# zkwebauthn/webauthn-halo2

Hardware: AMD Instinct MI355X
Metric: webauthn_es256_proofs_per_sec_k19 (higher is better)
Workload: dtype u256-montgomery (9x29-bit carry-free limbs in the hot kernels: bucket accumulation, NTT, reduction tails, quotient; 8x32-bit limbs elsewhere and in memory)

## Files before the change

include/zkmi355.h:

```cpp
#ifndef ZKMI355_H
#define ZKMI355_H

#include <stddef.h>
#include <stdint.h>

#ifdef __cplusplus
extern "C" {
#endif

#define ZK_OK 0
#define ZK_EINVAL (-1)
#define ZK_ENOMEM (-2)
#define ZK_EHIP (-3)
#define ZK_ENODEV (-4)
#define ZK_ESTATE (-5)
#define ZK_EWITNESS (-6)
#define ZK_EINTERNAL (-7)
#define ZK_ELAYOUT (-8)

typedef struct zk_ctx zk_ctx;
typedef uint64_t zk_poly;

#define ZK_BASIS_MONOMIAL 0
#define ZK_BASIS_LAGRANGE 1
// ... 106 lines not shown
#define ZK_SCHEME_GWC 1
#define ZK_SCHEME_SHPLONK 2

int zk_keygen(zk_ctx* ctx, const zk_circuit_params* params, const uint64_t* fixed_canonical ,
              size_t n_fixed_columns ,
              const uint32_t* copies, size_t n_copies, zk_pk* out);
int zk_pk_set_transcript_repr(zk_ctx* ctx, zk_pk pk, const uint64_t transcript_repr_mont[4]);
int zk_pk_free(zk_ctx* ctx, zk_pk pk);
int zk_vk_export(zk_ctx* ctx, zk_pk pk, uint64_t* fixed_commitments, uint64_t* perm_commitments,
                 uint64_t transcript_repr[4], uint32_t counts[2]);
int zk_vk_write(zk_ctx* ctx, zk_pk pk, int format, uint8_t* out, size_t cap, size_t* len);
int zk_vk_load(zk_ctx* ctx, zk_pk pk, const uint8_t* vk_bytes, size_t len, int format, const uint64_t transcript_repr_mont[4]);
int zk_pk_write(zk_ctx* ctx, zk_pk pk, int format, uint8_t* out, size_t cap, size_t* len);
int zk_pk_read(zk_ctx* ctx, const zk_circuit_params* params, const uint8_t* bytes, size_t len, int format,
               const uint64_t transcript_repr_mont[4], zk_pk* out);
int zk_pk_shape(zk_ctx* ctx, zk_pk pk, uint32_t out[8]);
int zk_quotient(zk_ctx* ctx, zk_pk pk, const zk_poly* advice_ext, size_t n_advice, const zk_poly* perm_z_ext, size_t n_chunks,
                const zk_poly* lookup_ext, size_t n_lookups, const uint64_t beta[4], const uint64_t gamma[4], const uint64_t y[4],
                int divide, zk_poly out_ext);
int zk_lookup_permute(zk_ctx* ctx, zk_pk pk, const zk_poly* advice, size_t n_advice, zk_poly* permuted_input ,
                      zk_poly* permuted_table , size_t n_lookups);
int zk_lookup_product(zk_ctx* ctx, zk_pk pk, const zk_poly* advice, size_t n_advice, const zk_poly* permuted_input,
                      const zk_poly* permuted_table, size_t n_lookups, const uint64_t beta[4], const uint64_t gamma[4],
                      zk_poly* z_out );
int zk_permutation_product(zk_ctx* ctx, zk_pk pk, const zk_poly* advice, size_t n_advice, const uint64_t beta[4],
                           const uint64_t gamma[4], zk_poly* z_out , size_t n_chunks);
#define ZK_PK_FIXED_POLY 0
#define ZK_PK_SIGMA_POLY 1
int zk_pk_export_poly(zk_ctx* ctx, zk_pk pk, int which, size_t index, zk_poly dst);
int zk_random_poly(zk_ctx* ctx, const uint8_t chacha_key[32], uint64_t first_block, zk_poly out);
int zk_proof_size(zk_ctx* ctx, zk_pk pk, int transcript, int scheme, size_t* out);
int zk_prove(zk_ctx* ctx, zk_pk pk, const zk_poly* advice, size_t n_advice, const uint8_t rng_seed[32],
             int transcript, int scheme, uint8_t* proof_out, size_t proof_cap, size_t* proof_len);
#define ZK_PROVE_BATCH_MAX 64
int zk_prove_batch(zk_ctx* ctx, zk_pk pk, size_t batch, const zk_poly* advice , size_t n_advice,
                   const uint8_t* rng_seeds , int transcript, int scheme, uint8_t* proofs_out, size_t proof_stride,
                   size_t* proof_len);
int zk_poly_upload_canonical(zk_ctx* ctx, zk_poly p, const uint64_t* host_canonical, size_t n);

#define ZK_FAIL_GATE 1
#define ZK_FAIL_GATE_BLINDED 2
#define ZK_FAIL_LOOKUP 3
#define ZK_FAIL_COPY 4
typedef struct { uint32_t kind, index, row, other_index, other_row, reserved; } zk_witness_failure;
int zk_witness_check(zk_ctx* ctx, zk_pk pk, const zk_poly* advice, size_t n_advice, zk_witness_failure* out, size_t cap,
                     uint64_t counts[5]);

#define ZK_PK_PART_FIXED_COMMIT 1
#define ZK_PK_PART_SIGMA_COMMIT 2
#define ZK_PK_PART_FIXED_POLY   3
#define ZK_PK_PART_SIGMA_POLY   4
#define ZK_PK_PART_FIXED_COSET  5
#define ZK_PK_PART_SIGMA_COSET  6
#define ZK_PK_PART_L_COSET      7
#define ZK_PK_PART_SIGMA_LABEL  8
#define ZK_PK_PART_SIGMA_MAP    9
typedef struct { uint32_t part, column, index, reserved; uint64_t count; } zk_pk_finding;

#define ZK_PK_CHECK_COMMITMENTS 1u
#define ZK_PK_CHECK_POLYS       2u
#define ZK_PK_CHECK_COSETS      4u
#define ZK_PK_CHECK_SIGMA       8u
#define ZK_PK_CHECK_ALL        15u
#define ZK_PK_CHECK_REPR       16u
int zk_pk_check(zk_ctx* ctx, zk_pk pk, uint32_t* flags, zk_pk_finding* out, size_t cap, size_t* n_findings);

int zk_vk_read(zk_ctx* ctx, const zk_circuit_params* params, const uint8_t* bytes, size_t len, int format,
               const uint64_t transcript_repr_mont[4], zk_pk* out);
int zk_vk_from_parts(zk_ctx* ctx, const zk_circuit_params* params, const uint64_t* fixed_commitments, const uint64_t* perm_commitments,
                     const uint64_t transcript_repr_mont[4], zk_pk* out);
int zk_verify(zk_ctx* ctx, zk_pk pk, int transcript, int scheme, const uint8_t* proof, size_t len, int* ok);
#define ZK_VERIFY_BATCH_MAX 1024
int zk_verify_batch(zk_ctx* ctx, zk_pk pk, size_t batch, int transcript, int scheme, const uint8_t* const* proofs, const size_t* lens,
                    uint8_t* verdicts);

#define ZK_T_MSM 0
#define ZK_T_NTT 1
#define ZK_T_QUOTIENT 2
#define ZK_T_EVAL 3
#define ZK_T_MSM_ACCUM 4
#define ZK_T_MSM_COLUMNS 5
#define ZK_T_MSM_TAIL_MAIN 6
#define ZK_T_MSM_TAIL 7
#define ZK_T_COUNT 8
int zk_last_kernel_ms(zk_ctx* ctx, int which, float* out_ms);
int zk_audit_report(zk_ctx* ctx, uint64_t counts[2], char* msg, size_t cap);
int zk_timer_reset(zk_ctx* ctx);
int zk_clock_probe(zk_ctx* ctx, uint32_t millis, uint64_t out[4]);
int zk_timer_stats(zk_ctx* ctx, int which, double* total_ms, uint64_t* count);

typedef struct {
    uint32_t n_queues;
    uint32_t flags;
    uint8_t  main_queue[8];
    uint8_t  role_queue[8][3];
    uint8_t  spare_queue[8];
    uint32_t rounds, streams;
    float    probe_ms;
} zk_placement;
#define ZK_PLACEMENT_MAINS_OK   1u
#define ZK_PLACEMENT_LONE_OK    2u
#define ZK_PLACEMENT_PAIR_OK    4u
#define ZK_PLACEMENT_LAYER1_OK  8u
#define ZK_PLACEMENT_OK        15u
#define ZK_PLACEMENT_CALIBRATED 16u
#define ZK_PLACEMENT_UNRESOLVED 32u
int zk_stream_placement(int device_id, int mode , zk_placement* out);
typedef struct {
    int32_t  slot;
    uint8_t  queue[4];
    uint64_t counts[4];
} zk_ctx_streams;
int zk_ctx_stream_info(zk_ctx* ctx, zk_ctx_streams* out);

#ifdef __cplusplus
}
#endif
#endif
```

webauthn-halo2_amd/csrc/ctx.h:

```cpp
#pragma once
#include <map>
#include <memory>
#include <new>
#include <mutex>
#include <unordered_map>
#include <vector>

#include "../../include/zkmi355.h"
#include "engine.h"
#include "audit.h"
#include "hostutil.h"

using namespace zk;

struct zk_pk_rec;

struct PolyRec {
    Fr* ptr;
    size_t n;
};

struct SrsBlock {
    int device = -1;
    G1Affine *g = nullptr, *g_lagrange = nullptr, *g_table = nullptr, *g_lagrange_table = nullptr;
    ~SrsBlock() {
        if (device >= 0) hipSetDevice(device);
        if (g) hipFree(g);
        if (g_lagrange) hipFree(g_lagrange);
        if (g_table) hipFree(g_table);
        if (g_lagrange_table) hipFree(g_lagrange_table);
    }
};

struct zk_ctx {
    int device = -1;
    hipStream_t stream = nullptr;
    int stream_slot = -1;
    bool stream_own_priority = false;
    int last_hip = 0;
    StreamAudit audit;
    bool audit_fault = false;
    std::mutex mu;
    std::map<uint32_t, Fr*> twiddles;
    std::map<uint32_t, Fr*> coset_points;
    std::map<uint32_t, Fr*> twiddles_ntt;
    std::map<uint32_t, Fr> ninv;
    std::map<uint32_t, Fr*> twiddles_ninv;
    std::map<uint32_t, Fr*> coset3_pre;
    std::map<uint32_t, Coset3Consts> coset3_consts;
    uint32_t opt_quotient_domain = 0;
    std::shared_ptr<SrsBlock> srs;
    int srs_k = -1;
    G1Affine* g = nullptr;
    G1Affine* g_lagrange = nullptr;
    G1Affine* g_table = nullptr;
    G1Affine* g_lagrange_table = nullptr;
    uint32_t table_c = 0;
    bool g_has_identity = true, g_lagrange_has_identity = true;
    bool g2_valid = false;
    uint8_t g2_raw[128] = {0}, s_g2_raw[128] = {0};
    uint64_t srs_gen = 0;
    uint32_t opt_msm_window = 0, opt_msm_batch = 0, opt_ntt_max_r = 0, opt_gp_batch_invert = 0;
    uint32_t opt_tail_stream = 0;
    uint32_t opt_tail_main_above = 0;
    uint32_t opt_batch_pass_cols = 0;
    uint32_t msm_min_cols = 0;
    uint32_t opt_no_activity_hold = 0;
    bool opt_activity_pinned = false;
    bool act_held = false;
    int act_slot = -1;
    hipStream_t tail_stream = nullptr;
    hipStream_t msm_stream = nullptr;
    hipEvent_t ev_msm_in = nullptr;
    bool msm_side = false;
    uint32_t opt_msm_stream = 0;
    uint32_t opt_msm_t1 = 0;
    hipStream_t xform_stream = nullptr;
    hipEvent_t ev_rows = nullptr, ev_xform = nullptr;
    bool xform_pending = false;
    uint32_t opt_xform_stream = 0;
    uint64_t stream_counts[4] = {0, 0, 0, 0};
    static constexpr int MSM_LANES = 3;
    struct MsmLane {
        MsmWorkspace* ws = nullptr;
        MsmWorkspace* ws_gen = nullptr;
        MsmWorkspace* ws_run = nullptr;
        hipStream_t tail = nullptr;
        hipEvent_t head_done = nullptr, tail_done = nullptr;
        hipEvent_t t_head[2] = {nullptr, nullptr};
        hipEvent_t t_acc[4] = {nullptr, nullptr, nullptr, nullptr};
        size_t n = 0;
        const G1Affine* table = nullptr;
        G1X* host_buf = nullptr;
        bool busy = false;
        uint32_t nwin = 0, cw = 0;
        uint32_t batch = 1;
        bool fixed = false;
    } lanes[MSM_LANES];
    Fr* scratch = nullptr;
    size_t scratch_n = 0;
    void* seam_buf[2] = {nullptr, nullptr};
    size_t seam_bytes[2] = {0, 0};
    Fr* small = nullptr;
    struct VerifyWs* vws = nullptr;
    Fr* host_small = nullptr;
    std::unordered_map<uint64_t, PolyRec> polys;
    static constexpr size_t POLY_SPARE_MAX = 16, POLY_SPARE_BYTES = (size_t)2 << 30;
    std::vector<PolyRec> poly_spare;
    size_t poly_spare_bytes = 0;
    uint64_t next_handle = 1;
    Fr zeta, zeta2;
    std::unordered_map<uint64_t, zk_pk_rec*> pks;
    hipEvent_t ev[ZK_T_COUNT][2] = {};
    bool ev_valid[ZK_T_COUNT] = {false};
    double acc_ms[ZK_T_COUNT] = {0};
    uint64_t acc_n[ZK_T_COUNT] = {0};
    uint64_t msm_launches = 0;
    float last_plain_ms[ZK_T_COUNT] = {0};
};

static inline hipError_t aud_record(zk_ctx* c, hipEvent_t ev, hipStream_t st) {
    const hipError_t e = hipEventRecord(ev, st);
    c->audit.record(ev, st);
    return e;
}
static inline hipError_t aud_wait(zk_ctx* c, hipStream_t st, hipEvent_t ev) {
    const hipError_t e = hipStreamWaitEvent(st, ev, 0);
    c->audit.wait(st, ev);
    return e;
}
static inline hipError_t aud_sync(zk_ctx* c, hipStream_t st) {
    const hipError_t e = hipStreamSynchronize(st);
    if (e == hipSuccess) c->audit.host_stream(st);
    return e;
}
static inline hipError_t aud_esync(zk_ctx* c, hipEvent_t ev) {
    const hipError_t e = hipEventSynchronize(ev);
    if (e == hipSuccess) c->audit.host_event(ev);
    return e;
}
static inline int aud_verdict(zk_ctx* c, uint64_t violations_before, int rc) {
    return (rc == ZK_OK && c->audit.on && c->audit.violations != violations_before) ? ZK_EINTERNAL : rc;
}

#define ZK_API(name, params, args)                          \
    static int name##_impl params;                          \
    extern "C" int name params {                            \
        try {                                               \
            return name##_impl args;                        \
        } catch (const std::bad_alloc&) {                   \
            return ZK_ENOMEM;                               \
        } catch (...) {                                     \
            return ZK_EINTERNAL;                            \
        }                                                   \
    }                                                       \
    static int name##_impl params

#define HIPCHK(ctx, x)                 \
    do {                               \
// ... 42 lines not shown
```

webauthn-halo2_amd/csrc/engine.h:

```cpp
#pragma once
#include <hip/hip_runtime.h>
#include <stddef.h>
#include <stdint.h>

#include "ec.hip.h"
#include "field.hip.h"

namespace zk {

static constexpr uint32_t NTT_MAX_BATCH = 96;
struct NttJob {
    const Fr* src;
    Fr* dst;
    Fr* tmp;
    uint32_t batch;
    const Fr* srcs[NTT_MAX_BATCH];
    Fr* dsts[NTT_MAX_BATCH];
    const Fr* tw;
    const Fr* tw_last;
    uint32_t tw_last_has_post;
    uint32_t log_n;
    uint32_t inverse;
    uint32_t n_in, n_out;
    uint32_t has_pre, has_post;
    Fr pre[3], post[3];
    const Fr* pre_tabs[NTT_MAX_BATCH];
    uint32_t max_log_r;
};
hipError_t ntt_run(const NttJob& job, hipStream_t st);
void launch_twiddles(Fr* tw, const Fr& w, uint32_t n, hipStream_t st);
void launch_twiddles_scaled(Fr* tw, const Fr& w, const Fr& scale, uint32_t n, hipStream_t st);
void launch_twiddles_internal(Fr* tw, const Fr& w, uint32_t n, hipStream_t st);

struct Coset3Consts {
    Fr inv2, inv_2z, zi, inv_2z2;
    Fr zinv[3];
};
void launch_coset3_pre(const Fr* tw_ext, uint32_t n, uint32_t j, const Fr zp1024[3], Fr* tab, hipStream_t st);
void launch_coset3_relayout(const Fr* const* src, Fr* const* dst, uint32_t count, uint32_t n, hipStream_t st);
void launch_coset3_combine(Fr* h, const Fr* tw_ext, uint32_t n, const Coset3Consts& k, hipStream_t st);

struct MsmWorkspace;
static constexpr uint32_t MSM_MAX_BATCH = 256;
MsmWorkspace* msm_workspace_create(size_t max_n, uint32_t c, hipError_t* err, uint32_t max_batch = 1);
void msm_workspace_destroy(MsmWorkspace* ws);
uint32_t msm_auto_window(size_t n, uint32_t override_c = 0);
uint32_t msm_auto_window_generic(size_t n);
uint32_t msm_num_windows(uint32_t c);
size_t msm_ws_max_n(const MsmWorkspace* ws);
uint32_t msm_ws_max_batch(const MsmWorkspace* ws);
uint32_t msm_ws_window(const MsmWorkspace* ws);
void msm_ws_set_t1_mode(MsmWorkspace* ws, uint32_t mode);
bool msm_ws_last_pass_wide(const MsmWorkspace* ws);
hipError_t msm_build_table(const G1Affine* bases, uint32_t n, uint32_t c, G1Affine* table, hipStream_t st);
bool msm_table_is_internal(uint32_t c, size_t n);
hipError_t msm_run(MsmWorkspace* ws, const Fr* const* scalars_list, uint32_t batch, const G1Affine* bases, size_t n,
                   hipStream_t st, G1X* host_window_sums, uint32_t* nwin_out, uint32_t* c_out,
                   hipEvent_t* accum_events = nullptr, const G1Affine* table = nullptr, uint32_t table_stride = 0,
                   hipStream_t tail_st = nullptr, hipEvent_t head_done = nullptr, bool bases_may_be_identity = true);
hipError_t msm_bases_have_identity(const G1Affine* bases, uint32_t n, hipStream_t st, uint32_t* d_word, uint32_t* h_word, bool* out);
uint32_t msm_sums_per_result(uint32_t c);
uint32_t msm_ws_sums_per_result(const MsmWorkspace* ws);
G1Jac msm_ws_finish_fixed(const MsmWorkspace* ws, const G1X* sums);
uint32_t msm_wide_redo_count(const MsmWorkspace* ws, const G1X* host_window_sums, uint32_t batch);
hipError_t msm_wide_redo(MsmWorkspace* ws, uint32_t batch, size_t n, hipStream_t st, G1X* host_window_sums, const G1Affine* table);
G1Jac msm_finish_host(const G1X* window_sums, uint32_t nwin, uint32_t c);

G1Affine g1_jac_to_affine_host(const G1Jac& p);

}
```

webauthn-halo2_amd/csrc/engine.hip:

```cpp
#include <stdlib.h>

#include <algorithm>
#include <atomic>
#include <chrono>
#include <new>

#include "ctx.h"
#include "placement.h"

namespace zk {
placement::Classes placement_probe(const hipStream_t* streams, int n, placement::Stamp* stamps);
uint32_t eval_blocks(uint32_t n);
void launch_eval(const Fr* c, uint32_t n, const Fr& x, Fr* scratch, hipStream_t st);
void launch_srs_lagrange_scalars(const Fr* tw, uint32_t n, const Fr& s, const Fr& c, Fr* out, hipStream_t st);
void launch_srs_fixed_base(const Fr* scalars, uint32_t n, const G1Affine* table, G1Affine* out, hipStream_t st);

G1Affine g1_jac_to_affine_host(const G1Jac& p) {
    G1Affine r;
    if (p.z.is_zero()) {
        r.x = Fq::zero();
        r.y = Fq::zero();
        return r;
    }
    const Fq zi = fe_inv_fast(p.z);
    const Fq zi2 = fe_sqr(zi);
    r.x = fe_mul(p.x, zi2);
    r.y = fe_mul(p.y, fe_mul(zi2, zi));
    return r;
}
}

int ctx_bind(zk_ctx* c) {
    hipError_t e = hipSetDevice(c->device);
    if (e != hipSuccess) {
        c->last_hip = (int)e;
        return ZK_EHIP;
    }
    return ZK_OK;
}

int ctx_ensure_scratch(zk_ctx* c, size_t n) {
    if (c->scratch_n >= n) return ZK_OK;
    if (c->xform_stream) aud_sync(c, c->xform_stream);
    if (c->scratch) hipFree(c->scratch);
    c->scratch = nullptr;
    c->scratch_n = 0;
    hipError_t e = hipMalloc(&c->scratch, n * sizeof(Fr));
    if (e != hipSuccess) {
        c->last_hip = (int)e;
        return ZK_ENOMEM;
    }
    c->scratch_n = n;
    return ZK_OK;
}

int ctx_get_twiddles(zk_ctx* c, uint32_t log_n, const Fr** out) {
    auto it = c->twiddles.find(log_n);
    if (it != c->twiddles.end()) {
        *out = it->second;
        return ZK_OK;
    }
    if (log_n > 28) return ZK_EINVAL;
    Fr* tw = nullptr;
    const size_t n = (size_t)1 << log_n;
    if (hipMalloc(&tw, n * sizeof(Fr)) != hipSuccess) return ZK_ENOMEM;
    launch_twiddles(tw, fr_omega(log_n), (uint32_t)n, c->stream);
    aud_sync(c, c->stream);
    c->twiddles[log_n] = tw;
    *out = tw;
    return ZK_OK;
}

int ctx_get_twiddles_ntt(zk_ctx* c, uint32_t log_n, const Fr** out) {
    auto it = c->twiddles_ntt.find(log_n);
    if (it != c->twiddles_ntt.end()) {
        *out = it->second;
        return ZK_OK;
    }
    if (log_n > 28) return ZK_EINVAL;
    Fr* tw = nullptr;
    const size_t n = (size_t)1 << log_n;
    if (hipMalloc(&tw, n * sizeof(Fr)) != hipSuccess) return ZK_ENOMEM;
    launch_twiddles_internal(tw, fr_omega(log_n), (uint32_t)n, c->stream);
    aud_sync(c, c->stream);
    c->twiddles_ntt[log_n] = tw;
    *out = tw;
    return ZK_OK;
}

int ctx_get_twiddles_ninv(zk_ctx* c, uint32_t log_n, const Fr** out) {
    auto it = c->twiddles_ninv.find(log_n);
    if (it != c->twiddles_ninv.end()) {
        *out = it->second;
        return ZK_OK;
    }
    if (log_n > 28) return ZK_EINVAL;
// ... 180 lines not shown
int64_t act_now() { return std::chrono::duration_cast<std::chrono::nanoseconds>(std::chrono::steady_clock::now().time_since_epoch()).count(); }
}
void ctx_activity_register(zk_ctx* c) {
    c->act_slot = -1;
    if (c->device < 0 || c->device >= ACT_DEVICES) return;
    std::atomic<uint64_t>& used = g_act_used[c->device];
    uint64_t cur = used.load();
    for (;;) {
        if (~cur == 0) return;
        const int slot = __builtin_ctzll(~cur);
        if (used.compare_exchange_weak(cur, cur | (1ull << slot))) {
            g_act_ts[c->device][slot].store(0);
            c->act_slot = slot;
            return;
        }
    }
}
void ctx_activity_unregister(zk_ctx* c) {
    if (c->act_slot < 0 || c->device < 0 || c->device >= ACT_DEVICES) return;
    g_act_ts[c->device][c->act_slot].store(0);
    g_act_used[c->device].fetch_and(~(1ull << c->act_slot));
    c->act_slot = -1;
}
static int activity_count(int device, int64_t now) {
    int active = 0;
    uint64_t used = g_act_used[device].load();
    while (used) {
        const int slot = __builtin_ctzll(used);
        used &= used - 1;
        const int64_t ts = g_act_ts[device][slot].load();
        if (ts && (ts == ACT_HELD || now - ts < ACT_WINDOW_NS)) active++;
    }
    return active;
}
int ctx_activity_touch(zk_ctx* c) {
    if (c->device < 0 || c->device >= ACT_DEVICES) return 1;
    const int64_t now = act_now();
    if (c->act_slot >= 0 && !c->act_held) g_act_ts[c->device][c->act_slot].store(now);
    return (c->act_slot >= 0 ? 0 : 1) + activity_count(c->device, now);
}
void ctx_activity_hold(zk_ctx* c, bool on) {
    if (on && c->opt_no_activity_hold) return;
    if (!on && c->opt_activity_pinned) return;
    c->act_held = on;
    if (c->act_slot < 0 || c->device < 0 || c->device >= ACT_DEVICES) return;
    g_act_ts[c->device][c->act_slot].store(on ? ACT_HELD : act_now());
}

int ctx_msm_begin_batch(zk_ctx* c, int lane, const Fr* const* d_scalars, uint32_t batch, const G1Affine* d_bases, size_t n) {
    if (lane < 0 || lane >= zk_ctx::MSM_LANES || c->lanes[lane].busy || batch == 0) return ZK_EINVAL;
    zk_ctx::MsmLane& L = c->lanes[lane];
    MsmWorkspace* ws;
    const G1Affine* table = nullptr;
    uint32_t stride = 0;
    bool ident = true;
    if (c->srs_k >= 0 && c->table_c) {
        if (d_bases == c->g) {
            table = c->g_table;
            ident = c->g_has_identity;
        } else if (d_bases == c->g_lagrange) {
            table = c->g_lagrange_table;
            ident = c->g_lagrange_has_identity;
        }
        stride = 1u << c->srs_k;
    }
    int rc = get_msm_ws(c, lane, table ? (size_t)stride : n, table ? c->table_c : 0u, &ws);
    if (rc) return rc;
    if (batch > 1 && (!table || batch > msm_ws_max_batch(ws))) return ZK_EINVAL;
    const int active = ctx_activity_touch(c);
    const uint32_t above = c->opt_tail_main_above ? c->opt_tail_main_above : 2u;
    const bool tail_on_main = c->opt_tail_stream == 2 || (c->opt_tail_stream == 0 && (uint32_t)active > above);
    if ((!tail_on_main || c->msm_side) && !c->tail_stream && ctx_side_stream(c, &c->tail_stream, 0)) return ZK_EHIP;
    L.tail = tail_on_main ? c->stream : c->tail_stream;
    if (L.tail == c->stream) c->acc_n[ZK_T_MSM_TAIL_MAIN]++;
    hipStream_t hs = c->stream;
    if (c->msm_side && c->msm_stream) {
        hs = c->msm_stream;
        HIPCHK(c, aud_record(c, c->ev_msm_in, c->stream));
        HIPCHK(c, aud_wait(c, hs, c->ev_msm_in));
        if (L.tail == c->stream) L.tail = c->tail_stream;
    }
    c->stream_counts[L.tail == c->stream ? 0 : 1]++;
    HIPCHK(c, aud_record(c, L.t_head[0], hs));
    msm_ws_set_t1_mode(ws, c->opt_msm_t1);
    HIPCHK(c, msm_run(ws, d_scalars, batch, d_bases, n, hs, L.host_buf, &L.nwin, &L.cw, L.t_acc, table, stride, L.tail,
                      L.head_done, !table || ident));
    if (c->audit.on) {
        const void* rd[MSM_MAX_BATCH];
        for (uint32_t q = 0; q < batch; q++) rd[q] = d_scalars[q];
        const void* wr[1] = {ws};
        c->audit.op_v(hs, rd, batch, wr, 1, "MSM pass: sort head + accumulation");
        if (L.tail != hs) {
            c->audit.record(L.head_done, hs);
            c->audit.wait(L.tail, L.head_done);
        }
        c->audit.op(L.tail, {ws}, {ws, L.host_buf}, "MSM pass: reduction tail");
    }
    HIPCHK(c, aud_record(c, L.tail_done, L.tail));
    HIPCHK(c, aud_record(c, L.t_head[1], hs));
    c->msm_launches++;
    L.n = n;
    L.batch = batch;
    L.table = table;
    L.fixed = table != nullptr;
    L.busy = true;
    return ZK_OK;
}

int ctx_msm_begin(zk_ctx* c, int lane, const Fr* d_scalars, const G1Affine* d_bases, size_t n) {
    return ctx_msm_begin_batch(c, lane, &d_scalars, 1, d_bases, n);
}

int ctx_msm_end_batch(zk_ctx* c, int lane, G1Jac* out) {
    if (lane < 0 || lane >= zk_ctx::MSM_LANES || !c->lanes[lane].busy) return ZK_EINVAL;
    zk_ctx::MsmLane& L = c->lanes[lane];
    L.busy = false;
    HIPCHK(c, aud_esync(c, L.tail_done));
    c->audit.host_read(L.host_buf, "MSM pass: the host collects the sums");
    if (L.fixed && L.n > 0 && msm_wide_redo_count(L.ws_run, L.host_buf, L.batch)) {
        HIPCHK(c, msm_wide_redo(L.ws_run, L.batch, L.n, L.tail, L.host_buf, L.table));
        c->audit.op(L.tail, {L.ws_run}, {L.ws_run, L.host_buf}, "MSM pass: checked redo + tail");
        HIPCHK(c, aud_sync(c, L.tail));
    }
    if (L.fixed) {
        const uint32_t per = msm_ws_sums_per_result(L.ws_run);
        for (uint32_t q = 0; q < L.batch; q++) out[q] = msm_ws_finish_fixed(L.ws_run, L.host_buf + (size_t)q * per);
    } else {
        out[0] = msm_finish_host(L.host_buf, L.nwin, L.cw);
    }
    float ms = 0.f;
    c->acc_n[ZK_T_MSM]++;
    if (L.n > 0 && hipEventElapsedTime(&ms, L.t_head[0], L.t_acc[1]) == hipSuccess) {
        c->acc_ms[ZK_T_MSM] += ms;
        c->last_plain_ms[ZK_T_MSM] = ms;
    }
    if (L.n > 0 && hipEventElapsedTime(&ms, L.t_acc[0], L.t_acc[1]) == hipSuccess) {
        c->acc_ms[ZK_T_MSM_ACCUM] += ms;
        c->acc_n[ZK_T_MSM_ACCUM]++;
        c->acc_n[ZK_T_MSM_COLUMNS] += L.batch;
        c->last_plain_ms[ZK_T_MSM_ACCUM] = ms;
    }
    if (L.n > 0 && L.fixed && msm_ws_last_pass_wide(L.ws_run) && hipEventElapsedTime(&ms, L.t_acc[2], L.t_acc[3]) == hipSuccess) {
        c->acc_ms[ZK_T_MSM_TAIL] += ms;
        c->acc_n[ZK_T_MSM_TAIL]++;
        c->last_plain_ms[ZK_T_MSM_TAIL] = ms;
    }
    return ZK_OK;
}

void ctx_msm_drain(zk_ctx* c) {
    for (int q = 0; q < zk_ctx::MSM_LANES; q++)
        if (c->lanes[q].busy) {
            aud_esync(c, c->lanes[q].tail_done);
            c->lanes[q].busy = false;
        }
}

int ctx_msm_end(zk_ctx* c, int lane, G1Jac* out) {
    if (lane >= 0 && lane < zk_ctx::MSM_LANES && c->lanes[lane].busy && c->lanes[lane].batch != 1) return ZK_EINVAL;
    return ctx_msm_end_batch(c, lane, out);
}

int ctx_msm_device(zk_ctx* c, const Fr* d_scalars, const G1Affine* d_bases, size_t n, G1Jac* out) {
    int rc = ctx_msm_begin(c, 0, d_scalars, d_bases, n);
    if (rc) return rc;
    return ctx_msm_end(c, 0, out);
}


int zk_device_count(void) {
    int n = 0;
    if (hipGetDeviceCount(&n) != hipSuccess) return 0;
    return n;
}

ZK_API(zk_device_pci_bus_id, (int device_id, char* out, size_t cap), (device_id, out, cap)) {
    if (!out || cap < 16) return ZK_EINVAL;
    int ndev = 0;
    if (hipGetDeviceCount(&ndev) != hipSuccess || ndev <= 0) return ZK_ENODEV;
    if (device_id < 0 || device_id >= ndev) return ZK_EINVAL;
    if (hipDeviceGetPCIBusId(out, (int)cap, device_id) != hipSuccess) return ZK_EHIP;
    return ZK_OK;
}
// ... 1147 lines not shown
        const Fr two = fr_from_u64(2);
        Coset3Consts q;
        q.inv2 = fe_inv_fast(two);
        q.inv_2z = fe_inv_fast(fe_mul(two, z));
        q.zi = fe_mul(z, i4);
        q.inv_2z2 = fe_inv_fast(fe_mul(two, fe_sqr(z)));
        q.zinv[0] = Fr::one();
        q.zinv[1] = c->zeta2;
        q.zinv[2] = c->zeta;
        it = c->coset3_consts.emplace(k, q).first;
    }
    if (c->audit.on) c->audit.op(c->stream, {h}, {h}, "three cosets -> h pieces");
    launch_coset3_combine(h, tw_ext, (uint32_t)n, it->second, c->stream);
    return ZK_OK;
}

static int ntt_resident(zk_ctx* c, PolyRec* src, PolyRec* dst, uint32_t log_n, bool inverse, bool coset, size_t n_out) {
    return ctx_ntt(c, src->ptr, src->n, dst->ptr, log_n, inverse, coset, n_out);
}

static uint32_t log2_exact(size_t n) {
    uint32_t l = 0;
    while (((size_t)1 << l) < n) l++;
    return ((size_t)1 << l) == n ? l : 0xffffffffu;
}

ZK_API(zk_lagrange_to_coeff, (zk_ctx* c, zk_poly h), (c, h)) {
    if (!c) return ZK_EINVAL;
    std::lock_guard<std::mutex> lk(c->mu);
    PolyRec* r = find_poly(c, h);
    if (!r) return ZK_EINVAL;
    const uint32_t lg = log2_exact(r->n);
    if (lg > 26) return ZK_EINVAL;
    int rc = ctx_bind(c);
    if (rc) return rc;
    return ntt_resident(c, r, r, lg, true, false, r->n);
}

ZK_API(zk_coeff_to_lagrange, (zk_ctx* c, zk_poly h), (c, h)) {
    if (!c) return ZK_EINVAL;
    std::lock_guard<std::mutex> lk(c->mu);
    PolyRec* r = find_poly(c, h);
    if (!r) return ZK_EINVAL;
    const uint32_t lg = log2_exact(r->n);
    if (lg > 26) return ZK_EINVAL;
    int rc = ctx_bind(c);
    if (rc) return rc;
    return ntt_resident(c, r, r, lg, false, false, r->n);
}

ZK_API(zk_coeff_to_extended, (zk_ctx* c, zk_poly src, zk_poly dst), (c, src, dst)) {
    if (!c) return ZK_EINVAL;
    std::lock_guard<std::mutex> lk(c->mu);
    PolyRec *s = find_poly(c, src), *d = find_poly(c, dst);
    if (!s || !d || s == d) return ZK_EINVAL;
    const uint32_t lg = log2_exact(d->n);
    if (lg > 26 || s->n > d->n) return ZK_EINVAL;
    int rc = ctx_bind(c);
    if (rc) return rc;
    return ntt_resident(c, s, d, lg, false, true, d->n);
}

ZK_API(zk_extended_to_coeff, (zk_ctx* c, zk_poly ext, size_t n_out), (c, ext, n_out)) {
    if (!c) return ZK_EINVAL;
    std::lock_guard<std::mutex> lk(c->mu);
    PolyRec* r = find_poly(c, ext);
    if (!r || n_out > r->n) return ZK_EINVAL;
    const uint32_t lg = log2_exact(r->n);
    if (lg > 26) return ZK_EINVAL;
    int rc = ctx_bind(c);
    if (rc) return rc;
    return ntt_resident(c, r, r, lg, true, true, n_out);
}

ZK_API(zk_eval, (zk_ctx* c, zk_poly h, const uint64_t x[4], uint64_t out[4]), (c, h, x, out)) {
    if (!c || !x || !out) return ZK_EINVAL;
    std::lock_guard<std::mutex> lk(c->mu);
    PolyRec* r = find_poly(c, h);
    if (!r || r->n > 0xffffffffu) return ZK_EINVAL;
    int rc = ctx_bind(c);
    if (rc) return rc;
    Fr xx;
    memcpy(&xx, x, 32);
    const uint32_t blocks = eval_blocks((uint32_t)r->n);
    aud_record(c, c->ev[ZK_T_EVAL][0], c->stream);
    launch_eval(r->ptr, (uint32_t)r->n, xx, c->small, c->stream);
    aud_record(c, c->ev[ZK_T_EVAL][1], c->stream);
    c->ev_valid[ZK_T_EVAL] = true;
    HIPCHK(c, hipMemcpyAsync(c->host_small, c->small + blocks, sizeof(Fr), hipMemcpyDeviceToHost, c->stream));
    HIPCHK(c, aud_sync(c, c->stream));
    memcpy(out, c->host_small, 32);
    return ZK_OK;
}

namespace zk {
uint32_t kate_division_scratch(uint32_t n);
void launch_kate_division(const Fr* p, Fr* q, uint32_t n, const Fr& z, Fr* scratch, hipStream_t st);
}

ZK_API(zk_kate_division, (zk_ctx* c, zk_poly hp, const uint64_t z[4], zk_poly hq), (c, hp, z, hq)) {
    if (!c || !z) return ZK_EINVAL;
    std::lock_guard<std::mutex> lk(c->mu);
    PolyRec* p = find_poly(c, hp);
    PolyRec* q = find_poly(c, hq);
    if (!p || !q || p->n != q->n || p->n == 0 || p->n > ((size_t)1 << 26)) return ZK_EINVAL;
    int rc = ctx_bind(c);
    if (rc) return rc;
    if ((rc = ctx_ensure_scratch(c, kate_division_scratch((uint32_t)p->n)))) return rc;
    Fr zz;
    memcpy(&zz, z, 32);
    launch_kate_division(p->ptr, q->ptr, (uint32_t)p->n, zz, c->scratch, c->stream);
    HIPCHK(c, hipGetLastError());
    HIPCHK(c, aud_sync(c, c->stream));
    return ZK_OK;
}
```

webauthn-halo2_amd/csrc/field29.hip.h:

```cpp
#pragma once
#include "field.hip.h"

namespace zk {

static constexpr uint32_t M29 = (1u << 29) - 1;

template <class PRM>
struct Lim29 {
    static constexpr uint32_t kp_limb(uint32_t K, int i) {
        uint64_t w[9] = {0, 0, 0, 0, 0, 0, 0, 0, 0};
        uint64_t carry = 0;
        for (int j = 0; j < 8; j++) {
            const uint64_t t = (uint64_t)PRM::P[j] * K + carry;
            w[j] = t & 0xffffffffu;
            carry = t >> 32;
        }
        w[8] = carry;
        const int bit = 29 * i, q = bit >> 5, o = bit & 31;
        uint64_t two = w[q];
        if (q + 1 < 9) two |= w[q + 1] << 32;
        return (uint32_t)(two >> o) & M29;
    }
    static constexpr uint32_t INV = PRM::INV & M29;
    static constexpr uint32_t spread(uint32_t K, int E, int i) {
// ... 251 lines not shown
                x[cnt] = a.l[k / 2];
                y[cnt] = a.l[k / 2];
                cnt++;
            }
            if (k == 0) mad_first(acc, a.l[0], a.l[0]);
            else madcol_v(acc, cnt, x, y);
        } else {
#pragma unroll
            for (int i = (k > 8 ? k - 8 : 0); 2 * i < k; i++) mad29<SER>(acc, a2[i], a.l[k - i]);
            if ((k & 1) == 0) mad29<SER>(acc, a.l[k / 2], a.l[k / 2]);
        }
        if (k < 9) {
            if (k) col_mp<PRM, SER>(acc, m, k, 0, k - 1);
            m[k] = ((uint32_t)acc * Lim29<PRM>::INV) & M29;
            mad29c<SER>(acc, m[k], Lim29<PRM>::P[0]);
        } else {
            col_mp<PRM, SER>(acc, m, k, k - 8, 8);
            if (ZK_MUL29_MASKRUN && SER && MUL29_BLOCK) raw[k - 9] = (uint32_t)acc;
            else r.l[k - 9] = (uint32_t)acc & M29;
        }
        acc >>= 29;
    }
    if (ZK_MUL29_MASKRUN && SER && MUL29_BLOCK) mask_run8(r.l, raw);
    r.l[8] = (uint32_t)acc;
    return r;
}

template <int K, class PRM, bool SER = MUL29_SER>
__device__ __forceinline__ Fe29<PRM> mulKadd29(const Fe29<PRM> (&a)[K], const Fe29<PRM> (&b)[K]) {
    static_assert(K >= 1 && K <= 5, "a column of 9 K + 9 products of 58 bits must fit 64 bits");
    uint32_t m[9];
    Fe29<PRM> r;
    uint64_t acc = 0;
#pragma unroll
    for (int k = 0; k < 17; k++) {
#pragma unroll
        for (int j = 0; j < K; j++) {
#pragma unroll
            for (int i = (k > 8 ? k - 8 : 0); i <= (k < 9 ? k : 8); i++) acc += (uint64_t)a[j].l[i] * b[j].l[k - i];
        }
        if (k < 9) {
#pragma unroll
            for (int i = 0; i < k; i++) acc += (uint64_t)m[i] * Lim29<PRM>::P[k - i];
            m[k] = ((uint32_t)acc * Lim29<PRM>::INV) & M29;
            acc += (uint64_t)m[k] * Lim29<PRM>::P[0];
        } else {
#pragma unroll
            for (int i = k - 8; i < 9; i++) acc += (uint64_t)m[i] * Lim29<PRM>::P[k - i];
            r.l[k - 9] = (uint32_t)acc & M29;
        }
        acc >>= 29;
    }
    r.l[8] = (uint32_t)acc;
    return r;
}

template <class PRM>
__device__ __forceinline__ Fe29<PRM> add29(const Fe29<PRM>& a, const Fe29<PRM>& b) {
    Fe29<PRM> r;
#pragma unroll
    for (int i = 0; i < 9; i++) r.l[i] = a.l[i] + b.l[i];
    return r;
}

template <uint32_t K, int E, class PRM>
__device__ __forceinline__ Fe29<PRM> sub29(const Fe29<PRM>& a, const Fe29<PRM>& b) {
    Fe29<PRM> r;
#pragma unroll
    for (int i = 0; i < 9; i++) r.l[i] = a.l[i] + (Spread29<PRM, K, E>::C[i] - b.l[i]);
    return r;
}

template <class PRM>
__device__ __forceinline__ Fe29<PRM> norm29(const Fe29<PRM>& a) {
    Fe29<PRM> r;
    uint32_t c = 0;
#pragma unroll
    for (int i = 0; i < 8; i++) {
        const uint32_t t = a.l[i] + c;
        r.l[i] = t & M29;
        c = t >> 29;
    }
    r.l[8] = a.l[8] + c;
    return r;
}

template <class PRM>
__device__ __forceinline__ bool is_zero29(const Fe29<PRM>& a) {
    uint32_t any = 0, dif = 0;
#pragma unroll
    for (int i = 0; i < 9; i++) {
        any |= a.l[i];
        dif |= a.l[i] ^ Lim29<PRM>::P[i];
    }
    return any == 0 || dif == 0;
}

template <class PRM>
struct Conv29 {
    static constexpr void pow2_words(int e, uint32_t (&out)[8]) {
        uint32_t v[8] = {1, 0, 0, 0, 0, 0, 0, 0};
        for (int s = 0; s < e; s++) {
            uint32_t carry = 0;
            for (int j = 0; j < 8; j++) {
                const uint32_t n = (v[j] << 1) | carry;
                carry = v[j] >> 31;
                v[j] = n;
            }
            bool ge = true;
            for (int j = 7; j >= 0; j--) {
                if (v[j] != PRM::P[j]) {
                    ge = v[j] > PRM::P[j];
                    break;
                }
            }
            if (ge) {
                uint64_t borrow = 0;
                for (int j = 0; j < 8; j++) {
                    const uint64_t t = (uint64_t)v[j] - PRM::P[j] - borrow;
                    v[j] = (uint32_t)t;
                    borrow = (t >> 63) & 1;
                }
            }
        }
        for (int j = 0; j < 8; j++) out[j] = v[j];
    }
    static constexpr uint32_t pow2_limb(int e, int i) {
        uint32_t w[8] = {0, 0, 0, 0, 0, 0, 0, 0};
        pow2_words(e, w);
        const int bit = 29 * i, q = bit >> 5, o = bit & 31;
        uint64_t two = w[q];
        if (q + 1 < 8) two |= (uint64_t)w[q + 1] << 32;
        return (uint32_t)(two >> o) & M29;
    }
};

template <class PRM, int E>
struct Pow2_29 {
    typedef Conv29<PRM> C;
    static constexpr uint32_t L[9] = {C::pow2_limb(E, 0), C::pow2_limb(E, 1), C::pow2_limb(E, 2), C::pow2_limb(E, 3), C::pow2_limb(E, 4),
                                      C::pow2_limb(E, 5), C::pow2_limb(E, 6), C::pow2_limb(E, 7), C::pow2_limb(E, 8)};
};
template <int E, class PRM>
__device__ __forceinline__ Fe29<PRM> const_pow2_29() {
    Fe29<PRM> r;
#pragma unroll
    for (int i = 0; i < 9; i++) r.l[i] = Pow2_29<PRM, E>::L[i];
    return r;
}

template <class PRM>
__device__ __forceinline__ Fe29<PRM> std_to_internal(const Fe<PRM>& a) {
    return mul29(to29(a), const_pow2_29<266, PRM>());
}
template <class PRM>
__device__ __forceinline__ Fe<PRM> internal_to_std(const Fe29<PRM>& a) {
    Fe<PRM> r = from29(mul29(a, const_pow2_29<256, PRM>()));
    reduce_once(r);
    return r;
}

}
```

webauthn-halo2_amd/csrc/msm.hip:

```cpp
#include <stdlib.h>
#include <string.h>
#include <vector>

#ifndef ZK_MUL29_ASM
#define ZK_MUL29_ASM 2
#endif
#ifndef ZK_TAIL_SER
#define ZK_TAIL_SER false
#endif
#ifndef ZK_T1B_SER
#define ZK_T1B_SER true
#endif
#ifndef ZK_T1B_LMAX
#define ZK_T1B_LMAX 24
#endif
#include "ec29.hip.h"
#include "engine.h"

namespace zk {

static constexpr uint32_t SIGN_BIT = 0x80000000u;
static constexpr uint32_t SKIP_ENTRY = 0xffffffffu;
static constexpr uint32_t WIDE_FLAG = 0x40000000u;
static constexpr uint32_t CHUNK = 16384;
static constexpr uint32_t SORT_LDS_BUCKETS = 8192;
#ifndef ZK_SEG0
#define ZK_SEG0 16
#endif
#ifndef ZK_GA
#define ZK_GA 4
#endif
static constexpr uint32_t SEG0 = ZK_SEG0;
static constexpr uint32_t GA = ZK_GA;
#ifndef ZK_GLANES
#define ZK_GLANES 16
#endif
static constexpr uint32_t GLANES_FIXED = ZK_GLANES;
#ifndef ZK_GSHARE
#define ZK_GSHARE 64
#endif
static constexpr uint32_t GSHARE = ZK_GSHARE;
static constexpr uint32_t PAD = SEG0 * GA;

struct MsmBatch {
    const Fr* s[MSM_MAX_BATCH];
};

struct MsmWorkspace {
    size_t max_n;
    uint32_t max_batch;
    uint32_t c, nwin, nb;
    uint32_t parts_fixed, parts_generic;
    size_t slot_elems;
    int16_t* digits;
    uint32_t* totals;
    uint32_t* bucket_start;
    uint32_t* blockbase;
    uint32_t* counts;
    uint32_t* entries;
    uint32_t* inter;
    uint32_t* coarse;
    uint32_t coarse_stride;
    uint32_t* cursor;
    size_t inter_stride;
    uint32_t* redo;
    G1X29S* slot_pt;
    G1X29S* partial;
    G1X29S* part;
    G1X* bit_sum;
    bool wide;
    bool w_redo_valid;
    uint32_t w_t1_mode;
    bool w_last_wide;
    bool w_clean;
    uint32_t* w_tot[2];
    uint32_t* w_cur[2];
    uint32_t w_par;
    uint32_t w_used_cols[2];
    uint32_t w_ib, w_fb;
    size_t w_ent_stride;
    uint32_t w_lane_stride;
    uint32_t w_slot_stride;
    uint32_t w_part_stride;
    uint32_t* w_lane_b;
    uint32_t* w_bstart;
    uint32_t* w_pstart;
    uint32_t* w_pbucket;
    G1X29S* w_part;
    G1X29S* w_rc;
};

static inline uint32_t nwin_for(uint32_t c) { return 254 / c + 1; }
#ifndef ZK_W17_MIN_LG
#define ZK_W17_MIN_LG 99
#endif
static bool msm_wide_shape(uint32_t c, size_t table_stride, uint32_t* ib_out, uint32_t* fb_out) {
    if (c < 15 || c > 17 || table_stride == 0) return false;
    const uint64_t idx = (uint64_t)nwin_for(c) * table_stride;
    uint32_t ib = 24;
    while (((uint64_t)1 << ib) < idx) ib++;
    if (ib > 26) return false;
    const uint32_t fb = 31 - ib > 7 ? 7 : 31 - ib;
    if (((1u << (c - 1)) >> fb) > 512) return false;
    if (ib_out) *ib_out = ib;
    if (fb_out) *fb_out = fb;
    return true;
}
static bool msm_wide_applies(uint32_t c, size_t table_stride) { return msm_wide_shape(c, table_stride, nullptr, nullptr); }
uint32_t msm_auto_window(size_t n, uint32_t override_c) {
    uint32_t lg = 0;
    while (((size_t)1 << (lg + 1)) <= n) lg++;
    int c = lg >= 22 ? 15 : (lg == 21 ? 16 : (lg >= ZK_W17_MIN_LG ? 17 : (lg >= 16 ? 16 : (int)lg - 5)));
    if (override_c) c = (int)override_c;
    if (c < 9) c = 9;
    if (c > 17) c = 17;
    while (c > 15 && !msm_wide_applies(c, n)) c--;
    if (c >= 15 && n < 1024) c = 14;
    return (uint32_t)c;
}

uint32_t msm_auto_window_generic(size_t n) {
    uint32_t lg = 0;
    while (((size_t)1 << (lg + 1)) <= n) lg++;
    int c = lg >= 19 ? (int)lg - 6 : (lg >= 16 ? 12 : (int)lg - 5);
    if (c > 14) c = lg >= 21 ? 15 : 14;
    if (c < 9) c = 9;
    return (uint32_t)c;
}

uint32_t msm_num_windows(uint32_t c) { return nwin_for(c); }
size_t msm_ws_max_n(const MsmWorkspace* ws) { return ws->max_n; }
uint32_t msm_ws_max_batch(const MsmWorkspace* ws) { return ws->max_batch; }
uint32_t msm_ws_window(const MsmWorkspace* ws) { return ws->c; }
void msm_ws_set_t1_mode(MsmWorkspace* ws, uint32_t mode) { ws->w_t1_mode = mode; }
bool msm_ws_last_pass_wide(const MsmWorkspace* ws) { return ws->w_last_wide; }

#include "msm_legacy.hip.h"
#include "msm_wide.hip.h"
#include "msm_tables.hip.h"


#define MSM_TRY(x)                     \
    do {                               \
        hipError_t _e = (x);           \
        if (_e != hipSuccess) {        \
            if (err) *err = _e;        \
            msm_workspace_destroy(ws); \
            return nullptr;            \
        }                              \
    } while (0)

MsmWorkspace* msm_workspace_create(size_t max_n, uint32_t c, hipError_t* err, uint32_t max_batch) {
    if (err) *err = hipSuccess;
    if (c == 0) c = msm_auto_window(max_n);
    if (max_batch == 0) max_batch = 1;
    if (c < 9 || c > 17 || (c >= 16 && !msm_wide_applies(c, max_n)) || max_n == 0 || max_n > ((size_t)1 << 26) || max_batch > MSM_MAX_BATCH) {
        if (err) *err = hipErrorInvalidValue;
        return nullptr;
    }
    MsmWorkspace* ws = new MsmWorkspace();
    memset(ws, 0, sizeof(*ws));
    ws->max_n = max_n;
    ws->max_batch = max_batch;
    ws->c = c;
    ws->nwin = nwin_for(c);
    ws->nb = 1u << (c - 1);
    ws->parts_fixed = 8;
    ws->parts_generic = 1;
    const size_t slices = ws->nwin > max_batch ? ws->nwin : max_batch;
    const size_t nbt = slices * ws->nb;
    const size_t ent = (size_t)max_batch * max_n * ws->nwin + nbt * (PAD - 1);
    const size_t nchunks = (max_n + CHUNK - 1) / CHUNK;
    const size_t threads = (ent + SEG0 - 1) / SEG0 + 1;
    size_t part_n = (size_t)ws->nwin * ws->nb * ws->parts_generic;
    if ((size_t)max_batch * ws->nb * ws->parts_fixed > part_n) part_n = (size_t)max_batch * ws->nb * ws->parts_fixed;
    MSM_TRY(hipMalloc(&ws->digits, (size_t)max_batch * max_n * ws->nwin * sizeof(int16_t)));
    MSM_TRY(hipMalloc(&ws->totals, (nbt + 1) * 4));
    MSM_TRY(hipMalloc(&ws->bucket_start, (nbt + 1) * 4));
    {
        const size_t generic_blocks = nchunks * ws->nwin, fixed_blocks = (size_t)max_batch * ((max_n + FCHUNK - 1) / FCHUNK);
        MSM_TRY(hipMalloc(&ws->blockbase, (generic_blocks > fixed_blocks ? generic_blocks : fixed_blocks) * ws->nb * 4));
    }
    MSM_TRY(hipMalloc(&ws->counts, 4 * 4 * (MSM_MAX_BATCH + 1)));
    MSM_TRY(hipMalloc(&ws->entries, ent * sizeof(uint32_t)));
    {
        const size_t nblk_max = (max_n + FCHUNK - 1) / FCHUNK;
        ws->inter_stride = max_n * ws->nwin;
        ws->coarse_stride = (uint32_t)(WHDR + nblk_max * WCB);
        MSM_TRY(hipMalloc(&ws->inter, (size_t)max_batch * ws->inter_stride * sizeof(uint32_t)));
        MSM_TRY(hipMalloc(&ws->coarse, (size_t)max_batch * ws->coarse_stride * sizeof(uint32_t)));
        MSM_TRY(hipMalloc(&ws->cursor, (size_t)max_batch * ws->nb * sizeof(uint32_t)));
    }
    MSM_TRY(hipMalloc(&ws->redo, threads * sizeof(uint32_t)));
    ws->slot_elems = threads;
    MSM_TRY(hipMalloc(&ws->slot_pt, threads * sizeof(G1X29S)));
    MSM_TRY(hipMalloc(&ws->partial, (threads / GA + 2) * sizeof(G1X29S)));
    MSM_TRY(hipMalloc(&ws->part, part_n * sizeof(G1X29S)));
    MSM_TRY(hipMalloc(&ws->bit_sum, slices * c * BITSUM_MAX_SPLIT * sizeof(G1X)));
    ws->wide = msm_wide_shape(c, max_n, &ws->w_ib, &ws->w_fb);
    ws->w_clean = false;
    if (ws->wide) {
        ws->w_ent_stride = (max_n * ws->nwin + 63) & ~(size_t)63;
        if (ws->w_ent_stride * max_batch > ent) {
            if (err) *err = hipErrorInvalidValue;
            msm_workspace_destroy(ws);
            return nullptr;
        }
        ws->w_lane_stride = (uint32_t)(ws->w_ent_stride / WL) + 64;
        ws->w_slot_stride = ws->w_lane_stride + ws->nb + 64;
        ws->w_part_stride = ((ws->w_lane_stride + 2 * ws->nb) / WCAP_MIN + ws->nb + 2 * (ws->nb >> ws->w_fb) + 127) & ~63u;
        if ((size_t)max_batch * ws->w_slot_stride > threads) {
            if (err) *err = hipErrorInvalidValue;
            msm_workspace_destroy(ws);
            return nullptr;
        }
        ws->w_tot[0] = ws->totals;
        ws->w_cur[0] = ws->cursor;
// ... 47 lines not shown
    const uint32_t WCAP = wcap_for(batch);
    uint32_t row_bits = 0;
    while ((1u << row_bits) < rows) row_bits++;
    *nwin_out = batch;
    *c_out = c;
    hipError_t e;
    WideGeo g;
    memset(&g, 0, sizeof(g));
    g.c = c;
    g.nwin = nwin;
    g.nb = nb;
    g.ib = ws->w_ib;
    g.fb = ws->w_fb;
    g.bins = nb >> g.fb;
    for (uint32_t w = 0; w < nwin; w++) {
        const uint32_t bit = c - 1 + w * c;
        g.K[bit >> 5] |= 1u << (bit & 31);
    }
#ifdef ZK_MSM_POISON
    hipMemsetAsync(ws->slot_pt, 0xA5, ws->slot_elems * sizeof(G1X29S), st);
    hipMemsetAsync(ws->w_part, 0xA5, (size_t)ws->max_batch * ws->w_part_stride * sizeof(G1X29S), st);
    hipMemsetAsync(ws->w_rc, 0xA5, (size_t)ws->max_batch * ((ws->nb >> 8) + 256) * sizeof(G1X29S), st);
#endif
    if (!ws->w_clean) {
        const uint32_t all = ws->max_batch * nb;
        uint32_t m = all;
        if (ws->max_batch * WCB > m) m = ws->max_batch * WCB;
        if (4 * (MSM_MAX_BATCH + 1) > m) m = 4 * (MSM_MAX_BATCH + 1);
        hipLaunchKernelGGL(msm_wclear_kernel, dim3((m + 255) / 256), dim3(256), 0, st, ws->w_tot[0], ws->w_cur[0], ws->w_tot[1], ws->w_cur[1],
                           all, ws->counts, ws->coarse, ws->coarse_stride, ws->max_batch);
        ws->w_used_cols[0] = ws->w_used_cols[1] = 0;
    }
    ws->w_clean = false;
    uint32_t* const totals = ws->w_tot[ws->w_par];
    uint32_t* const cursor = ws->w_cur[ws->w_par];
    uint32_t* const next_totals = ws->w_tot[ws->w_par ^ 1];
    uint32_t* const next_cursor = ws->w_cur[ws->w_par ^ 1];
    const uint32_t n32 = (uint32_t)n;
    const uint32_t lanes = (uint32_t)(((size_t)n * nwin + WL - 1) / WL);
    if (n > 0) {
        const uint32_t nblk = (n32 + FCHUNK - 1) / FCHUNK;
        MsmBatch mb;
        memset(&mb, 0, sizeof(mb));
        for (uint32_t q = 0; q < batch; q++) mb.s[q] = scalars_list[q];
        const dim3 gh(nblk, batch);
        if (c == 17) {
            hipLaunchKernelGGL(msm_whist_kernel<17>, gh, dim3(256), 0, st, mb, n32, g, ws->coarse, ws->coarse_stride, ws->counts);
            hipLaunchKernelGGL(msm_wscatter1_kernel<17>, gh, dim3(256), 0, st, mb, n32, g, table_stride, ws->coarse, ws->coarse_stride,
                               ws->inter, ws->inter_stride, ws->counts, WCAP);
        } else if (c == 16) {
            hipLaunchKernelGGL(msm_whist_kernel<16>, gh, dim3(256), 0, st, mb, n32, g, ws->coarse, ws->coarse_stride, ws->counts);
            hipLaunchKernelGGL(msm_wscatter1_kernel<16>, gh, dim3(256), 0, st, mb, n32, g, table_stride, ws->coarse, ws->coarse_stride,
                               ws->inter, ws->inter_stride, ws->counts, WCAP);
        } else {
            hipLaunchKernelGGL(msm_whist_kernel<15>, gh, dim3(256), 0, st, mb, n32, g, ws->coarse, ws->coarse_stride, ws->counts);
            hipLaunchKernelGGL(msm_wscatter1_kernel<15>, gh, dim3(256), 0, st, mb, n32, g, table_stride, ws->coarse, ws->coarse_stride,
                               ws->inter, ws->inter_stride, ws->counts, WCAP);
        }
        const uint32_t max_chunks = (uint32_t)(((uint64_t)n32 * nwin + SUB - 1) / SUB) + g.bins;
        hipLaunchKernelGGL(msm_wfinehist_kernel, dim3(max_chunks + 1, batch), dim3(256), 0, st, ws->inter, ws->inter_stride, ws->coarse,
                           ws->coarse_stride, g, totals, next_totals, next_cursor, ws->w_used_cols[ws->w_par ^ 1]);
        hipLaunchKernelGGL(msm_wscatter2_kernel, dim3(max_chunks + 1, batch), dim3(256), 0, st, ws->inter, ws->inter_stride, ws->coarse,
                           ws->coarse_stride, g, totals, ws->w_bstart, cursor, ws->entries, ws->w_ent_stride, ws->w_lane_b, ws->w_lane_stride,
                           ws->w_pstart, ws->w_pbucket, ws->w_part_stride, WCAP);
        if (accum_events) hipEventRecord(accum_events[0], st);
        if (bases_may_be_identity) {
            hipLaunchKernelGGL(msm_wacc_kernel, dim3((lanes + 63) / 64, batch), dim3(64), 0, st, ws->entries, ws->w_ent_stride, table, ws->counts,
                               ws->w_lane_b, ws->w_lane_stride, ws->w_bstart, nb, ws->slot_pt, ws->w_slot_stride, g.ib);
        } else {
            hipLaunchKernelGGL(msm_wacc_fast_kernel, dim3((lanes + 63) / 64, batch), dim3(64), 0, st, ws->entries, ws->w_ent_stride, table,
                               ws->counts, ws->w_lane_b, ws->w_lane_stride, ws->w_bstart, nb, ws->slot_pt, ws->w_slot_stride, ws->redo, g.ib);
        }
        if (accum_events) hipEventRecord(accum_events[1], st);
    }
    hipStream_t ts = st;
    if (tail_st && tail_st != st) {
        if ((e = hipEventRecord(head_done, st)) != hipSuccess) return e;
        if ((e = hipStreamWaitEvent(tail_st, head_done, 0)) != hipSuccess) return e;
        ts = tail_st;
    }
    if (accum_events && accum_events[2]) hipEventRecord(accum_events[2], ts);
    if (n > 0) {
        const uint32_t max_parts = (lanes + 2 * nb) / WCAP + nb + 2 * g.bins + 64;
        const bool per_bucket = ws->w_t1_mode == 1;
        uint32_t lmin = 0;
        if (per_bucket) {
            lmin = ZK_T1B_LMAX;
            hipLaunchKernelGGL(msm_wbucket_kernel, dim3(nb / 64, batch), dim3(64), 0, ts, ws->slot_pt, ws->w_slot_stride, totals, ws->w_bstart,
                               ws->w_pstart, ws->w_part_stride, nb, ws->w_part, WCAP, lmin);
        }
        hipLaunchKernelGGL(msm_wparts_kernel, dim3((max_parts + 63) / 64, batch), dim3(64), 0, ts, ws->slot_pt, ws->w_slot_stride, totals,
                           ws->w_bstart, ws->w_pstart, ws->w_pbucket, ws->w_part_stride, nb, ws->counts, ws->w_part, WCAP, lmin);
    }
    hipLaunchKernelGGL(msm_wrowcol_kernel, dim3(rows + 256, batch), dim3(64), 0, ts, ws->w_part, ws->w_part_stride, totals, ws->w_bstart,
                       ws->w_pstart, nb, ws->w_rc, WCAP);
    G1X* out_dev = nullptr;
    if ((e = hipHostGetDevicePointer((void**)&out_dev, host_window_sums, 0)) != hipSuccess) return e;
    hipLaunchKernelGGL(msm_wbits_kernel, dim3(9 + row_bits, batch), dim3(64), 0, ts, ws->w_rc, nb, out_dev, ws->counts);
    if (accum_events && accum_events[3]) hipEventRecord(accum_events[3], ts);
    if ((e = hipGetLastError()) != hipSuccess) return e;
    ws->w_clean = true;
    ws->w_redo_valid = n > 0 && !bases_may_be_identity;
    if (n > 0) {
        ws->w_used_cols[ws->w_par] = batch;
        ws->w_used_cols[ws->w_par ^ 1] = 0;
        ws->w_par ^= 1;
    }
    return hipSuccess;
}

uint32_t msm_wide_redo_count(const MsmWorkspace* ws, const G1X* host_window_sums, uint32_t batch) {
    if (!ws->wide || !ws->w_redo_valid) return 0;
    uint32_t v;
    memcpy(&v, host_window_sums + (size_t)batch * WIDE_SUMS, 4);
    return v;
}

hipError_t msm_wide_redo(MsmWorkspace* ws, uint32_t batch, size_t n, hipStream_t st, G1X* host_window_sums, const G1Affine* table) {
    if (!ws->wide || n == 0 || batch == 0 || batch > ws->max_batch) return hipErrorInvalidValue;
    const uint32_t nb = ws->nb, rows = nb >> 8, nwin = ws->nwin, WCAP = wcap_for(batch);
    uint32_t row_bits = 0;
    while ((1u << row_bits) < rows) row_bits++;
    const uint32_t lanes = (uint32_t)(((size_t)n * nwin + WL - 1) / WL);
    const uint32_t bins = nb >> ws->w_fb;
    uint32_t* const totals = ws->w_tot[ws->w_par ^ 1];
    hipLaunchKernelGGL(msm_wacc_redo_kernel, dim3(256), dim3(64), 0, st, ws->entries, ws->w_ent_stride, table, ws->counts, ws->w_lane_b,
                       ws->w_lane_stride, ws->w_bstart, nb, ws->slot_pt, ws->w_slot_stride, ws->redo, ws->w_ib);
    hipError_t e = hipMemsetAsync(ws->counts + 1, 0, 4, st);
    if (e != hipSuccess) return e;
    const uint32_t max_parts = (lanes + 2 * nb) / WCAP + nb + 2 * bins + 64;
    hipLaunchKernelGGL(msm_wparts_kernel, dim3((max_parts + 63) / 64, batch), dim3(64), 0, st, ws->slot_pt, ws->w_slot_stride, totals,
                       ws->w_bstart, ws->w_pstart, ws->w_pbucket, ws->w_part_stride, nb, ws->counts, ws->w_part, WCAP, 0u);
    hipLaunchKernelGGL(msm_wrowcol_kernel, dim3(rows + 256, batch), dim3(64), 0, st, ws->w_part, ws->w_part_stride, totals, ws->w_bstart,
                       ws->w_pstart, nb, ws->w_rc, WCAP);
    G1X* out_dev = nullptr;
    if ((e = hipHostGetDevicePointer((void**)&out_dev, host_window_sums, 0)) != hipSuccess) return e;
    hipLaunchKernelGGL(msm_wbits_kernel, dim3(9 + row_bits, batch), dim3(64), 0, st, ws->w_rc, nb, out_dev, ws->counts);
    return hipGetLastError();
}

hipError_t msm_run(MsmWorkspace* ws, const Fr* const* scalars_list, uint32_t batch, const G1Affine* bases, size_t n,
                   hipStream_t st, G1X* host_window_sums, uint32_t* nwin_out, uint32_t* c_out, hipEvent_t* accum_events,
                   const G1Affine* table, uint32_t table_stride, hipStream_t tail_st, hipEvent_t head_done,
                   bool bases_may_be_identity) {
    if (n > ws->max_n || batch == 0 || batch > ws->max_batch) return hipErrorInvalidValue;
    const uint32_t c = ws->c, nwin = ws->nwin, nb = ws->nb;
    const bool fixed = table != nullptr;
    ws->w_redo_valid = false;
    ws->w_last_wide = fixed && ws->wide && table_stride == ws->max_n;
    if (fixed && ws->wide && table_stride == ws->max_n)
        return msm_run_wide(ws, scalars_list, batch, n, st, host_window_sums, nwin_out, c_out, accum_events, table, table_stride, tail_st,
                            head_done, bases_may_be_identity);
    if (c > 15) return hipErrorInvalidValue;
    ws->w_clean = false;
    const bool fused = fixed && nb <= SORT_LDS_BUCKETS;
    if (!fused && batch != 1) return hipErrorInvalidValue;
    const Fr* scalars = scalars_list[0];
    const uint32_t slices = fixed ? batch : nwin;
    const uint32_t nbt = slices * nb;
    const uint32_t parts = fixed ? ws->parts_fixed : ws->parts_generic;
    *nwin_out = slices;
    *c_out = c;
    hipError_t e;
    {
#ifdef ZK_MSM_POISON
        hipMemsetAsync(ws->part, 0xA5, (size_t)nbt * parts * sizeof(G1X29S), st);
#endif
        const uint32_t clear_parts = n > 0 ? 0u : nbt * parts;
        uint32_t m = nbt + 1;
        if (clear_parts > m) m = clear_parts;
        if (batch * CBINS_MAX > m) m = batch * CBINS_MAX;
        const bool sort2 = sort2_applies(fused, n, nb, nwin, table_stride);
        hipLaunchKernelGGL(msm_clear_kernel, dim3((m + 255) / 256), dim3(256), 0, st, ws->part, clear_parts, ws->totals, nbt + 1,
                           ws->counts, ws->cursor, sort2 ? nbt : 0u, ws->coarse, ws->coarse_stride, sort2 ? batch : 0u);
    }
    if (n > 0) {
        const uint32_t n32 = (uint32_t)n;
        const uint32_t stride = (uint32_t)ws->max_n;
        const uint32_t nchunks = (n32 + CHUNK - 1) / CHUNK;
        const bool sort2 = sort2_applies(fused, n, nb, nwin, table_stride);
        if (sort2) {
            const uint32_t nblk = (n32 + FCHUNK - 1) / FCHUNK;
            MsmBatch mb;
            memset(&mb, 0, sizeof(mb));
            for (uint32_t q = 0; q < batch; q++) mb.s[q] = scalars_list[q];
            hipLaunchKernelGGL(msm_recode_hist2_kernel, dim3(nblk, batch), dim3(256), (nb + 256 * 9) * 4, st, mb, n32, stride, c, nwin, nb,
                               ws->digits, ws->totals, ws->coarse, ws->coarse_stride);
            hipLaunchKernelGGL(msm_scan_kernel, dim3(1), dim3(1024), 0, st, ws->totals, ws->bucket_start, nbt, ws->counts);
            hipLaunchKernelGGL(msm_scan_coarse_kernel, dim3(batch), dim3(CBINS_MAX), 0, st, ws->totals, nb, ws->coarse, ws->coarse_stride, nb >> 6, 6u);
            hipLaunchKernelGGL(msm_scatter1_kernel, dim3(nblk, batch), dim3(256), 0, st, ws->digits, n32, stride, nwin, nb, table_stride,
                               ws->coarse, ws->coarse_stride, ws->inter, ws->inter_stride, 6u);
            const uint32_t max_chunks = (uint32_t)(((uint64_t)n32 * nwin + SUB - 1) / SUB) + (nb >> 6);
            hipLaunchKernelGGL(msm_scatter2_kernel, dim3(max_chunks, batch), dim3(256), 0, st, ws->inter, ws->inter_stride, ws->coarse,
                               ws->coarse_stride, nb, ws->totals, ws->bucket_start, ws->cursor, ws->entries, 6u, PAD, (size_t)0, (const uint8_t*)nullptr);
        } else if (fused) {
            const uint32_t nblk = (n32 + FCHUNK - 1) / FCHUNK;
            MsmBatch mb;
            memset(&mb, 0, sizeof(mb));
            for (uint32_t q = 0; q < batch; q++) mb.s[q] = scalars_list[q];
            hipLaunchKernelGGL(msm_recode_hist_kernel, dim3(nblk, batch), dim3(256), (nb + 256 * 9) * 4, st, mb, n32, stride, c,
                               nwin, nb, ws->digits, ws->totals, ws->blockbase);
            hipLaunchKernelGGL(msm_scan_kernel, dim3(1), dim3(1024), 0, st, ws->totals, ws->bucket_start, nbt, ws->counts);
            const uint32_t per_launch = n32 >= (1u << 18) ? 1 : batch;
            for (uint32_t q = 0; q < batch; q += per_launch)
                hipLaunchKernelGGL(msm_scatter_fixed_kernel, dim3(nblk, per_launch), dim3(SCAT_T), nb * 4, st,
                                   ws->digits + (size_t)q * nwin * stride, n32, stride, nwin, nb, table_stride,
                                   ws->totals + (size_t)q * nb, ws->bucket_start + (size_t)q * nb,
                                   ws->blockbase + (size_t)q * nblk * nb, ws->entries);
        } else {
            hipLaunchKernelGGL(msm_recode_kernel, dim3((n32 + 255) / 256), dim3(256), 0, st, scalars, n32, stride, c, nwin,
                               ws->digits);
            hipLaunchKernelGGL(msm_sort_kernel<false>, dim3(nchunks * nwin), dim3(256), (nb < SORT_LDS_BUCKETS ? nb : SORT_LDS_BUCKETS) * 4, st, ws->digits, n32, stride,
                               nchunks, nb, fixed ? 1u : 0u, table_stride, ws->totals, ws->bucket_start, ws->blockbase,
                               (uint32_t*)nullptr);
            hipLaunchKernelGGL(msm_scan_kernel, dim3(1), dim3(1024), 0, st, ws->totals, ws->bucket_start, nbt, ws->counts);
            hipLaunchKernelGGL(msm_sort_kernel<true>, dim3(nchunks * nwin), dim3(256), (nb < SORT_LDS_BUCKETS ? nb : SORT_LDS_BUCKETS) * 4, st, ws->digits, n32, stride,
                               nchunks, nb, fixed ? 1u : 0u, table_stride, ws->totals, ws->bucket_start, ws->blockbase,
                               ws->entries);
            hipLaunchKernelGGL(msm_pad_kernel, dim3((nbt + 255) / 256), dim3(256), 0, st, ws->totals, ws->bucket_start, nbt,
                               ws->entries);
        }
        const size_t worst = (size_t)(fixed ? batch : 1) * n * nwin + (size_t)nbt * (PAD - 1);
        const size_t threads = (worst + SEG0 - 1) / SEG0;
        if (accum_events) hipEventRecord(accum_events[0], st);
        if (bases_may_be_identity) {
            hipLaunchKernelGGL(msm_accumulate_kernel, dim3((uint32_t)((threads + 63) / 64)), dim3(64), 0, st, ws->entries,
                               fixed ? table : bases, ws->counts, ws->slot_pt);
        } else {
            hipLaunchKernelGGL(msm_accumulate_fast_kernel, dim3((uint32_t)((threads + 63) / 64)), dim3(64), 0, st, ws->entries,
                               fixed ? table : bases, ws->counts, ws->redo, ws->slot_pt);
        }
        if (accum_events) hipEventRecord(accum_events[1], st);
// ... 70 lines not shown
```

webauthn-halo2_amd/csrc/ntt.hip:

```cpp
#include <stdlib.h>
#include <string.h>

#include "engine.h"
#include "field29.hip.h"
#include "ntt_plan.h"

namespace zk {

#ifndef ZK_NTT_TILE_LOG
#define ZK_NTT_TILE_LOG 9
#endif
#ifndef ZK_NTT_MINW
#define ZK_NTT_MINW 1
#endif
#ifndef ZK_NTT_PAD
#define ZK_NTT_PAD 1
#endif
static constexpr int NTT_TILE_LOG = ZK_NTT_TILE_LOG;
typedef Fe29<FrParams> Fr29;

struct NttPassArgs {
    const Fr* in[NTT_MAX_BATCH];
    Fr* out[NTT_MAX_BATCH];
    const Fr* tw;
    const Fr* tw_last;
    uint32_t log_n;
    uint32_t log_r;
    uint32_t log_ns;
    uint32_t log_t;
    uint32_t inverse;
    uint32_t last;
    uint32_t n_in;
    uint32_t n_out;
    uint32_t has_pre;
    uint32_t has_post;
    Fr pre[3];
    const Fr* pre_tab[NTT_MAX_BATCH];
    Fr post[3];
};

#ifndef ZK_NTT_SOA
#define ZK_NTT_SOA 0
#endif
__device__ __forceinline__ uint32_t swz(uint32_t i) { return i ^ (((i >> 6) & 3u) << 4); }
__device__ __forceinline__ Fr29 tile_load(const uint32_t* lds, uint32_t tile, uint32_t row, uint32_t p, uint32_t t, uint32_t log_t) {
    Fr29 r;
#if ZK_NTT_SOA
    const uint32_t* q = lds + swz((p << log_t) | t);
#pragma unroll
    for (int i = 0; i < 9; i++) r.l[i] = q[i * tile];
#else
    const uint32_t* q = lds + p * row + t * 9;
#pragma unroll
    for (int i = 0; i < 9; i++) r.l[i] = q[i];
#endif
    return r;
}
__device__ __forceinline__ void tile_store(uint32_t* lds, uint32_t tile, uint32_t row, uint32_t p, uint32_t t, uint32_t log_t, const Fr29& a) {
#if ZK_NTT_SOA
    uint32_t* q = lds + swz((p << log_t) | t);
#pragma unroll
    for (int i = 0; i < 9; i++) q[i * tile] = a.l[i];
#else
    uint32_t* q = lds + p * row + t * 9;
#pragma unroll
    for (int i = 0; i < 9; i++) q[i] = a.l[i];
#endif
}
__device__ __forceinline__ Fr29 lds_load29(const uint32_t* p) {
    Fr29 r;
#pragma unroll
    for (int i = 0; i < 9; i++) r.l[i] = p[i];
    return r;
}
__device__ __forceinline__ void lds_store29(uint32_t* p, const Fr29& a) {
#pragma unroll
    for (int i = 0; i < 9; i++) p[i] = a.l[i];
}

__device__ __forceinline__ Fr29 reduce_below_2_256(const Fr29& a) {
    const uint32_t t = a.l[8] >> 22;
    const uint32_t m = (t * 84u) >> 6;
    Fr29 r;
    int64_t acc = 0;
#pragma unroll
    for (int i = 0; i < 8; i++) {
        acc += (int64_t)a.l[i] - (int64_t)((uint64_t)m * Lim29<FrParams>::P[i]);
        r.l[i] = (uint32_t)acc & M29;
        acc >>= 29;
    }
    acc += (int64_t)a.l[8] - (int64_t)((uint64_t)m * Lim29<FrParams>::P[8]);
    r.l[8] = (uint32_t)acc;
    return r;
}

__device__ __forceinline__ Fr reduce_canonical(const Fr29& a) {
    constexpr uint32_t P8 = Lim29<FrParams>::P[8];
    constexpr uint64_t M = ((uint64_t)1 << 53) / (P8 + 1);
    static_assert(M < ((uint64_t)1 << 32), "M must fit a word");
    const uint32_t qe = (uint32_t)(((uint64_t)a.l[8] * (uint32_t)M) >> 53);
    Fr29 r;
    int64_t acc = 0;
#pragma unroll
    for (int i = 0; i < 8; i++) {
        acc += (int64_t)a.l[i] - (int64_t)((uint64_t)qe * Lim29<FrParams>::P[i]);
        r.l[i] = (uint32_t)acc & M29;
        acc >>= 29;
    }
    acc += (int64_t)a.l[8] - (int64_t)((uint64_t)qe * Lim29<FrParams>::P[8]);
    r.l[8] = (uint32_t)acc;
    Fr o = from29(r);
    reduce_once(o);
    return o;
}

template <int E = 29>
__device__ __forceinline__ void bfly_mul(Fr29& u, Fr29& v, const Fr29& w) {
    const Fr29 t = mul29(v, w);
    v = sub29<3, 29>(u, t);
    u = add29(u, t);
}
template <uint32_t K, int E>
__device__ __forceinline__ void bfly_plain(Fr29& u, Fr29& v) {
    const Fr29 t = v;
    v = sub29<K, E>(u, t);
    u = add29(u, t);
}

template <uint32_t KIN>
__device__ __forceinline__ void round0(Fr29& e0, Fr29& e1, Fr29& e2, Fr29& e3, const Fr29& w4) {
    bfly_plain<KIN + 1, 29>(e0, e1);
    bfly_plain<KIN + 1, 29>(e2, e3);
    bfly_plain<2 * KIN + 1, 30>(e0, e2);
    bfly_mul(e1, e3, w4);
}

enum { NTT_GENERAL = 0, NTT_FOLD = 1, NTT_ZQ = 2 };
template <uint32_t KIN, int MODE, int TL = NTT_TILE_LOG>
#ifndef ZK_NTT_WAVES
#define ZK_NTT_WAVES 0
#endif
#if ZK_NTT_WAVES
__attribute__((amdgpu_waves_per_eu(ZK_NTT_WAVES, ZK_NTT_WAVES)))
#endif
__global__ __launch_bounds__(1 << (TL - 2), ZK_NTT_MINW) void ntt_pass_kernel(const NttPassArgs a) {
    constexpr uint32_t NTT_THREADS = 1u << (TL - 2);
    constexpr int NTT_TILE_LOG = TL;
    extern __shared__ __attribute__((aligned(16))) uint32_t lds[];
    const Fr* __restrict__ vin = a.in[blockIdx.y];
    Fr* __restrict__ vout = a.out[blockIdx.y];

    const uint32_t N = 1u << a.log_n;
    const uint32_t R = 1u << a.log_r;
    const uint32_t T = 1u << a.log_t;
    const uint32_t tile = R * T;
    const uint32_t j0 = blockIdx.x * T;
    const uint32_t ns_mask = (1u << a.log_ns) - 1;
    const uint32_t col_stride = N >> a.log_r;
    const uint32_t tw_shift = a.log_n - a.log_ns - a.log_r;
    const uint32_t nmask = N - 1;
    const uint32_t row = T * 9 + ZK_NTT_PAD;
    uint32_t* wr = lds + (ZK_NTT_SOA ? 9 * tile : R * row);
    const uint32_t brev_shift = 32 - a.log_r;

    for (uint32_t j = threadIdx.x; j < (R >> 1); j += NTT_THREADS) {
        const uint32_t ex = j << (a.log_n - a.log_r);
        lds_store29(wr + j * 9, to29(fe_load(a.tw + (a.inverse ? ((N - ex) & nmask) : ex))));
    }

    auto src_index = [&](uint32_t e, uint32_t& t, uint32_t& r) {
        t = e & (T - 1);
        r = e >> a.log_t;
        return j0 + t + r * col_stride;
    };
    auto tw_index = [&](uint32_t t, uint32_t r) {
        const uint32_t ex = (r * ((j0 + t) & ns_mask)) << tw_shift;
        return a.inverse ? ((N - ex) & nmask) : ex;
    };
    const Fr* __restrict__ twl = MODE == NTT_FOLD ? a.tw_last : a.tw;
    const Fr* __restrict__ ptab = (MODE == NTT_GENERAL && a.log_ns == 0) ? a.pre_tab[blockIdx.y] : nullptr;
    auto place = [&](uint32_t t, uint32_t r, uint32_t idx, const Fr& v, const Fr& w, uint32_t ti) {
        Fr29 x;
        if (idx < a.n_in) {
            if (MODE == NTT_FOLD) {
                x = mul29(to29(v), to29(w));
            } else if (a.log_ns == 0) {
                if (ptab) {
                    x = mul29(to29(v), to29(w));
                } else {
                    const uint32_t m = a.has_pre ? idx % 3 : 0;
                    x = m ? mul29(to29(v), to29(a.pre[m])) : to29_x32(v);
                }
            } else {
                x = to29(v);
                if (ti) x = mul29(x, to29(w));
            }
// ... 308 lines not shown
```

webauthn-halo2_amd/csrc/poly.hip:

```cpp
#include "engine.h"
#include "prover.h"
#include <string.h>

namespace zk {

__global__ __launch_bounds__(256) void poly_eval_partial_kernel(const Fr* __restrict__ c, uint32_t n, Fr x, Fr y,
                                                                Fr* __restrict__ block_out) {
    __shared__ Fr sh[256];
    const uint32_t S = gridDim.x * 256;
    const uint32_t t = blockIdx.x * 256 + threadIdx.x;
    Fr acc = Fr::zero();
    if (t < n) {
        uint32_t m = (n - 1 - t) / S;
        acc = fe_load(c + t + m * S);
        while (m-- > 0) acc = fe_add(fe_mul(acc, y), fe_load(c + t + m * S));
        Fr xp = Fr::one();
        Fr base = x;
        for (uint32_t e = t; e; e >>= 1) {
            if (e & 1) xp = fe_mul(xp, base);
            base = fe_sqr(base);
        }
        acc = fe_mul(acc, xp);
    }
    sh[threadIdx.x] = acc;
    __syncthreads();
    for (uint32_t s = 128; s > 0; s >>= 1) {
        if (threadIdx.x < s) sh[threadIdx.x] = fe_add(sh[threadIdx.x], sh[threadIdx.x + s]);
        __syncthreads();
    }
    if (threadIdx.x == 0) fe_store(block_out + blockIdx.x, sh[0]);
}

__global__ __launch_bounds__(256) void poly_sum_kernel(const Fr* __restrict__ in, uint32_t m, Fr* __restrict__ out) {
    __shared__ Fr sh[256];
    Fr acc = Fr::zero();
    for (uint32_t i = threadIdx.x; i < m; i += 256) acc = fe_add(acc, fe_load(in + i));
    sh[threadIdx.x] = acc;
    __syncthreads();
    for (uint32_t s = 128; s > 0; s >>= 1) {
        if (threadIdx.x < s) sh[threadIdx.x] = fe_add(sh[threadIdx.x], sh[threadIdx.x + s]);
        __syncthreads();
    }
    if (threadIdx.x == 0) fe_store(out, sh[0]);
}

uint32_t eval_blocks(uint32_t n) {
    uint32_t b = (n + 256 * 16 - 1) / (256 * 16);
    if (b < 1) b = 1;
    if (b > 1024) b = 1024;
    return b;
}

void launch_eval(const Fr* c, uint32_t n, const Fr& x, Fr* scratch, hipStream_t st) {
    const uint32_t blocks = eval_blocks(n);
    const uint32_t S = blocks * 256;
    Fr y = Fr::one(), base = x;
    for (uint32_t e = S; e; e >>= 1) {
        if (e & 1) y = fe_mul(y, base);
        base = fe_sqr(base);
    }
    hipLaunchKernelGGL(poly_eval_partial_kernel, dim3(blocks), dim3(256), 0, st, c, n, x, y, scratch);
    hipLaunchKernelGGL(poly_sum_kernel, dim3(1), dim3(256), 0, st, scratch, blocks, scratch + blocks);
}

__global__ __launch_bounds__(256) void poly_eval_batch_kernel(const EvalItem* __restrict__ items, uint32_t n, uint32_t M,
                                                              Fr* __restrict__ block_out) {
    __shared__ Fr sh[256];
    const uint32_t e = blockIdx.y;
    const Fr* __restrict__ c = items[e].poly;
    const Fr y = items[e].y;
    const uint32_t base = blockIdx.x * 256 * M + threadIdx.x;
    Fr acc = Fr::zero();
#pragma unroll 1
    for (uint32_t m = M; m-- > 0;) {
        const uint32_t idx = base + 256 * m;
        if (idx < n) {
            const Fr v = fe_load(c + idx);
            acc = fe_add(fe_mul(acc, y), v);
        }
    }
    sh[threadIdx.x] = acc;
    __syncthreads();
    const uint32_t live = min(256u, n - min(n, blockIdx.x * 256 * M));
#pragma unroll 1
    for (int l = 7; l >= 0; l--) {
        const uint32_t s = 1u << l;
        if (s >= live) continue;
        if (threadIdx.x < s) sh[threadIdx.x] = fe_add(sh[threadIdx.x], fe_mul(sh[threadIdx.x + s], items[e].pw[l]));
        __syncthreads();
    }
    if (threadIdx.x == 0) fe_store(block_out + e * gridDim.x + blockIdx.x, sh[0]);
}

__global__ __launch_bounds__(256) void poly_sum_batch_kernel(const EvalItem* __restrict__ items, const Fr* __restrict__ in, uint32_t m,
                                                             Fr* __restrict__ out) {
    __shared__ Fr sh[256];
    const uint32_t e = blockIdx.x;
    const Fr* src = in + (size_t)e * m;
    Fr acc = Fr::zero();
#pragma unroll 1
    for (uint32_t q = (m + 255) / 256; q-- > 0;) {
        const uint32_t idx = threadIdx.x + 256 * q;
        if (idx < m) acc = fe_add(fe_mul(acc, items[e].zpw[8]), fe_load(src + idx));
    }
    sh[threadIdx.x] = acc;
    __syncthreads();
#pragma unroll 1
    for (int l = 7; l >= 0; l--) {
        const uint32_t s = 1u << l;
        if (s >= m) continue;
        if (threadIdx.x < s) sh[threadIdx.x] = fe_add(sh[threadIdx.x], fe_mul(sh[threadIdx.x + s], items[e].zpw[l]));
        __syncthreads();
    }
    if (threadIdx.x == 0) fe_store(out + e, sh[0]);
}

void launch_eval_batch(EvalItem* h_items, EvalItem* d_items, uint32_t count, uint32_t n, Fr* scratch, Fr* out,
                       hipStream_t st) {
    const uint32_t blocks = eval_blocks(n);
    const uint32_t M = (n + blocks * 256 - 1) / (blocks * 256);
    uint32_t distinct[16], nd = 0;
    for (uint32_t e = 0; e < count; e++) {
        EvalItem& it = h_items[e];
        uint32_t same = count;
        for (uint32_t d = 0; d < nd; d++)
            if (memcmp(&h_items[distinct[d]].x, &it.x, sizeof(Fr)) == 0) {
                same = distinct[d];
                break;
            }
        if (same != count) {
            memcpy(it.pw, h_items[same].pw, sizeof(it.pw) + sizeof(it.y) + sizeof(it.zpw));
            continue;
        }
        if (nd < 16) distinct[nd++] = e;
        it.pw[0] = it.x;
        for (int l = 1; l < 8; l++) it.pw[l] = fe_sqr(it.pw[l - 1]);
        it.y = fe_sqr(it.pw[7]);
        Fr z = Fr::one(), base = it.y;
        for (uint32_t k = M; k; k >>= 1) {
            if (k & 1) z = fe_mul(z, base);
            base = fe_sqr(base);
        }
        it.zpw[0] = z;
        for (int l = 1; l < 9; l++) it.zpw[l] = fe_sqr(it.zpw[l - 1]);
    }
    hipMemcpyAsync(d_items, h_items, (size_t)count * sizeof(EvalItem), hipMemcpyHostToDevice, st);
    hipLaunchKernelGGL(poly_eval_batch_kernel, dim3(blocks, count), dim3(256), 0, st, d_items, n, M, scratch);
    hipLaunchKernelGGL(poly_sum_batch_kernel, dim3(count), dim3(256), 0, st, d_items, scratch, blocks, out);
}


__global__ __launch_bounds__(256) void coset3_pre_kernel(const Fr* __restrict__ tw_ext, uint32_t n, uint32_t j, Fr z0, Fr z1, Fr z2,
                                                         Fr* __restrict__ tab) {
    const uint32_t m = blockIdx.x * 256 + threadIdx.x;
    if (m >= n) return;
    const uint32_t r = m % 3;
    fe_store(tab + m, fe_mul(fe_load(tw_ext + (size_t)j * m), r == 0 ? z0 : r == 1 ? z1 : z2));
}
void launch_coset3_pre(const Fr* tw_ext, uint32_t n, uint32_t j, const Fr zp1024[3], Fr* tab, hipStream_t st) {
    hipLaunchKernelGGL(coset3_pre_kernel, dim3((n + 255) / 256), dim3(256), 0, st, tw_ext, n, j, zp1024[0], zp1024[1], zp1024[2], tab);
}

struct Coset3Vecs {
    const Fr* src[32];
    Fr* dst[32];
};
__global__ __launch_bounds__(256) void coset3_relayout_kernel(Coset3Vecs v, uint32_t n) {
    const uint32_t i = blockIdx.x * 256 + threadIdx.x;
    if (i >= n) return;
    const Fr* __restrict__ s = v.src[blockIdx.y];
    Fr* __restrict__ d = v.dst[blockIdx.y];
#pragma unroll
    for (uint32_t j = 0; j < 3; j++) fe_store(d + (size_t)j * n + i, fe_load(s + 4 * (size_t)i + j));
}
void launch_coset3_relayout(const Fr* const* src, Fr* const* dst, uint32_t count, uint32_t n, hipStream_t st) {
    for (uint32_t c0 = 0; c0 < count; c0 += 32) {
        Coset3Vecs v;
        const uint32_t cnt = count - c0 < 32 ? count - c0 : 32;
        for (uint32_t q = 0; q < cnt; q++) {
            v.src[q] = src[c0 + q];
            v.dst[q] = dst[c0 + q];
        }
        hipLaunchKernelGGL(coset3_relayout_kernel, dim3((n + 255) / 256, cnt), dim3(256), 0, st, v, n);
    }
}

__global__ __launch_bounds__(256) void coset3_combine_kernel(Fr* __restrict__ h, const Fr* __restrict__ tw_ext, uint32_t n, Coset3Consts k) {
    const uint32_t m = blockIdx.x * 256 + threadIdx.x;
    if (m >= n) return;
    const uint32_t N4 = 4 * n;
    const Fr v0 = fe_load(h + m);
    const Fr v1 = fe_mul(fe_load(h + (size_t)n + m), fe_load(tw_ext + ((N4 - m) & (N4 - 1))));
    const Fr v2 = fe_mul(fe_load(h + 2 * (size_t)n + m), fe_load(tw_ext + ((N4 - 2 * m) & (N4 - 1))));
    const Fr h1 = fe_mul(fe_sub(v0, v2), k.inv_2z);
    const Fr A = fe_mul(fe_add(v0, v2), k.inv2);
    const Fr B = fe_sub(v1, fe_mul(h1, k.zi));
    const Fr h0 = fe_mul(fe_add(A, B), k.inv2);
    const Fr h2 = fe_mul(fe_sub(A, B), k.inv_2z2);
    const uint32_t r = m % 3;
    const Fr s = r == 0 ? k.zinv[0] : r == 1 ? k.zinv[1] : k.zinv[2];
    fe_store(h + m, fe_mul(h0, s));
    fe_store(h + (size_t)n + m, fe_mul(h1, s));
    fe_store(h + 2 * (size_t)n + m, fe_mul(h2, s));
}
void launch_coset3_combine(Fr* h, const Fr* tw_ext, uint32_t n, const Coset3Consts& k, hipStream_t st) {
    hipLaunchKernelGGL(coset3_combine_kernel, dim3((n + 255) / 256), dim3(256), 0, st, h, tw_ext, n, k);
}


__global__ __launch_bounds__(256) void srs_lagrange_scalars_kernel(const Fr* __restrict__ tw, uint32_t n, Fr s, Fr c,
                                                                   Fr* __restrict__ out) {
    const uint32_t i = blockIdx.x * 256 + threadIdx.x;
    if (i >= n) return;
    const Fr wi = fe_load(tw + i);
    const Fr d = fe_sub(s, wi);
    fe_store(out + i, fe_mul(fe_mul(wi, c), fe_inv(d)));
}

__global__ __launch_bounds__(64) void srs_fixed_base_kernel(const Fr* __restrict__ scalars, uint32_t n,
                                                            const G1Affine* __restrict__ table,
                                                            G1Affine* __restrict__ out) {
    const uint32_t i = blockIdx.x * 64 + threadIdx.x;
    if (i >= n) return;
    const Fr s = fe_from_mont(fe_load(scalars + i));
    G1X acc = G1X::identity();
#pragma unroll 1
    for (int w = 0; w < 32; w++) {
// ... 30 lines not shown
```

webauthn-halo2_amd/csrc/prover.hip:

```cpp
#include <stdlib.h>

#include <algorithm>
#include <deque>
#include <functional>
#include <memory>
#include <unordered_map>
#include <vector>

#include "pk.h"
#include "transcript.h"
#include "vkrepr.h"

using namespace zk;

#ifdef ZK_HOST_TRACE
#include <chrono>
#include <cstdio>
static std::chrono::steady_clock::time_point& ht_last() {
    static thread_local std::chrono::steady_clock::time_point t = std::chrono::steady_clock::now();
    return t;
}
#define HT(name)                                                                                                  \
    do {                                                                                                          \
        const auto ht_now = std::chrono::steady_clock::now();                                                     \
// ... 1009 lines not shown
    };

    struct EvIdx {
        size_t i_fix = 0, i_rand = 0, i_sig = 0, i_z = 0, i_lk = 0, n_written = 0;
    };
    void build_evals(std::vector<Q>& ev, EvIdx& ix) const {
        for (auto& aq : lay.advice_queries) ev.push_back(Q{pk->adv_poly[aq.first], aq.second, Fr::zero()});
        ix.i_fix = ev.size();
        for (uint32_t f = 0; f < lay.n_fix; f++) ev.push_back(Q{pk->fixed_poly[f], 0, Fr::zero()});
        ix.i_rand = ev.size();
        ev.push_back(Q{pk->random_poly, 0, Fr::zero()});
        ix.i_sig = ev.size();
        for (uint32_t p = 0; p < lay.perm_cols.size(); p++) ev.push_back(Q{pk->sigma_poly[p], 0, Fr::zero()});
        ix.i_z = ev.size();
        for (uint32_t ci = 0; ci < lay.n_chunks; ci++) {
            ev.push_back(Q{pk->z_poly[ci], 0, Fr::zero()});
            ev.push_back(Q{pk->z_poly[ci], 1, Fr::zero()});
            if (ci != lay.n_chunks - 1) ev.push_back(Q{pk->z_poly[ci], lay.last_rot, Fr::zero()});
        }
        ix.i_lk = ev.size();
        for (uint32_t l = 0; l < lay.n_lookups; l++) {
            ev.push_back(Q{pk->lk_z_poly[l], 0, Fr::zero()});
            ev.push_back(Q{pk->lk_z_poly[l], 1, Fr::zero()});
            ev.push_back(Q{pk->lk_ap_poly[l], 0, Fr::zero()});
            ev.push_back(Q{pk->lk_ap_poly[l], -1, Fr::zero()});
            ev.push_back(Q{pk->lk_sp_poly[l], 0, Fr::zero()});
        }
        ix.n_written = ev.size();
        ev.push_back(Q{pk->h_comb, 0, Fr::zero()});
    }
    std::vector<Q> queries_from_evals(const std::vector<Q>& ev, const EvIdx& ix) const {
        std::vector<Q> queries(ev.begin(), ev.begin() + ix.i_fix);
        std::vector<Q> lastq(lay.n_chunks);
        size_t pos = ix.i_z;
        for (uint32_t ci = 0; ci < lay.n_chunks; ci++) {
            queries.push_back(ev[pos++]);
            queries.push_back(ev[pos++]);
            if (ci != lay.n_chunks - 1) lastq[ci] = ev[pos++];
        }
        for (int ci = (int)lay.n_chunks - 2; ci >= 0; ci--) queries.push_back(lastq[ci]);
        pos = ix.i_lk;
        for (uint32_t l = 0; l < lay.n_lookups; l++, pos += 5) {
            queries.push_back(ev[pos]);
            queries.push_back(ev[pos + 2]);
            queries.push_back(ev[pos + 4]);
            queries.push_back(ev[pos + 3]);
            queries.push_back(ev[pos + 1]);
        }
        for (size_t i = ix.i_fix; i < ix.i_rand; i++) queries.push_back(ev[i]);
        for (size_t i = ix.i_sig; i < ix.i_z; i++) queries.push_back(ev[i]);
        queries.push_back(ev[ix.n_written]);
        queries.push_back(ev[ix.i_rand]);
        return queries;
    }
    void combine_h(const Fr& x) {
        const Fr xn = fr_pow(x, n);
        LincombArgs a;
        memset(&a, 0, sizeof(a));
        a.out = pk->h_comb;
        a.n = n;
        a.count = lay.n_h;
        Fr p = Fr::one();
        for (uint32_t i = 0; i < lay.n_h; i++) {
            a.in[i] = pk->h_ext + (size_t)i * n;
            a.len[i] = n;
            a.c[i] = p;
            a.unit[i] = i == 0;
            p = fe_mul(p, xn);
        }
        A({pk->h_ext}, {pk->h_comb}, "h(X) from its pieces");
        launch_lincomb(a, st);
    }

    int begin() {
        xside = !batch_member && (c->opt_xform_stream == 1 || (c->opt_xform_stream == 0 && lay.k >= 18 && ctx_activity_touch(c) <= 1));
        c->msm_side = !batch_member && (c->opt_msm_stream == 1 || (c->opt_msm_stream == 0 && xside && c->opt_xform_stream == 0));
        if ((xside || c->msm_side || c->audit_fault) && (rc = ctx_lone_streams(c))) return rc;
        c->stream_counts[2] += xside;
        c->stream_counts[3] += c->msm_side;
        if ((rc = ctx_get_twiddles(c, lay.k, &tw)) || (rc = ctx_get_twiddles(c, lay.ext_k, &tw_ext))) return rc;
        {
            const uint32_t above = c->opt_tail_main_above ? c->opt_tail_main_above : 2u;
            loaded = c->opt_tail_stream == 2 || (c->opt_tail_stream == 0 && (uint32_t)ctx_activity_touch(c) > above);
        }
        cosets3 = lay.n_h == 3 && 3 <= ctx_ntt_max_batch(lay.k) &&
                  (c->opt_quotient_domain == 2 || (c->opt_quotient_domain == 0 && lay.k >= 16));
        if (cosets3 && !pk->is_member && (rc = pk_ensure_cosets3(c, pk))) return rc;
        omega = fr_omega(lay.k);
        omega_inv = fe_inv_fast(omega);
        tr->common_scalar(pk->transcript_repr);
        return ZK_OK;
    }

    int run(const Fr* const* advice_dev, int scheme) {
        if (begin()) return rc;
        const uint32_t bf = BLINDING_FACTORS, usable = lay.usable;

        const bool many = lay.n_adv > BATCH_ARGS_MIN;
        if (many) {
            CopyPair* h = static_cast<CopyPair*>(pk->h_batch_args);
            for (uint32_t j = 0; j < lay.n_adv; j++) h[j] = CopyPair{advice_dev[j], pk->adv_val[j]};
            if (c->audit.on) {
                std::vector<const void*> rd, wr;
                for (uint32_t j = 0; j < lay.n_adv; j++) {
                    rd.push_back(advice_dev[j]);
                    wr.push_back(pk->adv_val[j]);
                }
                AV(rd, wr, "advice columns into the workspace");
            }
            if (hipMemcpyAsync(pk->d_batch_args, h, lay.n_adv * sizeof(CopyPair), hipMemcpyHostToDevice, st) != hipSuccess) return ZK_EHIP;
            launch_copy_columns(static_cast<const CopyPair*>(pk->d_batch_args), lay.n_adv, n, st);
            if (aud_sync(c, st) != hipSuccess) return ZK_EHIP;
        }
        for (uint32_t j = 0; j < lay.n_adv; j++) {
            if (!many) {
                A({advice_dev[j]}, {pk->adv_val[j]}, "advice column into the workspace");
                hipMemcpyAsync(pk->adv_val[j], advice_dev[j], (size_t)n * sizeof(Fr), hipMemcpyDeviceToDevice, st);
            }
            set_rows(pk->adv_val[j], usable, draw(bf + 1));
        }
        draw(lay.n_adv);
        const bool pipe = lay.n_adv == 1 && lay.n_lookups == 1;
        const uint32_t max_batch = ctx_msm_max_batch(c);
        bool adv_transformed = false;
        if (pipe) {
            commit_begin(0, pk->adv_val[0], n, ZK_BASIS_LAGRANGE);
            if (xform_side()) {
                transforms({Forms{pk->adv_val[0], pk->adv_poly[0], pk->adv_coset[0]}});
                adv_transformed = true;
            }
        } else {
            LaneFifo f{{0, 1, 2}, {}};
            for (uint32_t j0 = 0; j0 < lay.n_adv && ok(); j0 += max_batch) {
                const uint32_t j1 = std::min(lay.n_adv, j0 + max_batch);
                std::vector<const Fr*> cols;
                for (uint32_t j = j0; j < j1; j++) cols.push_back(pk->adv_val[j]);
                fifo_begin_batch(f, cols, n, ZK_BASIS_LAGRANGE);
                std::vector<Forms> fm;
                for (uint32_t j = j0; j < j1; j++) fm.push_back(Forms{pk->adv_val[j], pk->adv_poly[j], pk->adv_coset[j]});
                transforms(fm);
            }
            fifo_drain(f);
        }
        if (!ok()) return rc;

        const uint32_t T = 1u << lay.lookup_bits;
        Fr theta = Fr::zero();
        bool theta_done = false;
        auto squeeze_theta = [&]() {
            if (!theta_done) {
                if (pipe) commit_end_write(0);
                theta = tr->squeeze();
                theta_done = true;
            }
        };
        hipMemsetAsync(pk->lks.err, 0, 4, st);
        LaneFifo lf{pipe ? std::vector<int>{1, 2} : std::vector<int>{0, 1, 2}, {}};
        Batcher lb{&lf, ZK_BASIS_LAGRANGE, max_batch, {}};
        std::vector<uint32_t> due;
        auto lookup_transforms = [&](bool with_advice) {
            std::vector<Forms> fm;
            if (with_advice) fm.push_back(Forms{pk->adv_val[0], pk->adv_poly[0], pk->adv_coset[0]});
            for (uint32_t l : due) {
                fm.push_back(Forms{pk->lk_ap[l], pk->lk_ap_poly[l], pk->lk_ap_coset[l]});
                fm.push_back(Forms{pk->lk_sp[l], pk->lk_sp_poly[l], pk->lk_sp_coset[l]});
            }
// ... 439 lines not shown
            }
            launch_kate_division_batch(bufs, bufs, zs, cnt, n, pk->kd_scratch, st);
        }
        {
            std::vector<Term> terms;
            Fr pv = Fr::one();
            for (size_t si = 0; si < rsets.size(); si++) {
                terms.push_back(Term{sbuf[si], pv});
                pv = fe_mul(pv, v);
            }
            lincomb_many(hx, terms, false, Fr::zero());
        HT("hx launched");
        }
        return rc;
    }
    int shplonk_stage2(Shplonk& S, const Fr** out) {
        const Fr u = tr->squeeze();
        HT("u squeezed");
        std::vector<Term> terms;
        Fr sub = Fr::zero();
        Fr pv = Fr::one();
        std::vector<Fr> z_diffs;
        for (auto& rs : S.rsets) {
            std::vector<Fr> diffs;
            for (int r : S.all_rots)
                if (std::find(rs.rots.begin(), rs.rots.end(), r) == rs.rots.end()) diffs.push_back(sh_rot_pt(S, r).pt);
            const Fr zi = vanishing_eval(diffs, u);
            z_diffs.push_back(zi);
            Fr py = Fr::one();
            for (size_t ci : rs.coms) {
                const Fr coef = fe_mul(fe_mul(pv, zi), py);
                terms.push_back(Term{S.com[ci].poly, coef});
                sub = fe_add(sub, fe_mul(coef, eval_small(S.low[ci], u)));
                py = fe_mul(py, S.yc);
            }
            pv = fe_mul(pv, S.v);
        }
        std::vector<Fr> all_pts;
        for (int r : S.all_rots) all_pts.push_back(sh_rot_pt(S, r).pt);
        const Fr zt = vanishing_eval(all_pts, u);
        terms.push_back(Term{S.hx, fe_neg(zt)});
        lincomb_many(pk->t_a, terms, true, sub);
        HT("L launched");
        A({pk->t_a}, {pk->t_b}, "SHPLONK: final division");
        launch_kate_division(pk->t_a, pk->t_b, n, u, pk->kd_scratch, st);
        A({pk->t_b}, {pk->t_b}, "SHPLONK: scale");
        launch_scale(pk->t_b, fe_inv_fast(z_diffs[0]), n, st);
        *out = pk->t_b;
        return rc;
    }
    int open_shplonk(const std::vector<Q>& queries, const Fr& x) {
        Shplonk S;
        if (int r = shplonk_stage1(queries, x, S)) return r;
        commit_write(S.hx, n, ZK_BASIS_MONOMIAL);
        if (!ok()) return rc;
        const Fr* last = nullptr;
        if (int r = shplonk_stage2(S, &last)) return r;
        commit_write(last, n, ZK_BASIS_MONOMIAL);
        return rc;
    }
};

#include "prover_batch.h"

}

namespace {
struct ProveQuiesce {
    zk_ctx* c;
    explicit ProveQuiesce(zk_ctx* ctx) : c(ctx) { ctx_activity_hold(c, true); }
    ProveQuiesce(const ProveQuiesce&) = delete;
    ProveQuiesce& operator=(const ProveQuiesce&) = delete;
    void settle() {
        ctx_msm_drain(c);
        if (c->msm_side) {
            aud_sync(c, c->msm_stream);
            c->msm_side = false;
        }
        if (c->xform_pending) {
            aud_sync(c, c->xform_stream);
            c->xform_pending = false;
        }
        aud_sync(c, c->stream);
        ctx_activity_hold(c, false);
    }
    ~ProveQuiesce() { settle(); }
};
}

ZK_API(zk_proof_size, (zk_ctx* c, zk_pk pkh, int transcript, int scheme, size_t* out), (c, pkh, transcript, scheme, out)) {
    if (!c || !out) return ZK_EINVAL;
    std::lock_guard<std::mutex> g(c->mu);
    auto it = c->pks.find(pkh);
    if (it == c->pks.end()) return ZK_EINVAL;
    if (transcript != ZK_TRANSCRIPT_BLAKE2B && transcript != ZK_TRANSCRIPT_EVM) return ZK_EINVAL;
    if (scheme == ZK_SCHEME_DEFAULT) scheme = transcript == ZK_TRANSCRIPT_EVM ? ZK_SCHEME_GWC : ZK_SCHEME_SHPLONK;
    if (scheme != ZK_SCHEME_GWC && scheme != ZK_SCHEME_SHPLONK) return ZK_EINVAL;
    const Layout& lay = it->second->lay;
    size_t points = lay.n_adv + 3 * lay.n_lookups + lay.n_chunks + 1 + lay.n_h;
    points += scheme == ZK_SCHEME_SHPLONK ? 2 : 5 + (lay.n_chunks > 1 ? 1 : 0);
    const size_t evals = lay.advice_queries.size() + lay.n_fix + 1 + lay.perm_cols.size() + 3 * lay.n_chunks - 1 +
                         5 * lay.n_lookups;
    *out = points * (transcript == ZK_TRANSCRIPT_EVM ? 64 : 32) + evals * 32;
    return ZK_OK;
}

ZK_API(zk_prove, (zk_ctx* c, zk_pk h, const zk_poly* advice, size_t n_advice, const uint8_t rng_seed[32], int transcript, int scheme, uint8_t* proof_out, size_t proof_cap, size_t* proof_len), (c, h, advice, n_advice, rng_seed, transcript, scheme, proof_out, proof_cap, proof_len)) {
    if (!c || !advice || !rng_seed || !proof_len) return ZK_EINVAL;
    std::lock_guard<std::mutex> lk(c->mu);
    auto it = c->pks.find(h);
    if (it == c->pks.end()) return ZK_EINVAL;
    zk_pk_rec* pk = it->second;
    const Layout& lay = pk->lay;
    if (pk->srs_gen != c->srs_gen) return ZK_ESTATE;
    if (pk->verify_only) return ZK_ESTATE;
    if (n_advice != lay.n_adv || c->srs_k != (int)lay.k) return ZK_EINVAL;
    if (transcript != ZK_TRANSCRIPT_BLAKE2B && transcript != ZK_TRANSCRIPT_EVM) return ZK_EINVAL;
    if (scheme == ZK_SCHEME_DEFAULT) scheme = transcript == ZK_TRANSCRIPT_EVM ? ZK_SCHEME_GWC : ZK_SCHEME_SHPLONK;
    if (scheme != ZK_SCHEME_GWC && scheme != ZK_SCHEME_SHPLONK) return ZK_EINVAL;
    int rc = ctx_bind(c);
    if (rc) return rc;
    std::vector<const Fr*> adv(n_advice);
    for (size_t j = 0; j < n_advice; j++) {
        auto pit = c->polys.find(advice[j]);
        if (pit == c->polys.end() || pit->second.n != lay.n) return ZK_EINVAL;
        adv[j] = pit->second.ptr;
    }
    EvmTranscript evm;
    Blake2bTranscript b2;
    Transcript* tr = transcript == ZK_TRANSCRIPT_EVM ? (Transcript*)&evm : (Transcript*)&b2;
    const uint64_t aud0 = c->audit.violations;
    c->audit.base_of.clear();
    Prover p(c, pk, rng_seed, tr);
    {
        ProveQuiesce quiesce(c);
        rc = p.run(adv.data(), scheme);
    }
    if ((rc = aud_verdict(c, aud0, rc))) return rc;
    if (hipGetLastError() != hipSuccess) return ZK_EHIP;
    *proof_len = tr->out.size();
    if (!proof_out || proof_cap < tr->out.size()) return proof_out ? ZK_EINVAL : ZK_OK;
    memcpy(proof_out, tr->out.data(), tr->out.size());
    return ZK_OK;
}

namespace {
struct PhaseCtx {
    zk_ctx* c;
    zk_pk_rec* pk;
    std::vector<Fr*> adv;
};
int phase_open(zk_ctx* c, zk_pk h, const zk_poly* advice, size_t n_advice, PhaseCtx& out) {
    auto it = c->pks.find(h);
    if (it == c->pks.end()) return ZK_EINVAL;
    zk_pk_rec* pk = it->second;
    if (pk->srs_gen != c->srs_gen || pk->verify_only) return ZK_ESTATE;
    if (n_advice != pk->lay.n_adv) return ZK_EINVAL;
    out.c = c;
    out.pk = pk;
    for (size_t j = 0; j < n_advice; j++) {
        auto pit = c->polys.find(advice[j]);
        if (pit == c->polys.end() || pit->second.n != pk->lay.n) return ZK_EINVAL;
        out.adv.push_back(pit->second.ptr);
    }
    return ctx_bind(c);
}
// ... 340 lines not shown
```

webauthn-halo2_amd/csrc/prover_kernels.hip:

```cpp
#include <string.h>

#include "prover.h"
#include "field29.hip.h"
#include "hostutil.h"

namespace zk {


__global__ void to_mont_kernel(Fr* a, uint32_t n) {
    const uint32_t i = blockIdx.x * blockDim.x + threadIdx.x;
    if (i < n) fe_store(a + i, fe_to_mont(fe_load(a + i)));
}
void launch_to_mont(Fr* a, uint32_t n, hipStream_t st) {
    hipLaunchKernelGGL(to_mont_kernel, dim3((n + 255) / 256), dim3(256), 0, st, a, n);
}

__global__ void mul_kernel(Fr* out, const Fr* a, const Fr* b, uint32_t n) {
    const uint32_t i = blockIdx.x * blockDim.x + threadIdx.x;
    if (i < n) fe_store(out + i, fe_mul(fe_load(a + i), fe_load(b + i)));
}
void launch_mul(Fr* out, const Fr* a, const Fr* b, uint32_t n, hipStream_t st) {
    hipLaunchKernelGGL(mul_kernel, dim3((n + 255) / 256), dim3(256), 0, st, out, a, b, n);
}

__global__ __launch_bounds__(256) void lincomb_kernel(LincombArgs a) {
    typedef Fe29<FrParams> Fr29;
    const uint32_t i = blockIdx.x * blockDim.x + threadIdx.x;
    if (i >= a.n) return;
    Fr29 zero;
#pragma unroll
    for (int l = 0; l < 9; l++) zero.l[l] = 0;
    auto get = [&](uint32_t j) { return i < a.len[j] ? to29(fe_load(a.in[j] + i)) : zero; };
    Fr29 acc = a.accumulate ? to29(fe_load(a.out + i)) : zero;
    uint32_t j = 0;
#pragma unroll 1
    while (j < a.count) {
        if (a.unit[j]) {
            acc = norm29(add29(acc, get(j)));
            j++;
        } else if (j + 4 <= a.count && !a.unit[j + 1] && !a.unit[j + 2] && !a.unit[j + 3]) {
            const Fr29 v[4] = {get(j), get(j + 1), get(j + 2), get(j + 3)};
            const Fr29 c[4] = {to29(a.c[j]), to29(a.c[j + 1]), to29(a.c[j + 2]), to29(a.c[j + 3])};
            acc = norm29(add29(acc, mulKadd29<4>(v, c)));
            j += 4;
        } else {
            acc = norm29(add29(acc, mul29(get(j), to29(a.c[j]))));
            j++;
        }
    }
    if (i == 0 && a.sub0) acc = norm29(sub29<2, 29>(acc, to29(a.sub0_val)));
    if (i < a.sub_low_n) acc = norm29(sub29<2, 29>(acc, to29(a.sub_low[i])));
    Fr r = from29(mul29(acc, const_pow2_29<261, FrParams>()));
    reduce_once(r);
    fe_store(a.out + i, r);
}
void launch_lincomb(const LincombArgs& a, hipStream_t st) {
    LincombArgs b = a;
    const Fr k32 = fr_from_u64(32);
    for (uint32_t j = 0; j < b.count; j++)
        if (!b.unit[j]) b.c[j] = fe_mul(b.c[j], k32);
    hipLaunchKernelGGL(lincomb_kernel, dim3((b.n + 255) / 256), dim3(256), 0, st, b);
}

__global__ __launch_bounds__(256) void lincomb_terms_kernel(const LcTerm* __restrict__ terms, uint32_t count, Fr* __restrict__ out,
                                                            uint32_t log_ns, uint32_t sub0, Fr sub0_val, uint32_t low_n, LcLow low) {
    typedef Fe29<FrParams> Fr29;
    __shared__ uint32_t part[256 * 9];
    const uint32_t ns = 1u << log_ns, rows = 256u >> log_ns;
    const uint32_t row = threadIdx.x & (rows - 1), sl = threadIdx.x >> (8 - log_ns);
    const uint32_t i = blockIdx.x * rows + row;
    const Fr29 id = const_pow2_29<261, FrParams>();
    Fr29 acc;
#pragma unroll
    for (int l = 0; l < 9; l++) acc.l[l] = 0;
    uint32_t j = sl, groups = 0;
#pragma unroll 1
    for (; j + 3 * ns < count; j += 4 * ns) {
        const Fr29 v[4] = {to29(fe_load(terms[j].in + i)), to29(fe_load(terms[j + ns].in + i)),
                           to29(fe_load(terms[j + 2 * ns].in + i)), to29(fe_load(terms[j + 3 * ns].in + i))};
        const Fr29 c[4] = {to29(fe_load(&terms[j].c)), to29(fe_load(&terms[j + ns].c)), to29(fe_load(&terms[j + 2 * ns].c)),
                           to29(fe_load(&terms[j + 3 * ns].c))};
        acc = norm29(add29(acc, mulKadd29<4>(v, c)));
        if (++groups == 64) {
            acc = mul29(acc, id);
            groups = 0;
        }
    }
#pragma unroll 1
    for (; j < count; j += ns) acc = norm29(add29(acc, mul29(to29(fe_load(terms[j].in + i)), to29(fe_load(&terms[j].c)))));
    const Fr29 share = mul29(acc, id);
#pragma unroll
    for (int l = 0; l < 9; l++) part[l * 256 + threadIdx.x] = share.l[l];
    __syncthreads();
    if (sl) return;
    Fr29 total = share;
    for (uint32_t s = 1; s < ns; s++) {
        Fr29 v;
#pragma unroll
        for (int l = 0; l < 9; l++) v.l[l] = part[l * 256 + s * rows + row];
        total = norm29(add29(total, v));
    }
    if (i == 0 && sub0) total = norm29(sub29<2, 29>(total, to29(sub0_val)));
    if (i < low_n) total = norm29(sub29<2, 29>(total, to29(low.v[i])));
    Fr r = from29(mul29(total, id));
    reduce_once(r);
    fe_store(out + i, r);
}
void launch_lincomb_terms(LcTerm* h_terms, LcTerm* d_terms, uint32_t count, Fr* out, uint32_t n, bool sub0, const Fr& sub0_val,
                          const Fr* low, uint32_t low_n, hipStream_t st) {
    const Fr k32 = fr_from_u64(32);
    for (uint32_t j = 0; j < count; j++) h_terms[j].c = fe_mul(h_terms[j].c, k32);
    hipMemcpyAsync(d_terms, h_terms, (size_t)count * sizeof(LcTerm), hipMemcpyHostToDevice, st);
    uint32_t lg = 0;
    while ((1u << (lg + 1)) <= n) lg++;
    uint32_t log_ns = 0;
    while (log_ns < 4 && lg + log_ns < 16 && (count >> (log_ns + 1)) >= 8) log_ns++;
    LcLow lw;
    memset(&lw, 0, sizeof(lw));
    for (uint32_t t = 0; t < low_n && t < 8; t++) lw.v[t] = low[t];
    hipLaunchKernelGGL(lincomb_terms_kernel, dim3(n >> (8 - log_ns)), dim3(256), 0, st, d_terms, count, out, log_ns, sub0 ? 1u : 0u,
                       sub0_val, low_n, lw);
}

__global__ void scale_kernel(Fr* a, Fr c, uint32_t n) {
    const uint32_t i = blockIdx.x * blockDim.x + threadIdx.x;
    if (i < n) fe_store(a + i, fe_mul(fe_load(a + i), c));
}
void launch_scale(Fr* a, const Fr& c, uint32_t n, hipStream_t st) {
    hipLaunchKernelGGL(scale_kernel, dim3((n + 255) / 256), dim3(256), 0, st, a, c, n);
}

__device__ __forceinline__ uint32_t rotl(uint32_t x, int n) { return (x << n) | (x >> (32 - n)); }
#define QR(a, b, c, d)                 \
    a += b; d ^= a; d = rotl(d, 16);   \
    c += d; b ^= c; b = rotl(b, 12);   \
    a += b; d ^= a; d = rotl(d, 8);    \
    c += d; b ^= c; b = rotl(b, 7);

__global__ void chacha_fr_kernel(ChaChaKey key, uint64_t start_block, Fr* out, uint32_t count) {
    const uint32_t i = blockIdx.x * blockDim.x + threadIdx.x;
    if (i >= count) return;
    const uint64_t ctr = start_block + i;
    uint32_t s[16] = {0x61707865, 0x3320646e, 0x79622d32, 0x6b206574};
#pragma unroll
    for (int k = 0; k < 8; k++) s[4 + k] = key.w[k];
    s[12] = (uint32_t)ctr;
    s[13] = (uint32_t)(ctr >> 32);
    s[14] = 0;
    s[15] = 0;
    uint32_t w[16];
#pragma unroll
    for (int k = 0; k < 16; k++) w[k] = s[k];
#pragma unroll 1
    for (int r = 0; r < 10; r++) {
        QR(w[0], w[4], w[8], w[12]) QR(w[1], w[5], w[9], w[13]) QR(w[2], w[6], w[10], w[14]) QR(w[3], w[7], w[11], w[15])
        QR(w[0], w[5], w[10], w[15]) QR(w[1], w[6], w[11], w[12]) QR(w[2], w[7], w[8], w[13]) QR(w[3], w[4], w[9], w[14])
    }
    Fr lo, hi;
#pragma unroll
    for (int k = 0; k < 8; k++) {
        lo.v[k] = w[k] + s[k];
        hi.v[k] = w[8 + k] + s[8 + k];
    }
    const Fr r2 = Fr::r2();
    const Fr r3 = fe_mul(r2, r2);
    fe_store(out + i, fe_add(fe_mul(r2, lo), fe_mul(r3, hi)));
}
void launch_chacha_fr(const ChaChaKey& key, uint64_t start_block, Fr* out, uint32_t count, hipStream_t st) {
    hipLaunchKernelGGL(chacha_fr_kernel, dim3((count + 255) / 256), dim3(256), 0, st, key, start_block, out, count);
}

__global__ __launch_bounds__(1024) void scan_u32_kernel(const uint32_t* __restrict__ in, uint32_t* __restrict__ out, uint32_t m) {
    __shared__ uint32_t part[1024];
    const uint32_t chunk = (m + 1023) / 1024;
    const uint32_t lo = min(m, threadIdx.x * chunk), hi = min(m, lo + chunk);
    uint32_t sum = 0;
    for (uint32_t i = lo; i < hi; i++) sum += in[i];
    part[threadIdx.x] = sum;
    __syncthreads();
    for (uint32_t d = 1; d < 1024; d <<= 1) {
        const uint32_t v = (threadIdx.x >= d) ? part[threadIdx.x - d] : 0;
        __syncthreads();
        part[threadIdx.x] += v;
        __syncthreads();
    }
    uint32_t run = part[threadIdx.x] - sum;
    for (uint32_t i = lo; i < hi; i++) {
        const uint32_t h = in[i];
        out[i] = run;
        run += h;
    }
    if (threadIdx.x == 1023) out[m] = part[1023];
}
void launch_scan_u32(const uint32_t* in, uint32_t* out, uint32_t m, hipStream_t st) {
    hipLaunchKernelGGL(scan_u32_kernel, dim3(1), dim3(1024), 0, st, in, out, m);
}

__global__ __launch_bounds__(256) void lk_hist_kernel(LkPtrs ptrs, uint32_t usable, uint32_t T, uint32_t* __restrict__ hist0,
                                                      uint32_t stride, uint32_t* __restrict__ err) {
    const Fr* __restrict__ inp = ptrs.inp[blockIdx.y];
    uint32_t* __restrict__ hist = hist0 + (size_t)blockIdx.y * stride;
    const uint32_t i = blockIdx.x * blockDim.x + threadIdx.x;
    uint32_t val = 0xffffffffu;
    if (i < usable) {
        const Fr v = fe_from_mont(fe_load(inp + i));
        if (!lk_in_table(v, T)) atomicOr(err, 1u);
        else val = v.v[0];
    }
    const unsigned long long zmask = __ballot(val == 0);
    if (val == 0) {
        if ((threadIdx.x & 63) == (uint32_t)__ffsll((long long)zmask) - 1) atomicAdd(&hist[0], (uint32_t)__popcll(zmask));
    } else if (val != 0xffffffffu) {
        atomicAdd(&hist[val], 1u);
    }
}

__global__ void lk_flags_kernel(const uint32_t* __restrict__ hist0, uint32_t T, uint32_t* __restrict__ present0,
                                uint32_t* __restrict__ absent0, uint32_t stride) {
    const uint32_t* __restrict__ hist = hist0 + (size_t)blockIdx.y * stride;
    uint32_t* __restrict__ present = present0 + (size_t)blockIdx.y * stride;
    uint32_t* __restrict__ absent = absent0 + (size_t)blockIdx.y * stride;
    const uint32_t v = blockIdx.x * blockDim.x + threadIdx.x;
    if (v >= T) return;
    const uint32_t h = hist[v];
    present[v] = h > 0;
    absent[v] = (v >= 1 && h == 0);
}

__device__ __forceinline__ Fr small_to_mont(uint32_t v) {
    Fr a = Fr::zero();
    a.v[0] = v;
    return fe_to_mont(a);
}

__global__ void lk_fill_kernel(uint32_t usable, uint32_t T, const uint32_t* __restrict__ hist0,
                               const uint32_t* __restrict__ off0, const uint32_t* __restrict__ dex0,
                               const uint32_t* __restrict__ aex0, uint32_t stride, LkPtrs ptrs) {
    const uint32_t* __restrict__ hist = hist0 + (size_t)blockIdx.y * stride;
    const uint32_t* __restrict__ off = off0 + (size_t)blockIdx.y * stride;
    const uint32_t* __restrict__ dex = dex0 + (size_t)blockIdx.y * stride;
    const uint32_t* __restrict__ aex = aex0 + (size_t)blockIdx.y * stride;
    Fr* __restrict__ ap = ptrs.ap[blockIdx.y];
    Fr* __restrict__ sp = ptrs.sp[blockIdx.y];
    const uint32_t p = blockIdx.x * blockDim.x + threadIdx.x;
    if (p >= usable) return;
    uint32_t lo = 0, hi = T - 1;
    while (lo < hi) {
        const uint32_t mid = (lo + hi + 1) >> 1;
        if (off[mid] <= p) lo = mid; else hi = mid - 1;
    }
    const uint32_t v = lo;
    fe_store(ap + p, small_to_mont(v));
    if (p == off[v]) {
        fe_store(sp + p, small_to_mont(v));
        return;
    }
    const uint32_t D = dex[v] + 1;
    const uint32_t j = p - D;
    const uint32_t m = usable - dex[T];
    const uint32_t q = m - 1 - j;
    const uint32_t c0 = (usable - T + 1) - (hist[0] > 0 ? 1u : 0u);
    if (q < c0) {
        fe_store(sp + p, Fr::zero());
        return;
    }
    const uint32_t t = q - c0 + 1;
    uint32_t a = 1, b = T - 1;
    while (a < b) {
        const uint32_t mid = (a + b) >> 1;
        if (aex[mid + 1] >= t) b = mid; else a = mid + 1;
    }
    fe_store(sp + p, small_to_mont(a));
}

static constexpr uint32_t S3_BLOCK = 1024;

__global__ __launch_bounds__(256) void scan3_sums_kernel(const uint32_t* __restrict__ b0, const uint32_t* __restrict__ b1,
                                                         const uint32_t* __restrict__ b2, uint32_t m,
                                                         uint32_t* __restrict__ bsum0 , uint32_t nblocks,
                                                         uint32_t stride) {
    const uint32_t* __restrict__ a0 = b0 + (size_t)blockIdx.y * stride;
    const uint32_t* __restrict__ a1 = b1 + (size_t)blockIdx.y * stride;
    const uint32_t* __restrict__ a2 = b2 + (size_t)blockIdx.y * stride;
    uint32_t* __restrict__ bsum = bsum0 + (size_t)blockIdx.y * stride;
    __shared__ uint32_t sh[3][256];
    const uint32_t base = blockIdx.x * S3_BLOCK + threadIdx.x * 4;
    uint32_t s0 = 0, s1 = 0, s2 = 0;
    for (uint32_t k = 0; k < 4; k++)
        if (base + k < m) {
            s0 += a0[base + k];
            s1 += a1[base + k];
            s2 += a2[base + k];
        }
    sh[0][threadIdx.x] = s0;
    sh[1][threadIdx.x] = s1;
    sh[2][threadIdx.x] = s2;
    __syncthreads();
    for (uint32_t d = 128; d > 0; d >>= 1) {
        if (threadIdx.x < d)
            for (int q = 0; q < 3; q++) sh[q][threadIdx.x] += sh[q][threadIdx.x + d];
        __syncthreads();
    }
    if (threadIdx.x < 3) bsum[threadIdx.x * nblocks + blockIdx.x] = sh[threadIdx.x][0];
}

__global__ __launch_bounds__(1024) void scan3_top_kernel(uint32_t* __restrict__ bsum0, uint32_t nblocks, uint32_t stride) {
    uint32_t* __restrict__ bsum = bsum0 + (size_t)blockIdx.x * stride;
    __shared__ uint32_t part[1024];
    for (int q = 0; q < 3; q++) {
        uint32_t* row = bsum + q * nblocks;
        const uint32_t chunk = (nblocks + 1023) / 1024;
        const uint32_t lo = min(nblocks, threadIdx.x * chunk), hi = min(nblocks, lo + chunk);
        uint32_t sum = 0;
        for (uint32_t i = lo; i < hi; i++) sum += row[i];
        part[threadIdx.x] = sum;
        __syncthreads();
        for (uint32_t d = 1; d < 1024; d <<= 1) {
            const uint32_t v = (threadIdx.x >= d) ? part[threadIdx.x - d] : 0;
            __syncthreads();
            part[threadIdx.x] += v;
            __syncthreads();
        }
        uint32_t run = part[threadIdx.x] - sum;
        for (uint32_t i = lo; i < hi; i++) {
            const uint32_t h = row[i];
            row[i] = run;
            run += h;
        }
        __syncthreads();
    }
}

__global__ __launch_bounds__(256) void scan3_apply_kernel(const uint32_t* __restrict__ b0, const uint32_t* __restrict__ b1,
                                                          const uint32_t* __restrict__ b2, uint32_t m,
                                                          const uint32_t* __restrict__ bsum0, uint32_t nblocks,
                                                          uint32_t* __restrict__ p0, uint32_t* __restrict__ p1,
                                                          uint32_t* __restrict__ p2, uint32_t stride) {
    const size_t shift = (size_t)blockIdx.y * stride;
    const uint32_t* __restrict__ a0 = b0 + shift;
    const uint32_t* __restrict__ a1 = b1 + shift;
    const uint32_t* __restrict__ a2 = b2 + shift;
    const uint32_t* __restrict__ bsum = bsum0 + shift;
    uint32_t* __restrict__ o0 = p0 + shift;
    uint32_t* __restrict__ o1 = p1 + shift;
    uint32_t* __restrict__ o2 = p2 + shift;
    __shared__ uint32_t sh[3][256];
    const uint32_t base = blockIdx.x * S3_BLOCK + threadIdx.x * 4;
    uint32_t v[3][4];
    uint32_t s[3] = {0, 0, 0};
    for (uint32_t k = 0; k < 4; k++) {
        const bool in = base + k < m;
        v[0][k] = in ? a0[base + k] : 0;
        v[1][k] = in ? a1[base + k] : 0;
        v[2][k] = in ? a2[base + k] : 0;
        for (int q = 0; q < 3; q++) s[q] += v[q][k];
    }
    for (int q = 0; q < 3; q++) sh[q][threadIdx.x] = s[q];
    __syncthreads();
    for (uint32_t d = 1; d < 256; d <<= 1) {
        uint32_t t[3] = {0, 0, 0};
        if (threadIdx.x >= d)
            for (int q = 0; q < 3; q++) t[q] = sh[q][threadIdx.x - d];
        __syncthreads();
        for (int q = 0; q < 3; q++) sh[q][threadIdx.x] += t[q];
        __syncthreads();
    }
    const uint32_t* const ins[3] = {a0, a1, a2};
    (void)ins;
    uint32_t* const outs[3] = {o0, o1, o2};
    for (int q = 0; q < 3; q++) {
        uint32_t run = bsum[q * nblocks + blockIdx.x] + sh[q][threadIdx.x] - s[q];
        for (uint32_t k = 0; k < 4; k++) {
            if (base + k < m) outs[q][base + k] = run;
            run += v[q][k];
        }
        if (blockIdx.x == nblocks - 1 && threadIdx.x == 255) outs[q][m] = run;
    }
}

void launch_lookup_permute(const LkPtrs& ptrs, uint32_t count, uint32_t usable, uint32_t T, LookupScratch& s, hipStream_t st) {
    hipMemsetAsync(s.hist, 0, ((size_t)(count - 1) * s.stride + T + 1) * 4, st);
    hipLaunchKernelGGL(lk_hist_kernel, dim3((usable + 255) / 256, count), dim3(256), 0, st, ptrs, usable, T, s.hist, s.stride, s.err);
    hipLaunchKernelGGL(lk_flags_kernel, dim3((T + 255) / 256, count), dim3(256), 0, st, s.hist, T, s.present, s.absent, s.stride);
    const uint32_t nblocks = (T + S3_BLOCK - 1) / S3_BLOCK;
    hipLaunchKernelGGL(scan3_sums_kernel, dim3(nblocks, count), dim3(256), 0, st, s.hist, s.present, s.absent, T, s.bsum, nblocks,
                       s.stride);
    hipLaunchKernelGGL(scan3_top_kernel, dim3(count), dim3(1024), 0, st, s.bsum, nblocks, s.stride);
    hipLaunchKernelGGL(scan3_apply_kernel, dim3(nblocks, count), dim3(256), 0, st, s.hist, s.present, s.absent, T, s.bsum, nblocks,
                       s.off, s.dex, s.aex, s.stride);
    hipLaunchKernelGGL(lk_fill_kernel, dim3((usable + 255) / 256, count), dim3(256), 0, st, usable, T, s.hist, s.off, s.dex, s.aex,
                       s.stride, ptrs);
}


__global__ void perm_numden_kernel(PermArgs a) {
    const uint32_t i = blockIdx.x * blockDim.x + threadIdx.x;
    if (i >= a.n) return;
    const Fr wi_beta = fe_mul(fe_load(a.tw + i), a.beta);
    Fr num = Fr::one(), den = Fr::one();
    for (uint32_t c = 0; c < a.ncols; c++) {
        const Fr v = fe_load(a.values[c] + i);
        const Fr vg = fe_add(v, a.gamma);
        den = fe_mul(den, fe_add(vg, fe_mul(a.beta, fe_load(a.sigma[c] + i))));
        num = fe_mul(num, fe_add(vg, fe_mul(wi_beta, a.delta[c])));
    }
    fe_store(a.num + i, num);
    fe_store(a.den + i, den);
}
void launch_perm_numden(const PermArgs& a, hipStream_t st) {
    hipLaunchKernelGGL(perm_numden_kernel, dim3((a.n + 255) / 256), dim3(256), 0, st, a);
}
__global__ void perm_numden_batch_kernel(const PermArgs* __restrict__ args) {
    const PermArgs& a = args[blockIdx.y];
    const uint32_t i = blockIdx.x * blockDim.x + threadIdx.x;
    if (i >= a.n) return;
    const Fr beta = a.beta, gamma = a.gamma;
    const Fr wi_beta = fe_mul(fe_load(a.tw + i), beta);
    Fr num = Fr::one(), den = Fr::one();
    for (uint32_t c = 0; c < a.ncols; c++) {
        const Fr v = fe_load(a.values[c] + i);
        const Fr vg = fe_add(v, gamma);
        den = fe_mul(den, fe_add(vg, fe_mul(beta, fe_load(a.sigma[c] + i))));
        num = fe_mul(num, fe_add(vg, fe_mul(wi_beta, a.delta[c])));
    }
    fe_store(a.num + i, num);
    fe_store(a.den + i, den);
}
void launch_perm_numden_batch(const PermArgs* d_args, uint32_t count, uint32_t n, hipStream_t st) {
    hipLaunchKernelGGL(perm_numden_batch_kernel, dim3((n + 255) / 256, count), dim3(256), 0, st, d_args);
}
__global__ void lk_numden_batch_kernel(const LkNumDenArgs* __restrict__ args, Fr beta, Fr gamma, uint32_t n) {
    const LkNumDenArgs a = args[blockIdx.y];
    const uint32_t i = blockIdx.x * blockDim.x + threadIdx.x;
    if (i >= n) return;
    fe_store(a.den + i, fe_mul(fe_add(fe_load(a.ap + i), beta), fe_add(fe_load(a.sp + i), gamma)));
    fe_store(a.num + i, fe_mul(fe_add(fe_load(a.inp + i), beta), fe_add(fe_load(a.tab + i), gamma)));
}
void launch_lk_numden_batch(const LkNumDenArgs* d_args, uint32_t count, const Fr& beta, const Fr& gamma, uint32_t n, hipStream_t st) {
    hipLaunchKernelGGL(lk_numden_batch_kernel, dim3((n + 255) / 256, count), dim3(256), 0, st, d_args, beta, gamma, n);
}
__global__ void copy_columns_kernel(const CopyPair* __restrict__ pairs, uint32_t n) {
    const CopyPair p = pairs[blockIdx.y];
    const uint32_t i = blockIdx.x * blockDim.x + threadIdx.x;
    if (i < n) fe_store(p.dst + i, fe_load(p.src + i));
}
void launch_copy_columns(const CopyPair* d_pairs, uint32_t count, uint32_t n, hipStream_t st) {
    hipLaunchKernelGGL(copy_columns_kernel, dim3((n + 255) / 256, count), dim3(256), 0, st, d_pairs, n);
}

__global__ void lk_numden_kernel(const Fr* ap, const Fr* sp, const Fr* inp, const Fr* tab, Fr beta, Fr gamma, Fr* num,
                                 Fr* den, uint32_t n) {
    const uint32_t i = blockIdx.x * blockDim.x + threadIdx.x;
    if (i >= n) return;
    fe_store(den + i, fe_mul(fe_add(fe_load(ap + i), beta), fe_add(fe_load(sp + i), gamma)));
    fe_store(num + i, fe_mul(fe_add(fe_load(inp + i), beta), fe_add(fe_load(tab + i), gamma)));
}
void launch_lk_numden(const Fr* ap, const Fr* sp, const Fr* inp, const Fr* tab, const Fr& beta, const Fr& gamma, Fr* num,
                      Fr* den, uint32_t n, hipStream_t st) {
    hipLaunchKernelGGL(lk_numden_kernel, dim3((n + 255) / 256), dim3(256), 0, st, ap, sp, inp, tab, beta, gamma, num, den, n);
}

__global__ void frac_kernel(const Fr* __restrict__ num, const Fr* __restrict__ den, Fr* __restrict__ frac, uint32_t n) {
    constexpr int E = 16;
    const uint32_t base = (blockIdx.x * blockDim.x + threadIdx.x) * E;
    if (base >= n) return;
    Fr d[E], pre[E];
    Fr acc = Fr::one();
#pragma unroll
    for (int k = 0; k < E; k++) {
        d[k] = (base + k < n) ? fe_load(den + base + k) : Fr::one();
        pre[k] = acc;
        if (!d[k].is_zero()) acc = fe_mul(acc, d[k]);
    }
    Fr inv = fe_inv(acc);
#pragma unroll
    for (int k = E - 1; k >= 0; k--) {
        if (base + k < n) {
            Fr r = Fr::zero();
            if (!d[k].is_zero()) {
                r = fe_mul(inv, pre[k]);
                inv = fe_mul(inv, d[k]);
            }
            fe_store(frac + base + k, fe_mul(r, fe_load(num + base + k)));
        }
    }
}
void launch_frac(const Fr* num, const Fr* den, Fr* frac, uint32_t n, hipStream_t st) {
    const uint32_t threads = (n + 15) / 16;
    hipLaunchKernelGGL(frac_kernel, dim3((threads + 63) / 64), dim3(64), 0, st, num, den, frac, n);
}

static constexpr uint32_t PP_E = 8, PP_T = 256, PP_B = PP_E * PP_T;

__global__ __launch_bounds__(PP_T) void pp_local_kernel(const Fr* __restrict__ f, Fr* __restrict__ local, Fr* __restrict__ tot, uint32_t n) {
    __shared__ Fr sh[PP_T];
    const uint32_t base = blockIdx.x * PP_B + threadIdx.x * PP_E;
    Fr v[PP_E];
    Fr acc = Fr::one();
#pragma unroll
    for (uint32_t k = 0; k < PP_E; k++) {
        if (base + k < n) acc = fe_mul(acc, fe_load(f + base + k));
        v[k] = acc;
    }
    sh[threadIdx.x] = acc;
    __syncthreads();
    for (uint32_t d = 1; d < PP_T; d <<= 1) {
        Fr o = Fr::one();
        const bool has = threadIdx.x >= d;
        if (has) o = sh[threadIdx.x - d];
        __syncthreads();
        if (has) sh[threadIdx.x] = fe_mul(sh[threadIdx.x], o);
        __syncthreads();
    }
    const Fr excl = threadIdx.x ? sh[threadIdx.x - 1] : Fr::one();
#pragma unroll
    for (uint32_t k = 0; k < PP_E; k++)
        if (base + k < n) fe_store(local + base + k, fe_mul(v[k], excl));
    if (threadIdx.x == PP_T - 1) fe_store(tot + blockIdx.x, sh[PP_T - 1]);
}

__global__ __launch_bounds__(1024) void pp_offsets_kernel(Fr* __restrict__ tot, uint32_t nblocks, const Fr* __restrict__ init_ptr, Fr init_val) {
    __shared__ Fr sh[1024];
    const Fr init = init_ptr ? fe_load(init_ptr) : init_val;
    const uint32_t chunk = (nblocks + 1023) / 1024;
    const uint32_t lo = min(nblocks, threadIdx.x * chunk), hi = min(nblocks, lo + chunk);
    Fr acc = Fr::one();
    for (uint32_t i = lo; i < hi; i++) acc = fe_mul(acc, fe_load(tot + i));
    sh[threadIdx.x] = acc;
    __syncthreads();
    for (uint32_t d = 1; d < 1024; d <<= 1) {
        Fr o = Fr::one();
        const bool has = threadIdx.x >= d;
        if (has) o = sh[threadIdx.x - d];
        __syncthreads();
        if (has) sh[threadIdx.x] = fe_mul(sh[threadIdx.x], o);
        __syncthreads();
    }
    Fr run = fe_mul(init, threadIdx.x ? sh[threadIdx.x - 1] : Fr::one());
    for (uint32_t i = lo; i < hi; i++) {
        const Fr t = fe_load(tot + i);
        fe_store(tot + i, run);
        run = fe_mul(run, t);
    }
}

__global__ __launch_bounds__(PP_T) void pp_apply_kernel(const Fr* __restrict__ local, const Fr* __restrict__ offs, Fr* __restrict__ z, uint32_t n) {
    const uint32_t i = blockIdx.x * PP_T + threadIdx.x;
    if (i >= n) return;
    const Fr off = fe_load(offs + i / PP_B);
    if (i == 0) fe_store(z, off);
    if (i + 1 < n) fe_store(z + i + 1, fe_mul(off, fe_load(local + i)));
}

void launch_prefix_product(const Fr* f, Fr* z, uint32_t n, const Fr* init_dev, const Fr& init_val, Fr* tmp_local, Fr* tmp_tot, hipStream_t st) {
    const uint32_t nblocks = (n + PP_B - 1) / PP_B;
    hipLaunchKernelGGL(pp_local_kernel, dim3(nblocks), dim3(PP_T), 0, st, f, tmp_local, tmp_tot, n);
    hipLaunchKernelGGL(pp_offsets_kernel, dim3(1), dim3(1024), 0, st, tmp_tot, nblocks, init_dev, init_val);
    hipLaunchKernelGGL(pp_apply_kernel, dim3((n + PP_T - 1) / PP_T), dim3(PP_T), 0, st, tmp_local, tmp_tot, z, n);
}

__global__ __launch_bounds__(PP_T) void gp_local_batch_kernel(const GpItem* __restrict__ items, uint32_t n) {
    const GpItem it = items[blockIdx.y];
    __shared__ Fr shp[PP_T], shr[PP_T];
    const uint32_t base = blockIdx.x * PP_B + threadIdx.x * PP_E;
    Fr v[PP_E], w[PP_E];
    Fr acc = Fr::one();
#pragma unroll
    for (uint32_t k = 0; k < PP_E; k++) {
        if (base + k < n) acc = fe_mul(acc, fe_load(it.num + base + k));
        v[k] = acc;
    }
    shp[threadIdx.x] = acc;
    acc = Fr::one();
#pragma unroll
    for (int k = PP_E - 1; k >= 0; k--) {
        if (base + k < n) acc = fe_mul(acc, fe_load(it.den + base + k));
        w[k] = acc;
    }
    shr[threadIdx.x] = acc;
    __syncthreads();
#pragma unroll 1
    for (uint32_t d = 1; d < PP_T; d <<= 1) {
        Fr op = Fr::one(), orr = Fr::one();
        const bool hp = threadIdx.x >= d, hr = threadIdx.x + d < PP_T;
        if (hp) op = shp[threadIdx.x - d];
        if (hr) orr = shr[threadIdx.x + d];
        __syncthreads();
        if (hp) shp[threadIdx.x] = fe_mul(shp[threadIdx.x], op);
        if (hr) shr[threadIdx.x] = fe_mul(shr[threadIdx.x], orr);
        __syncthreads();
    }
    const Fr ep = threadIdx.x ? shp[threadIdx.x - 1] : Fr::one();
    const Fr er = threadIdx.x + 1 < PP_T ? shr[threadIdx.x + 1] : Fr::one();
#pragma unroll
    for (uint32_t k = 0; k < PP_E; k++)
        if (base + k < n) {
            fe_store(it.loc_p + base + k, fe_mul(v[k], ep));
            fe_store(it.loc_r + base + k, fe_mul(w[k], er));
        }
    if (threadIdx.x == PP_T - 1) fe_store(it.tot_p + blockIdx.x, shp[PP_T - 1]);
    if (threadIdx.x == 0) fe_store(it.tot_r + blockIdx.x, shr[0]);
}

__global__ __launch_bounds__(256) void gp_offsets_batch_kernel(const GpItem* __restrict__ items, uint32_t nblocks,
                                                               Fr* __restrict__ q_out) {
    const GpItem it = items[blockIdx.x];
    __shared__ Fr shp[256], shr[256];
    const uint32_t chunk = (nblocks + 255) / 256;
    const uint32_t lo = min(nblocks, threadIdx.x * chunk), hi = min(nblocks, lo + chunk);
    Fr ap = Fr::one(), ar = Fr::one();
    for (uint32_t i = lo; i < hi; i++) {
        ap = fe_mul(ap, fe_load(it.tot_p + i));
        ar = fe_mul(ar, fe_load(it.tot_r + i));
    }
    shp[threadIdx.x] = ap;
    shr[threadIdx.x] = ar;
    __syncthreads();
#pragma unroll 1
    for (uint32_t d = 1; d < 256; d <<= 1) {
        Fr op = Fr::one(), orr = Fr::one();
        const bool hp = threadIdx.x >= d, hr = threadIdx.x + d < 256;
        if (hp) op = shp[threadIdx.x - d];
        if (hr) orr = shr[threadIdx.x + d];
        __syncthreads();
        if (hp) shp[threadIdx.x] = fe_mul(shp[threadIdx.x], op);
        if (hr) shr[threadIdx.x] = fe_mul(shr[threadIdx.x], orr);
        __syncthreads();
    }
    if (threadIdx.x == 0) fe_store(q_out + blockIdx.x, shr[0]);
    Fr run = threadIdx.x ? shp[threadIdx.x - 1] : Fr::one();
    for (uint32_t i = lo; i < hi; i++) {
        const Fr t = fe_load(it.tot_p + i);
        fe_store(it.tot_p + i, run);
        run = fe_mul(run, t);
    }
    run = threadIdx.x + 1 < 256 ? shr[threadIdx.x + 1] : Fr::one();
    for (uint32_t i = hi; i-- > lo;) {
        const Fr t = fe_load(it.tot_r + i);
        fe_store(it.tot_r + i, run);
        run = fe_mul(run, t);
    }
}

__global__ __launch_bounds__(256) void gp_chain_kernel(const GpItem* __restrict__ items, const Fr* __restrict__ q_inv, uint32_t nprod,
                                                       uint32_t row, Fr* __restrict__ kout, Fr* __restrict__ init_out) {
    __shared__ Fr sh[256];
    __shared__ uint32_t head[256];
    const uint32_t p = threadIdx.x;
    Fr v = Fr::one(), qi = Fr::one();
    bool chained_next = false;
    bool is_head = true;
    if (p < nprod) {
        const GpItem it = items[p];
        qi = fe_load(q_inv + p);
        is_head = p == 0 || !it.chain;
        chained_next = p + 1 < nprod && items[p + 1].chain;
        if (chained_next) {
            const Fr pfx = fe_mul(fe_load(it.tot_p + (row - 1) / PP_B), fe_load(it.loc_p + row - 1));
            const Fr sfx = fe_mul(fe_load(it.tot_r + row / PP_B), fe_load(it.loc_r + row));
            v = fe_mul(qi, fe_mul(pfx, sfx));
        }
    }
    sh[p] = v;
    head[p] = is_head ? 1u : 0u;
    __syncthreads();
#pragma unroll 1
    for (uint32_t d = 1; d < 256; d <<= 1) {
        Fr o = Fr::one();
        uint32_t oh = 0;
        const bool has = p >= d && !head[p];
        if (p >= d) oh = head[p - d];
        if (has) o = sh[p - d];
        __syncthreads();
        if (has) {
            sh[p] = fe_mul(sh[p], o);
            head[p] = oh;
        }
        __syncthreads();
    }
    if (p < nprod) {
        const Fr init = (p && items[p].chain) ? sh[p - 1] : Fr::one();
        fe_store(init_out + p, init);
        fe_store(kout + p, fe_mul(init, qi));
    }
}

__global__ __launch_bounds__(PP_T) void gp_apply_batch_kernel(const GpItem* __restrict__ items, const Fr* __restrict__ kk,
                                                              const Fr* __restrict__ init, uint32_t n) {
    const GpItem it = items[blockIdx.y];
    const uint32_t i = blockIdx.x * PP_T + threadIdx.x;
    if (i >= n) return;
    if (i == 0) fe_store(it.z, fe_load(init + blockIdx.y));
    if (i + 1 >= n) return;
    const Fr pfx = fe_mul(fe_mul(fe_load(it.tot_p + i / PP_B), fe_load(kk + blockIdx.y)), fe_load(it.loc_p + i));
    const Fr sfx = fe_mul(fe_load(it.tot_r + (i + 1) / PP_B), fe_load(it.loc_r + i + 1));
    fe_store(it.z + i + 1, fe_mul(pfx, sfx));
}

uint32_t gp_blocks(uint32_t n) { return (n + PP_B - 1) / PP_B; }

void launch_gp_batch_scan(const GpItem* d_items, uint32_t nprod, uint32_t n, Fr* q_dev, hipStream_t st) {
    const uint32_t nblocks = gp_blocks(n);
    hipLaunchKernelGGL(gp_local_batch_kernel, dim3(nblocks, nprod), dim3(PP_T), 0, st, d_items, n);
    hipLaunchKernelGGL(gp_offsets_batch_kernel, dim3(nprod), dim3(256), 0, st, d_items, nblocks, q_dev);
}
void launch_gp_batch_apply(const GpItem* d_items, uint32_t nprod, uint32_t n, uint32_t chain_row, const Fr* q_inv_dev, Fr* k_dev,
                           Fr* init_dev, hipStream_t st) {
    hipLaunchKernelGGL(gp_chain_kernel, dim3(1), dim3(256), 0, st, d_items, q_inv_dev, nprod, chain_row, k_dev, init_dev);
    hipLaunchKernelGGL(gp_apply_batch_kernel, dim3((n + PP_T - 1) / PP_T, nprod), dim3(PP_T), 0, st, d_items, k_dev, init_dev, n);
}

__global__ __launch_bounds__(64) void scatter_rows_kernel(const RowEntry* __restrict__ e) {
    const RowEntry* r = e + blockIdx.x;
    if (threadIdx.x < r->count) fe_store(r->dst + threadIdx.x, fe_load(r->vals + threadIdx.x));
}
void launch_scatter_rows(const RowEntry* d_entries, uint32_t count, hipStream_t st) {
    hipLaunchKernelGGL(scatter_rows_kernel, dim3(count), dim3(64), 0, st, d_entries);
}

#ifndef ZK_KD_L
#define ZK_KD_L 8
#endif
static constexpr uint32_t KD_L_MIN = ZK_KD_L;
static constexpr uint32_t KD_BLK = 256;
static constexpr uint32_t KD_TOP = 1024;
__host__ __device__ inline uint32_t kd_len(uint32_t n) {
    uint32_t L = KD_L_MIN;
    while (((n + L - 1) / L + KD_BLK - 1) / KD_BLK > KD_TOP) L <<= 1;
    return L;
}

struct KdPtrs {
    const Fr* p[KD_MAX_BATCH];
    Fr* q[KD_MAX_BATCH];
    Fr z[KD_MAX_BATCH];
};
struct KdStep {
    Fr step[KD_MAX_BATCH][8];
};
struct KdTop {
    Fr top[KD_MAX_BATCH][10];
};

__host__ __device__ inline uint32_t kd_scratch_elems(uint32_t n) {
    const uint32_t L = kd_len(n), m = (n + L - 1) / L, nblk = (m + KD_BLK - 1) / KD_BLK;
    return 2 * m + 2 * nblk + 256;
}
uint32_t kate_division_scratch(uint32_t n) { return kd_scratch_elems(n); }

__global__ __launch_bounds__(KD_BLK) void kd_scan_kernel(KdPtrs a, KdStep pw, KdTop tw, uint32_t n, Fr* __restrict__ scratch) {
    __shared__ Fr sh[KD_BLK];
    const uint32_t KD_L = kd_len(n);
    const uint32_t m = (n + KD_L - 1) / KD_L, nblk = (m + KD_BLK - 1) / KD_BLK;
    Fr* suf = scratch + (size_t)blockIdx.y * kd_scratch_elems(n) + m;
    Fr* agg = suf + m;
    Fr* tpow = agg + nblk;
    Fr* zpow = tpow + nblk;
    if (blockIdx.x >= nblk) {
        const bool top = blockIdx.x > nblk;
        const uint32_t e0 = top ? (blockIdx.x - nblk - 1) * KD_BLK + threadIdx.x : threadIdx.x;
        if (top && e0 >= nblk) return;
        Fr acc = Fr::one();
        if (top) {
            for (uint32_t e = e0, j = 0; e; e >>= 1, j++)
                if (e & 1) acc = fe_mul(acc, tw.top[blockIdx.y][j]);
            fe_store(tpow + e0, acc);
        } else {
            for (uint32_t e = e0, j = 0; e; e >>= 1, j++)
                if (e & 1) acc = fe_mul(acc, pw.step[blockIdx.y][j]);
            fe_store(zpow + e0, acc);
        }
        return;
    }
    const uint32_t t = blockIdx.x * KD_BLK + threadIdx.x;
    Fr v = Fr::zero();
    {
        const uint32_t base = t * KD_L;
        if (base < n) {
            const Fr* __restrict__ p = a.p[blockIdx.y];
            const Fr z = a.z[blockIdx.y];
            const uint32_t top = min(n, base + KD_L);
            for (uint32_t i = top; i-- > base;) v = fe_add(fe_mul(v, z), fe_load(p + i));
        }
    }
    sh[threadIdx.x] = v;
    __syncthreads();
#pragma unroll 1
    for (uint32_t j = 0, d = 1; d < KD_BLK; d <<= 1, j++) {
        Fr o = Fr::zero();
        const bool has = threadIdx.x + d < KD_BLK;
        if (has) o = sh[threadIdx.x + d];
        __syncthreads();
        if (has) {
            v = fe_add(v, fe_mul(o, pw.step[blockIdx.y][j]));
            sh[threadIdx.x] = v;
        }
        __syncthreads();
    }
    if (t < m) fe_store(suf + t, v);
    if (threadIdx.x == 0) fe_store(agg + blockIdx.x, v);
}

__global__ __launch_bounds__(KD_BLK) void kd_apply_kernel(KdPtrs a, uint32_t n, Fr* __restrict__ scratch) {
    __shared__ Fr sh[KD_BLK];
    const uint32_t KD_L = kd_len(n);
    const uint32_t m = (n + KD_L - 1) / KD_L, nblk = (m + KD_BLK - 1) / KD_BLK;
    const Fr* suf = scratch + (size_t)blockIdx.y * kd_scratch_elems(n) + m;
    const Fr* agg = suf + m;
    const Fr* tpow = agg + nblk;
    const Fr* zpow = tpow + nblk;
    const uint32_t blk = blockIdx.x;
    Fr g = Fr::zero();
    for (uint32_t b = blk + 1 + threadIdx.x; b < nblk; b += KD_BLK) g = fe_add(g, fe_mul(fe_load(agg + b), fe_load(tpow + (b - blk - 1))));
    sh[threadIdx.x] = g;
    __syncthreads();
    for (uint32_t d = KD_BLK / 2; d; d >>= 1) {
        if (threadIdx.x < d) sh[threadIdx.x] = fe_add(sh[threadIdx.x], sh[threadIdx.x + d]);
        __syncthreads();
    }
    const Fr G = sh[0];
    const uint32_t t = blk * KD_BLK + threadIdx.x;
    const uint32_t base = t * KD_L;
    if (base >= n) return;
    const Fr* __restrict__ p = a.p[blockIdx.y];
    Fr* __restrict__ q = a.q[blockIdx.y];
    const Fr z = a.z[blockIdx.y];
    const uint32_t top = min(n, base + KD_L);
    const uint32_t last = min(m, (blk + 1) * KD_BLK) - 1;
    Fr run = (t < last) ? fe_load(suf + t + 1) : Fr::zero();
    run = fe_add(run, fe_mul(fe_load(zpow + (last - t)), G));
    for (uint32_t i = top; i-- > base;) {
        const Fr pi = fe_load(p + i);
        fe_store(q + i, run);
        run = fe_add(fe_mul(run, z), pi);
    }
}

void launch_kate_division_batch(const Fr* const* p, Fr* const* q, const Fr* z, uint32_t count, uint32_t n, Fr* scratch,
                                hipStream_t st) {
    const uint32_t KD_L = kd_len(n);
    const uint32_t m = (n + KD_L - 1) / KD_L;
    const uint32_t nblk = (m + KD_BLK - 1) / KD_BLK;
    KdPtrs pt;
    KdStep stp;
    KdTop tp;
    memset(&pt, 0, sizeof(pt));
    memset(&stp, 0, sizeof(stp));
    memset(&tp, 0, sizeof(tp));
    for (uint32_t b = 0; b < count; b++) {
        pt.p[b] = p[b];
        pt.q[b] = q[b];
        pt.z[b] = z[b];
        Fr Z = z[b];
        for (uint32_t i = 1; i < KD_L; i <<= 1) Z = fe_sqr(Z);
        Fr cur = Z;
        for (int j = 0; j < 8; j++) {
            stp.step[b][j] = cur;
            cur = fe_sqr(cur);
        }
        for (int j = 0; j < 10; j++) {
            tp.top[b][j] = cur;
            cur = fe_sqr(cur);
        }
    }
    hipLaunchKernelGGL(kd_scan_kernel, dim3(nblk + 1 + (nblk + KD_BLK - 1) / KD_BLK, count), dim3(KD_BLK), 0, st, pt, stp, tp, n, scratch);
    hipLaunchKernelGGL(kd_apply_kernel, dim3(nblk, count), dim3(KD_BLK), 0, st, pt, n, scratch);
}

void launch_kate_division(const Fr* p, Fr* q, uint32_t n, const Fr& z, Fr* scratch, hipStream_t st) {
    launch_kate_division_batch(&p, &q, &z, 1, n, scratch, st);
}

}
```

webauthn-halo2_amd/engine.py:

```python
import ctypes
import os

import numpy as np

_HERE = os.path.dirname(os.path.abspath(__file__))
_LIB = None

ZK_BASIS_MONOMIAL = 0
ZK_BASIS_LAGRANGE = 1
ZK_T_MSM, ZK_T_NTT, ZK_T_QUOTIENT, ZK_T_EVAL, ZK_T_MSM_ACCUM, ZK_T_MSM_COLUMNS, ZK_T_MSM_TAIL_MAIN, ZK_T_MSM_TAIL = 0, 1, 2, 3, 4, 5, 6, 7


ZK_TRANSCRIPT_BLAKE2B, ZK_TRANSCRIPT_EVM = 0, 1
ZK_SERDE_PROCESSED, ZK_SERDE_RAW_BYTES, ZK_SERDE_RAW_BYTES_UNCHECKED = 0, 1, 2
ZK_OPT_MSM_WINDOW, ZK_OPT_MSM_BATCH, ZK_OPT_NTT_MAX_RADIX_LOG2, ZK_OPT_GP_BATCH_INVERT, ZK_OPT_MSM_TAIL_STREAM = 1, 2, 3, 4, 5
ZK_OPT_MSM_TAIL_MAIN_ABOVE, ZK_OPT_BATCH_PASS_COLUMNS, ZK_OPT_XFORM_STREAM, ZK_OPT_MSM_STREAM, ZK_OPT_MSM_T1, ZK_OPT_STREAM_AUDIT = 6, 7, 8, 9, 10, 11
ZK_OPT_STREAM_PRIORITY, ZK_OPT_QUOTIENT_DOMAIN, ZK_OPT_ACTIVITY_HOLD = 12, 13, 14
ZK_SCHEME_DEFAULT, ZK_SCHEME_GWC, ZK_SCHEME_SHPLONK = 0, 1, 2
ZK_VERIFY_BATCH_MAX = 1024
ZK_SRS_CHECK_POWERS, ZK_SRS_CHECK_LAGRANGE, ZK_SRS_CHECK_GENERATORS = 1, 2, 4
ZK_SRS_CONTRIB_SAME_SECRET, ZK_SRS_CONTRIB_LINKS, ZK_SRS_CONTRIB_NONTRIVIAL, ZK_SRS_CONTRIB_RESIDENT = 1, 2, 4, 8
ZK_FAIL_GATE, ZK_FAIL_GATE_BLINDED, ZK_FAIL_LOOKUP, ZK_FAIL_COPY = 1, 2, 3, 4
ZK_PK_FIXED_POLY, ZK_PK_SIGMA_POLY = 0, 1
(ZK_PK_PART_FIXED_COMMIT, ZK_PK_PART_SIGMA_COMMIT, ZK_PK_PART_FIXED_POLY, ZK_PK_PART_SIGMA_POLY, ZK_PK_PART_FIXED_COSET,
 ZK_PK_PART_SIGMA_COSET, ZK_PK_PART_L_COSET, ZK_PK_PART_SIGMA_LABEL, ZK_PK_PART_SIGMA_MAP) = range(1, 10)
ZK_PK_CHECK_COMMITMENTS, ZK_PK_CHECK_POLYS, ZK_PK_CHECK_COSETS, ZK_PK_CHECK_SIGMA, ZK_PK_CHECK_ALL, ZK_PK_CHECK_REPR = 1, 2, 4, 8, 15, 16
ZK_PLACEMENT_MAINS_OK, ZK_PLACEMENT_LONE_OK, ZK_PLACEMENT_PAIR_OK, ZK_PLACEMENT_LAYER1_OK, ZK_PLACEMENT_OK = 1, 2, 4, 8, 15
ZK_PLACEMENT_CALIBRATED, ZK_PLACEMENT_UNRESOLVED = 16, 32


def device_pci_bus_id(device=0):
    buf = ctypes.create_string_buffer(32)
    rc = load_library().zk_device_pci_bus_id(device, buf, len(buf))
    if rc:
        raise ZkError(rc, "zk_device_pci_bus_id")
    return buf.value.decode().lower()


def device_mem_info(device=0):
    free, total = ctypes.c_size_t(0), ctypes.c_size_t(0)
    rc = load_library().zk_device_mem_info(device, ctypes.byref(free), ctypes.byref(total))
    if rc:
        raise ZkError(rc, "zk_device_mem_info")
    return free.value, total.value


def stream_placement(device=0, calibrate=False) -> dict:
    r = PlacementC()
    rc = load_library().zk_stream_placement(device, 1 if calibrate else 0, ctypes.byref(r))
    if rc:
        raise ZkError(rc, "zk_stream_placement")
    f = r.flags
    return {"n_queues": r.n_queues, "flags": f, "ok": f & ZK_PLACEMENT_OK == ZK_PLACEMENT_OK,
            "mains_ok": bool(f & ZK_PLACEMENT_MAINS_OK), "lone_ok": bool(f & ZK_PLACEMENT_LONE_OK),
            "pair_ok": bool(f & ZK_PLACEMENT_PAIR_OK), "layer1_ok": bool(f & ZK_PLACEMENT_LAYER1_OK),
            "calibrated": bool(f & ZK_PLACEMENT_CALIBRATED), "unresolved": bool(f & ZK_PLACEMENT_UNRESOLVED),
            "main_queue": list(r.main_queue), "role_queue": [list(row) for row in r.role_queue], "spare_queue": list(r.spare_queue),
            "rounds": r.rounds, "streams": r.streams, "probe_ms": r.probe_ms}


class PinnedArray:

    def __init__(self, shape, dtype=np.uint64):
        self.L = load_library()
        nbytes = int(np.prod(shape)) * np.dtype(dtype).itemsize
        self.ptr = self.L.zk_host_alloc(nbytes)
        if not self.ptr:
            raise ZkError(-2, "zk_host_alloc")
        self.a = np.frombuffer((ctypes.c_uint8 * nbytes).from_address(self.ptr), dtype=dtype).reshape(shape)

    def free(self):
        if self.ptr:
            self.a = None
            self.L.zk_host_free(self.ptr)
            self.ptr = None

    def __del__(self):
        try:
            self.free()
        except Exception:
            pass


class CircuitParamsC(ctypes.Structure):
    _fields_ = [("k", ctypes.c_uint32), ("num_advice", ctypes.c_uint32), ("num_lookup_advice", ctypes.c_uint32),
                ("num_fixed", ctypes.c_uint32), ("lookup_bits", ctypes.c_uint32),
                ("num_idle_gate_columns", ctypes.c_uint32)]


class WitnessFailureC(ctypes.Structure):
    _fields_ = [("kind", ctypes.c_uint32), ("index", ctypes.c_uint32), ("row", ctypes.c_uint32), ("other_index", ctypes.c_uint32),
                ("other_row", ctypes.c_uint32), ("reserved", ctypes.c_uint32)]

# ... 646 lines not shown
```

Before: 102.9.

## Move eval, grand-product and Kate division kernels to 29-bit limbs; adapt MSM t1 mode

```diff
diff --git a/include/zkmi355.h b/include/zkmi355.h
--- a/include/zkmi355.h
+++ b/include/zkmi355.h
@@ -212,7 +212,9 @@
 #define ZK_T_MSM_COLUMNS 5
 #define ZK_T_MSM_TAIL_MAIN 6
 #define ZK_T_MSM_TAIL 7
-#define ZK_T_COUNT 8
+#define ZK_T_MSM_T1_PARTS 8
+#define ZK_T_MSM_T1_BUCKET 9
+#define ZK_T_COUNT 10
 int zk_last_kernel_ms(zk_ctx* ctx, int which, float* out_ms);
 int zk_audit_report(zk_ctx* ctx, uint64_t counts[2], char* msg, size_t cap);
 int zk_timer_reset(zk_ctx* ctx);
diff --git a/webauthn-halo2_amd/csrc/ctx.h b/webauthn-halo2_amd/csrc/ctx.h
--- a/webauthn-halo2_amd/csrc/ctx.h
+++ b/webauthn-halo2_amd/csrc/ctx.h
@@ -75,6 +75,7 @@
     bool msm_side = false;
     uint32_t opt_msm_stream = 0;
     uint32_t opt_msm_t1 = 0;
+    uint32_t proof_regime = 0;
     hipStream_t xform_stream = nullptr;
     hipEvent_t ev_rows = nullptr, ev_xform = nullptr;
     bool xform_pending = false;
diff --git a/webauthn-halo2_amd/csrc/engine.h b/webauthn-halo2_amd/csrc/engine.h
--- a/webauthn-halo2_amd/csrc/engine.h
+++ b/webauthn-halo2_amd/csrc/engine.h
@@ -50,7 +50,8 @@
 size_t msm_ws_max_n(const MsmWorkspace* ws);
 uint32_t msm_ws_max_batch(const MsmWorkspace* ws);
 uint32_t msm_ws_window(const MsmWorkspace* ws);
-void msm_ws_set_t1_mode(MsmWorkspace* ws, uint32_t mode);
+void msm_ws_set_t1_mode(MsmWorkspace* ws, uint32_t mode, bool loaded);
+int msm_ws_last_t1_form(const MsmWorkspace* ws);
 bool msm_ws_last_pass_wide(const MsmWorkspace* ws);
 hipError_t msm_build_table(const G1Affine* bases, uint32_t n, uint32_t c, G1Affine* table, hipStream_t st);
 bool msm_table_is_internal(uint32_t c, size_t n);
diff --git a/webauthn-halo2_amd/csrc/engine.hip b/webauthn-halo2_amd/csrc/engine.hip
--- a/webauthn-halo2_amd/csrc/engine.hip
+++ b/webauthn-halo2_amd/csrc/engine.hip
@@ -7,11 +7,11 @@
 
 #include "ctx.h"
 #include "placement.h"
+#include "prover.h"
 
 namespace zk {
 placement::Classes placement_probe(const hipStream_t* streams, int n, placement::Stamp* stamps);
 uint32_t eval_blocks(uint32_t n);
-void launch_eval(const Fr* c, uint32_t n, const Fr& x, Fr* scratch, hipStream_t st);
 void launch_srs_lagrange_scalars(const Fr* tw, uint32_t n, const Fr& s, const Fr& c, Fr* out, hipStream_t st);
 void launch_srs_fixed_base(const Fr* scalars, uint32_t n, const G1Affine* table, G1Affine* out, hipStream_t st);
 
@@ -358,7 +358,7 @@
     }
     c->stream_counts[L.tail == c->stream ? 0 : 1]++;
     HIPCHK(c, aud_record(c, L.t_head[0], hs));
-    msm_ws_set_t1_mode(ws, c->opt_msm_t1);
+    msm_ws_set_t1_mode(ws, c->opt_msm_t1, c->proof_regime ? c->proof_regime == 2 : tail_on_main);
     HIPCHK(c, msm_run(ws, d_scalars, batch, d_bases, n, hs, L.host_buf, &L.nwin, &L.cw, L.t_acc, table, stride, L.tail,
                       L.head_done, !table || ident));
     if (c->audit.on) {
@@ -375,6 +375,7 @@
     HIPCHK(c, aud_record(c, L.tail_done, L.tail));
     HIPCHK(c, aud_record(c, L.t_head[1], hs));
     c->msm_launches++;
+    if (msm_ws_last_t1_form(ws) >= 0) c->acc_n[msm_ws_last_t1_form(ws) ? ZK_T_MSM_T1_BUCKET : ZK_T_MSM_T1_PARTS]++;
     L.n = n;
     L.batch = batch;
     L.table = table;
@@ -1688,9 +1689,14 @@
     if (rc) return rc;
     Fr xx;
     memcpy(&xx, x, 32);
+    static_assert(sizeof(EvalItem) <= 24 * sizeof(Fr), "the item's place in c->small");
     const uint32_t blocks = eval_blocks((uint32_t)r->n);
+    EvalItem item;
+    memset(&item, 0, sizeof(item));
+    item.poly = r->ptr;
+    item.x = xx;
     aud_record(c, c->ev[ZK_T_EVAL][0], c->stream);
-    launch_eval(r->ptr, (uint32_t)r->n, xx, c->small, c->stream);
+    launch_eval_batch(&item, reinterpret_cast<EvalItem*>(c->small + 1032), 1, (uint32_t)r->n, c->small, c->small + blocks, c->stream);
     aud_record(c, c->ev[ZK_T_EVAL][1], c->stream);
     c->ev_valid[ZK_T_EVAL] = true;
     HIPCHK(c, hipMemcpyAsync(c->host_small, c->small + blocks, sizeof(Fr), hipMemcpyDeviceToHost, c->stream));
diff --git a/webauthn-halo2_amd/csrc/field29.hip.h b/webauthn-halo2_amd/csrc/field29.hip.h
--- a/webauthn-halo2_amd/csrc/field29.hip.h
+++ b/webauthn-halo2_amd/csrc/field29.hip.h
@@ -357,6 +357,55 @@
         c = t >> 29;
     }
     r.l[8] = a.l[8] + c;
+    return r;
+}
+
+template <class PRM>
+__device__ __forceinline__ Fe<PRM> reduce_canonical(const Fe29<PRM>& a) {
+    constexpr uint32_t P8 = Lim29<PRM>::P[8];
+    constexpr uint64_t M = ((uint64_t)1 << 53) / (P8 + 1);
+    static_assert(M < ((uint64_t)1 << 32), "M must fit a word");
+    const uint32_t qe = (uint32_t)(((uint64_t)a.l[8] * (uint32_t)M) >> 53);
+    Fe29<PRM> r;
+    int64_t acc = 0;
+#pragma unroll
+    for (int i = 0; i < 8; i++) {
+        acc += (int64_t)a.l[i] - (int64_t)((uint64_t)qe * Lim29<PRM>::P[i]);
+        r.l[i] = (uint32_t)acc & M29;
+        acc >>= 29;
+    }
+    acc += (int64_t)a.l[8] - (int64_t)((uint64_t)qe * Lim29<PRM>::P[8]);
+    r.l[8] = (uint32_t)acc;
+    Fe<PRM> o = from29(r);
+    reduce_once(o);
+    return o;
+}
+
+template <class PRM>
+__device__ __forceinline__ Fe<PRM> canon_lt2p(const Fe29<PRM>& a) {
+    Fe<PRM> r = from29(a);
+    reduce_once(r);
+    return r;
+}
+
+
+template <int STRIDE, class PRM>
+__device__ __forceinline__ Fe29<PRM> lds29_load(const uint32_t* sh, uint32_t t) {
+    Fe29<PRM> r;
+#pragma unroll
+    for (int i = 0; i < 9; i++) r.l[i] = sh[i * STRIDE + t];
+    return r;
+}
+template <int STRIDE, class PRM>
+__device__ __forceinline__ void lds29_store(uint32_t* sh, uint32_t t, const Fe29<PRM>& a) {
+#pragma unroll
+    for (int i = 0; i < 9; i++) sh[i * STRIDE + t] = a.l[i];
+}
+template <class PRM>
+__device__ __forceinline__ Fe29<PRM> zero29() {
+    Fe29<PRM> r;
+#pragma unroll
+    for (int i = 0; i < 9; i++) r.l[i] = 0;
     return r;
 }
 
diff --git a/webauthn-halo2_amd/csrc/msm.hip b/webauthn-halo2_amd/csrc/msm.hip
--- a/webauthn-halo2_amd/csrc/msm.hip
+++ b/webauthn-halo2_amd/csrc/msm.hip
@@ -71,6 +71,8 @@
     bool wide;
     bool w_redo_valid;
     uint32_t w_t1_mode;
+    bool w_t1_loaded;
+    int w_last_t1;
     bool w_last_wide;
     bool w_clean;
     uint32_t* w_tot[2];
@@ -132,7 +134,11 @@
 size_t msm_ws_max_n(const MsmWorkspace* ws) { return ws->max_n; }
 uint32_t msm_ws_max_batch(const MsmWorkspace* ws) { return ws->max_batch; }
 uint32_t msm_ws_window(const MsmWorkspace* ws) { return ws->c; }
-void msm_ws_set_t1_mode(MsmWorkspace* ws, uint32_t mode) { ws->w_t1_mode = mode; }
+void msm_ws_set_t1_mode(MsmWorkspace* ws, uint32_t mode, bool loaded) {
+    ws->w_t1_mode = mode;
+    ws->w_t1_loaded = loaded;
+}
+int msm_ws_last_t1_form(const MsmWorkspace* ws) { return ws->w_last_t1; }
 bool msm_ws_last_pass_wide(const MsmWorkspace* ws) { return ws->w_last_wide; }
 
 #include "msm_legacy.hip.h"
@@ -346,7 +352,8 @@
     if (accum_events && accum_events[2]) hipEventRecord(accum_events[2], ts);
     if (n > 0) {
         const uint32_t max_parts = (lanes + 2 * nb) / WCAP + nb + 2 * g.bins + 64;
-        const bool per_bucket = ws->w_t1_mode == 1;
+        const bool per_bucket = ws->w_t1_mode == 1 || (ws->w_t1_mode == 0 && ws->w_t1_loaded && batch >= 2);
+        ws->w_last_t1 = per_bucket ? 1 : 0;
         uint32_t lmin = 0;
         if (per_bucket) {
             lmin = ZK_T1B_LMAX;
@@ -412,6 +419,7 @@
     const bool fixed = table != nullptr;
     ws->w_redo_valid = false;
     ws->w_last_wide = fixed && ws->wide && table_stride == ws->max_n;
+    ws->w_last_t1 = -1;
     if (fixed && ws->wide && table_stride == ws->max_n)
         return msm_run_wide(ws, scalars_list, batch, n, st, host_window_sums, nwin_out, c_out, accum_events, table, table_stride, tail_st,
                             head_done, bases_may_be_identity);
diff --git a/webauthn-halo2_amd/csrc/ntt.hip b/webauthn-halo2_amd/csrc/ntt.hip
--- a/webauthn-halo2_amd/csrc/ntt.hip
+++ b/webauthn-halo2_amd/csrc/ntt.hip
@@ -92,26 +92,6 @@
     acc += (int64_t)a.l[8] - (int64_t)((uint64_t)m * Lim29<FrParams>::P[8]);
     r.l[8] = (uint32_t)acc;
     return r;
-}
-
-__device__ __forceinline__ Fr reduce_canonical(const Fr29& a) {
-    constexpr uint32_t P8 = Lim29<FrParams>::P[8];
-    constexpr uint64_t M = ((uint64_t)1 << 53) / (P8 + 1);
-    static_assert(M < ((uint64_t)1 << 32), "M must fit a word");
-    const uint32_t qe = (uint32_t)(((uint64_t)a.l[8] * (uint32_t)M) >> 53);
-    Fr29 r;
-    int64_t acc = 0;
-#pragma unroll
-    for (int i = 0; i < 8; i++) {
-        acc += (int64_t)a.l[i] - (int64_t)((uint64_t)qe * Lim29<FrParams>::P[i]);
-        r.l[i] = (uint32_t)acc & M29;
-        acc >>= 29;
-    }
-    acc += (int64_t)a.l[8] - (int64_t)((uint64_t)qe * Lim29<FrParams>::P[8]);
-    r.l[8] = (uint32_t)acc;
-    Fr o = from29(r);
-    reduce_once(o);
-    return o;
 }
 
 template <int E = 29>
diff --git a/webauthn-halo2_amd/csrc/poly.hip b/webauthn-halo2_amd/csrc/poly.hip
--- a/webauthn-halo2_amd/csrc/poly.hip
+++ b/webauthn-halo2_amd/csrc/poly.hip
@@ -1,48 +1,10 @@
 #include "engine.h"
 #include "prover.h"
+#include "field29.hip.h"
+#include "hostutil.h"
 #include <string.h>
 
 namespace zk {
-
-__global__ __launch_bounds__(256) void poly_eval_partial_kernel(const Fr* __restrict__ c, uint32_t n, Fr x, Fr y,
-                                                                Fr* __restrict__ block_out) {
-    __shared__ Fr sh[256];
-    const uint32_t S = gridDim.x * 256;
-    const uint32_t t = blockIdx.x * 256 + threadIdx.x;
-    Fr acc = Fr::zero();
-    if (t < n) {
-        uint32_t m = (n - 1 - t) / S;
-        acc = fe_load(c + t + m * S);
-        while (m-- > 0) acc = fe_add(fe_mul(acc, y), fe_load(c + t + m * S));
-        Fr xp = Fr::one();
-        Fr base = x;
-        for (uint32_t e = t; e; e >>= 1) {
-            if (e & 1) xp = fe_mul(xp, base);
-            base = fe_sqr(base);
-        }
-        acc = fe_mul(acc, xp);
-    }
-    sh[threadIdx.x] = acc;
-    __syncthreads();
-    for (uint32_t s = 128; s > 0; s >>= 1) {
-        if (threadIdx.x < s) sh[threadIdx.x] = fe_add(sh[threadIdx.x], sh[threadIdx.x + s]);
-        __syncthreads();
-    }
-    if (threadIdx.x == 0) fe_store(block_out + blockIdx.x, sh[0]);
-}
-
-__global__ __launch_bounds__(256) void poly_sum_kernel(const Fr* __restrict__ in, uint32_t m, Fr* __restrict__ out) {
-    __shared__ Fr sh[256];
-    Fr acc = Fr::zero();
-    for (uint32_t i = threadIdx.x; i < m; i += 256) acc = fe_add(acc, fe_load(in + i));
-    sh[threadIdx.x] = acc;
-    __syncthreads();
-    for (uint32_t s = 128; s > 0; s >>= 1) {
-        if (threadIdx.x < s) sh[threadIdx.x] = fe_add(sh[threadIdx.x], sh[threadIdx.x + s]);
-        __syncthreads();
-    }
-    if (threadIdx.x == 0) fe_store(out, sh[0]);
-}
 
 uint32_t eval_blocks(uint32_t n) {
     uint32_t b = (n + 256 * 16 - 1) / (256 * 16);
@@ -51,75 +13,67 @@
     return b;
 }
 
-void launch_eval(const Fr* c, uint32_t n, const Fr& x, Fr* scratch, hipStream_t st) {
-    const uint32_t blocks = eval_blocks(n);
-    const uint32_t S = blocks * 256;
-    Fr y = Fr::one(), base = x;
-    for (uint32_t e = S; e; e >>= 1) {
-        if (e & 1) y = fe_mul(y, base);
-        base = fe_sqr(base);
-    }
-    hipLaunchKernelGGL(poly_eval_partial_kernel, dim3(blocks), dim3(256), 0, st, c, n, x, y, scratch);
-    hipLaunchKernelGGL(poly_sum_kernel, dim3(1), dim3(256), 0, st, scratch, blocks, scratch + blocks);
-}
-
-__global__ __launch_bounds__(256) void poly_eval_batch_kernel(const EvalItem* __restrict__ items, uint32_t n, uint32_t M,
-                                                              Fr* __restrict__ block_out) {
-    __shared__ Fr sh[256];
-    const uint32_t e = blockIdx.y;
-    const Fr* __restrict__ c = items[e].poly;
-    const Fr y = items[e].y;
-    const uint32_t base = blockIdx.x * 256 * M + threadIdx.x;
-    Fr acc = Fr::zero();
-#pragma unroll 1
-    for (uint32_t m = M; m-- > 0;) {
-        const uint32_t idx = base + 256 * m;
-        if (idx < n) {
-            const Fr v = fe_load(c + idx);
-            acc = fe_add(fe_mul(acc, y), v);
-        }
-    }
-    sh[threadIdx.x] = acc;
+typedef Fe29<FrParams> Fr29;
+__device__ __forceinline__ Fr29 fold256(uint32_t* sh, Fr29 acc, uint32_t live, const Fr* __restrict__ pw32) {
+    acc = norm29(acc);
+    lds29_store<256>(sh, threadIdx.x, acc);
     __syncthreads();
-    const uint32_t live = min(256u, n - min(n, blockIdx.x * 256 * M));
 #pragma unroll 1
     for (int l = 7; l >= 0; l--) {
         const uint32_t s = 1u << l;
         if (s >= live) continue;
-        if (threadIdx.x < s) sh[threadIdx.x] = fe_add(sh[threadIdx.x], fe_mul(sh[threadIdx.x + s], items[e].pw[l]));
+        if (threadIdx.x < s) {
+            acc = norm29(add29(acc, mul29(lds29_load<256, FrParams>(sh, threadIdx.x + s), to29(pw32[l]))));
+            lds29_store<256>(sh, threadIdx.x, acc);
+        }
         __syncthreads();
     }
-    if (threadIdx.x == 0) fe_store(block_out + e * gridDim.x + blockIdx.x, sh[0]);
+    return acc;
+}
+
+__global__ __launch_bounds__(256) void poly_eval_batch_kernel(const EvalItem* __restrict__ items, uint32_t n, uint32_t M,
+                                                              Fr* __restrict__ block_out) {
+    __shared__ uint32_t sh[256 * 9];
+    const uint32_t e = blockIdx.y;
+    const Fr* __restrict__ c = items[e].poly;
+    const Fr29 y = to29(items[e].y);
+    const uint32_t base = blockIdx.x * 256 * M + threadIdx.x;
+    Fr29 acc = base + 256 * (M - 1) < n ? to29(fe_load(c + base + 256 * (M - 1))) : zero29<FrParams>();
+#pragma unroll 1
+    for (uint32_t m = M - 1; m-- > 0;) {
+        const uint32_t idx = base + 256 * m;
+        if (idx < n) {
+            const Fr29 v = to29(fe_load(c + idx));
+            acc = add29(mul29(acc, y), v);
+        }
+    }
+    const uint32_t live = min(256u, n - min(n, blockIdx.x * 256 * M));
+    acc = fold256(sh, acc, live, items[e].pw);
+    if (threadIdx.x == 0) fe_store(block_out + e * gridDim.x + blockIdx.x, reduce_canonical(acc));
 }
 
 __global__ __launch_bounds__(256) void poly_sum_batch_kernel(const EvalItem* __restrict__ items, const Fr* __restrict__ in, uint32_t m,
                                                              Fr* __restrict__ out) {
-    __shared__ Fr sh[256];
+    __shared__ uint32_t sh[256 * 9];
     const uint32_t e = blockIdx.x;
     const Fr* src = in + (size_t)e * m;
-    Fr acc = Fr::zero();
+    const Fr29 y = to29(items[e].zpw[8]);
+    Fr29 acc = zero29<FrParams>();
 #pragma unroll 1
     for (uint32_t q = (m + 255) / 256; q-- > 0;) {
         const uint32_t idx = threadIdx.x + 256 * q;
-        if (idx < m) acc = fe_add(fe_mul(acc, items[e].zpw[8]), fe_load(src + idx));
-    }
-    sh[threadIdx.x] = acc;
-    __syncthreads();
-#pragma unroll 1
-    for (int l = 7; l >= 0; l--) {
-        const uint32_t s = 1u << l;
-        if (s >= m) continue;
-        if (threadIdx.x < s) sh[threadIdx.x] = fe_add(sh[threadIdx.x], fe_mul(sh[threadIdx.x + s], items[e].zpw[l]));
-        __syncthreads();
-    }
-    if (threadIdx.x == 0) fe_store(out + e, sh[0]);
+        if (idx < m) acc = add29(mul29(acc, y), to29(fe_load(src + idx)));
+    }
+    acc = fold256(sh, acc, m, items[e].zpw);
+    if (threadIdx.x == 0) fe_store(out + e, reduce_canonical(acc));
 }
 
 void launch_eval_batch(EvalItem* h_items, EvalItem* d_items, uint32_t count, uint32_t n, Fr* scratch, Fr* out,
                        hipStream_t st) {
     const uint32_t blocks = eval_blocks(n);
-    const uint32_t M = (n + blocks * 256 - 1) / (blocks * 256);
+    const uint32_t M = n ? (n + blocks * 256 - 1) / (blocks * 256) : 1;
     uint32_t distinct[16], nd = 0;
+    const Fr k32 = fr_from_u64(32);
     for (uint32_t e = 0; e < count; e++) {
         EvalItem& it = h_items[e];
         uint32_t same = count;
@@ -143,6 +97,9 @@
         }
         it.zpw[0] = z;
         for (int l = 1; l < 9; l++) it.zpw[l] = fe_sqr(it.zpw[l - 1]);
+        for (int l = 0; l < 8; l++) it.pw[l] = fe_mul(it.pw[l], k32);
+        it.y = fe_mul(it.y, k32);
+        for (int l = 0; l < 9; l++) it.zpw[l] = fe_mul(it.zpw[l], k32);
     }
     hipMemcpyAsync(d_items, h_items, (size_t)count * sizeof(EvalItem), hipMemcpyHostToDevice, st);
     hipLaunchKernelGGL(poly_eval_batch_kernel, dim3(blocks, count), dim3(256), 0, st, d_items, n, M, scratch);
diff --git a/webauthn-halo2_amd/csrc/prover.hip b/webauthn-halo2_amd/csrc/prover.hip
--- a/webauthn-halo2_amd/csrc/prover.hip
+++ b/webauthn-halo2_amd/csrc/prover.hip
@@ -1115,6 +1115,7 @@
         {
             const uint32_t above = c->opt_tail_main_above ? c->opt_tail_main_above : 2u;
             loaded = c->opt_tail_stream == 2 || (c->opt_tail_stream == 0 && (uint32_t)ctx_activity_touch(c) > above);
+            c->proof_regime = loaded ? 2u : 1u;
         }
         cosets3 = lay.n_h == 3 && 3 <= ctx_ntt_max_batch(lay.k) &&
                   (c->opt_quotient_domain == 2 || (c->opt_quotient_domain == 0 && lay.k >= 16));
@@ -1720,6 +1721,7 @@
             c->xform_pending = false;
         }
         aud_sync(c, c->stream);
+        c->proof_regime = 0;
         ctx_activity_hold(c, false);
     }
     ~ProveQuiesce() { settle(); }
diff --git a/webauthn-halo2_amd/csrc/prover_kernels.hip b/webauthn-halo2_amd/csrc/prover_kernels.hip
--- a/webauthn-halo2_amd/csrc/prover_kernels.hip
+++ b/webauthn-halo2_amd/csrc/prover_kernels.hip
@@ -1,4 +1,6 @@
 #include <string.h>
+
+#include <utility>
 
 #include "prover.h"
 #include "field29.hip.h"
@@ -6,10 +8,17 @@
 
 namespace zk {
 
+typedef Fe29<FrParams> Fr29;
+template <class F, uint32_t... K>
+__device__ __forceinline__ void unrolled(F&& f, std::integer_sequence<uint32_t, K...>) {
+    (f(std::integral_constant<uint32_t, K>{}), ...);
+}
+__device__ __forceinline__ Fr mul_mem(const Fr& a, const Fr& b) { return canon_lt2p(mul29(to29_x32(a), to29(b))); }
+
 
 __global__ void to_mont_kernel(Fr* a, uint32_t n) {
     const uint32_t i = blockIdx.x * blockDim.x + threadIdx.x;
-    if (i < n) fe_store(a + i, fe_to_mont(fe_load(a + i)));
+    if (i < n) fe_store(a + i, canon_lt2p(mul29(to29(fe_load(a + i)), const_pow2_29<517, FrParams>())));
 }
 void launch_to_mont(Fr* a, uint32_t n, hipStream_t st) {
     hipLaunchKernelGGL(to_mont_kernel, dim3((n + 255) / 256), dim3(256), 0, st, a, n);
@@ -24,7 +33,6 @@
 }
 
 __global__ __launch_bounds__(256) void lincomb_kernel(LincombArgs a) {
-    typedef Fe29<FrParams> Fr29;
     const uint32_t i = blockIdx.x * blockDim.x + threadIdx.x;
     if (i >= a.n) return;
     Fr29 zero;
@@ -64,7 +72,6 @@
 
 __global__ __launch_bounds__(256) void lincomb_terms_kernel(const LcTerm* __restrict__ terms, uint32_t count, Fr* __restrict__ out,
                                                             uint32_t log_ns, uint32_t sub0, Fr sub0_val, uint32_t low_n, LcLow low) {
-    typedef Fe29<FrParams> Fr29;
     __shared__ uint32_t part[256 * 9];
     const uint32_t ns = 1u << log_ns, rows = 256u >> log_ns;
     const uint32_t row = threadIdx.x & (rows - 1), sl = threadIdx.x >> (8 - log_ns);
@@ -124,7 +131,7 @@
 
 __global__ void scale_kernel(Fr* a, Fr c, uint32_t n) {
     const uint32_t i = blockIdx.x * blockDim.x + threadIdx.x;
-    if (i < n) fe_store(a + i, fe_mul(fe_load(a + i), c));
+    if (i < n) fe_store(a + i, mul_mem(fe_load(a + i), c));
 }
 void launch_scale(Fr* a, const Fr& c, uint32_t n, hipStream_t st) {
     hipLaunchKernelGGL(scale_kernel, dim3((n + 255) / 256), dim3(256), 0, st, a, c, n);
@@ -162,9 +169,9 @@
         lo.v[k] = w[k] + s[k];
         hi.v[k] = w[8 + k] + s[8 + k];
     }
-    const Fr r2 = Fr::r2();
-    const Fr r3 = fe_mul(r2, r2);
-    fe_store(out + i, fe_add(fe_mul(r2, lo), fe_mul(r3, hi)));
+    const Fr29 v[2] = {to29(lo), to29(hi)};
+    const Fr29 k[2] = {const_pow2_29<517, FrParams>(), const_pow2_29<773, FrParams>()};
+    fe_store(out + i, canon_lt2p(mulKadd29<2>(v, k)));
 }
 void launch_chacha_fr(const ChaChaKey& key, uint64_t start_block, Fr* out, uint32_t count, hipStream_t st) {
     hipLaunchKernelGGL(chacha_fr_kernel, dim3((count + 255) / 256), dim3(256), 0, st, key, start_block, out, count);
@@ -228,9 +235,10 @@
 }
 
 __device__ __forceinline__ Fr small_to_mont(uint32_t v) {
-    Fr a = Fr::zero();
-    a.v[0] = v;
-    return fe_to_mont(a);
+    Fr29 a = zero29<FrParams>();
+    a.l[0] = v & M29;
+    a.l[1] = v >> 29;
+    return canon_lt2p(mul29(a, const_pow2_29<517, FrParams>()));
 }
 
 __global__ void lk_fill_kernel(uint32_t usable, uint32_t T, const uint32_t* __restrict__ hist0,
@@ -393,48 +401,46 @@
 }
 
 
-__global__ void perm_numden_kernel(PermArgs a) {
+__device__ __forceinline__ void perm_numden_row(const PermArgs& a, uint32_t i, const Fr29& beta_i) {
+    const Fr29 gamma_i = to29_x32(a.gamma);
+    const Fr29 wi_beta = mul29(to29_x32(fe_load(a.tw + i)), beta_i);
+    Fr29 num = const_pow2_29<256, FrParams>(), den = num;
+    for (uint32_t c = 0; c < a.ncols; c++) {
+        const Fr29 vg = add29(to29_x32(fe_load(a.values[c] + i)), gamma_i);
+        const Fr29 fd = add29(vg, mul29(to29_x32(fe_load(a.sigma[c] + i)), beta_i));
+        const Fr29 fn = add29(vg, mul29(wi_beta, to29_x32(a.delta[c])));
+        den = mul29(den, fd);
+        num = mul29(num, fn);
+    }
+    fe_store(a.num + i, canon_lt2p(num));
+    fe_store(a.den + i, canon_lt2p(den));
+}
+__global__ void perm_numden_kernel(PermArgs a, Fr beta32) {
     const uint32_t i = blockIdx.x * blockDim.x + threadIdx.x;
     if (i >= a.n) return;
-    const Fr wi_beta = fe_mul(fe_load(a.tw + i), a.beta);
-    Fr num = Fr::one(), den = Fr::one();
-    for (uint32_t c = 0; c < a.ncols; c++) {
-        const Fr v = fe_load(a.values[c] + i);
-        const Fr vg = fe_add(v, a.gamma);
-        den = fe_mul(den, fe_add(vg, fe_mul(a.beta, fe_load(a.sigma[c] + i))));
-        num = fe_mul(num, fe_add(vg, fe_mul(wi_beta, a.delta[c])));
-    }
-    fe_store(a.num + i, num);
-    fe_store(a.den + i, den);
+    perm_numden_row(a, i, to29(beta32));
 }
 void launch_perm_numden(const PermArgs& a, hipStream_t st) {
-    hipLaunchKernelGGL(perm_numden_kernel, dim3((a.n + 255) / 256), dim3(256), 0, st, a);
+    hipLaunchKernelGGL(perm_numden_kernel, dim3((a.n + 255) / 256), dim3(256), 0, st, a, fe_mul(a.beta, fr_from_u64(32)));
 }
 __global__ void perm_numden_batch_kernel(const PermArgs* __restrict__ args) {
     const PermArgs& a = args[blockIdx.y];
     const uint32_t i = blockIdx.x * blockDim.x + threadIdx.x;
     if (i >= a.n) return;
-    const Fr beta = a.beta, gamma = a.gamma;
-    const Fr wi_beta = fe_mul(fe_load(a.tw + i), beta);
-    Fr num = Fr::one(), den = Fr::one();
-    for (uint32_t c = 0; c < a.ncols; c++) {
-        const Fr v = fe_load(a.values[c] + i);
-        const Fr vg = fe_add(v, gamma);
-        den = fe_mul(den, fe_add(vg, fe_mul(beta, fe_load(a.sigma[c] + i))));
-        num = fe_mul(num, fe_add(vg, fe_mul(wi_beta, a.delta[c])));
-    }
-    fe_store(a.num + i, num);
-    fe_store(a.den + i, den);
+    perm_numden_row(a, i, std_to_internal(a.beta));
 }
 void launch_perm_numden_batch(const PermArgs* d_args, uint32_t count, uint32_t n, hipStream_t st) {
     hipLaunchKernelGGL(perm_numden_batch_kernel, dim3((n + 255) / 256, count), dim3(256), 0, st, d_args);
 }
+__device__ __forceinline__ Fr lk_factor(const Fr& x, const Fr& beta, const Fr& y, const Fr& gamma) {
+    return canon_lt2p(mul29(add29(to29_x32(x), to29_x32(beta)), add29(to29(y), to29(gamma))));
+}
 __global__ void lk_numden_batch_kernel(const LkNumDenArgs* __restrict__ args, Fr beta, Fr gamma, uint32_t n) {
     const LkNumDenArgs a = args[blockIdx.y];
     const uint32_t i = blockIdx.x * blockDim.x + threadIdx.x;
     if (i >= n) return;
-    fe_store(a.den + i, fe_mul(fe_add(fe_load(a.ap + i), beta), fe_add(fe_load(a.sp + i), gamma)));
-    fe_store(a.num + i, fe_mul(fe_add(fe_load(a.inp + i), beta), fe_add(fe_load(a.tab + i), gamma)));
+    fe_store(a.den + i, lk_factor(fe_load(a.ap + i), beta, fe_load(a.sp + i), gamma));
+    fe_store(a.num + i, lk_factor(fe_load(a.inp + i), beta, fe_load(a.tab + i), gamma));
 }
 void launch_lk_numden_batch(const LkNumDenArgs* d_args, uint32_t count, const Fr& beta, const Fr& gamma, uint32_t n, hipStream_t st) {
     hipLaunchKernelGGL(lk_numden_batch_kernel, dim3((n + 255) / 256, count), dim3(256), 0, st, d_args, beta, gamma, n);
@@ -452,8 +458,8 @@
                                  Fr* den, uint32_t n) {
     const uint32_t i = blockIdx.x * blockDim.x + threadIdx.x;
     if (i >= n) return;
-    fe_store(den + i, fe_mul(fe_add(fe_load(ap + i), beta), fe_add(fe_load(sp + i), gamma)));
-    fe_store(num + i, fe_mul(fe_add(fe_load(inp + i), beta), fe_add(fe_load(tab + i), gamma)));
+    fe_store(den + i, lk_factor(fe_load(ap + i), beta, fe_load(sp + i), gamma));
+    fe_store(num + i, lk_factor(fe_load(inp + i), beta, fe_load(tab + i), gamma));
 }
 void launch_lk_numden(const Fr* ap, const Fr* sp, const Fr* inp, const Fr* tab, const Fr& beta, const Fr& gamma, Fr* num,
                       Fr* den, uint32_t n, hipStream_t st) {
@@ -561,45 +567,62 @@
 
 __global__ __launch_bounds__(PP_T) void gp_local_batch_kernel(const GpItem* __restrict__ items, uint32_t n) {
     const GpItem it = items[blockIdx.y];
-    __shared__ Fr shp[PP_T], shr[PP_T];
+    __shared__ uint32_t shp[PP_T * 9], shr[PP_T * 9];
     const uint32_t base = blockIdx.x * PP_B + threadIdx.x * PP_E;
-    Fr v[PP_E], w[PP_E];
-    Fr acc = Fr::one();
+    const Fr29 to_i = const_pow2_29<266, FrParams>();
+    Fr29 v[PP_E], w[PP_E];
+    Fr29 acc = const_pow2_29<256, FrParams>();
 #pragma unroll
     for (uint32_t k = 0; k < PP_E; k++) {
-        if (base + k < n) acc = fe_mul(acc, fe_load(it.num + base + k));
+        if (base + k < n) {
+            const Fr x = fe_load(it.num + base + k);
+            acc = k == 0 ? to29(x) : mul29(acc, to29_x32(x));
+        }
         v[k] = acc;
     }
-    shp[threadIdx.x] = acc;
-    acc = Fr::one();
+    Fr29 P = mul29(acc, to_i);
+    lds29_store<PP_T>(shp, threadIdx.x, P);
+    acc = const_pow2_29<256, FrParams>();
 #pragma unroll
     for (int k = PP_E - 1; k >= 0; k--) {
-        if (base + k < n) acc = fe_mul(acc, fe_load(it.den + base + k));
+        if (base + k < n) {
+            const Fr x = fe_load(it.den + base + k);
+            acc = k == (int)PP_E - 1 ? to29(x) : mul29(acc, to29_x32(x));
+        }
         w[k] = acc;
     }
-    shr[threadIdx.x] = acc;
+    Fr29 R = mul29(acc, to_i);
+    lds29_store<PP_T>(shr, threadIdx.x, R);
     __syncthreads();
 #pragma unroll 1
     for (uint32_t d = 1; d < PP_T; d <<= 1) {
-        Fr op = Fr::one(), orr = Fr::one();
+        Fr29 op, orr;
         const bool hp = threadIdx.x >= d, hr = threadIdx.x + d < PP_T;
-        if (hp) op = shp[threadIdx.x - d];
-        if (hr) orr = shr[threadIdx.x + d];
-        __syncthreads();
-        if (hp) shp[threadIdx.x] = fe_mul(shp[threadIdx.x], op);
-        if (hr) shr[threadIdx.x] = fe_mul(shr[threadIdx.x], orr);
-        __syncthreads();
-    }
-    const Fr ep = threadIdx.x ? shp[threadIdx.x - 1] : Fr::one();
-    const Fr er = threadIdx.x + 1 < PP_T ? shr[threadIdx.x + 1] : Fr::one();
-#pragma unroll
-    for (uint32_t k = 0; k < PP_E; k++)
+        if (hp) op = lds29_load<PP_T, FrParams>(shp, threadIdx.x - d);
+        if (hr) orr = lds29_load<PP_T, FrParams>(shr, threadIdx.x + d);
+        __syncthreads();
+        if (hp) {
+            P = mul29(P, op);
+            lds29_store<PP_T>(shp, threadIdx.x, P);
+        }
+        if (hr) {
+            R = mul29(R, orr);
+            lds29_store<PP_T>(shr, threadIdx.x, R);
+        }
+        __syncthreads();
+    }
+    const Fr29 one_i = const_pow2_29<261, FrParams>();
+    const Fr29 ep = threadIdx.x ? lds29_load<PP_T, FrParams>(shp, threadIdx.x - 1) : one_i;
+    const Fr29 er = threadIdx.x + 1 < PP_T ? lds29_load<PP_T, FrParams>(shr, threadIdx.x + 1) : one_i;
+    unrolled([&](auto K) {
+        constexpr uint32_t k = decltype(K)::value;
         if (base + k < n) {
-            fe_store(it.loc_p + base + k, fe_mul(v[k], ep));
-            fe_store(it.loc_r + base + k, fe_mul(w[k], er));
-        }
-    if (threadIdx.x == PP_T - 1) fe_store(it.tot_p + blockIdx.x, shp[PP_T - 1]);
-    if (threadIdx.x == 0) fe_store(it.tot_r + blockIdx.x, shr[0]);
+            fe_store(it.loc_p + base + k, canon_lt2p(mul29(v[k], ep)));
+            fe_store(it.loc_r + base + k, canon_lt2p(mul29(w[k], er)));
+        }
+    }, std::make_integer_sequence<uint32_t, PP_E>{});
+    if (threadIdx.x == PP_T - 1) fe_store(it.tot_p + blockIdx.x, internal_to_std(P));
+    if (threadIdx.x == 0) fe_store(it.tot_r + blockIdx.x, internal_to_std(R));
 }
 
 __global__ __launch_bounds__(256) void gp_offsets_batch_kernel(const GpItem* __restrict__ items, uint32_t nblocks,
@@ -692,9 +715,11 @@
     if (i >= n) return;
     if (i == 0) fe_store(it.z, fe_load(init + blockIdx.y));
     if (i + 1 >= n) return;
-    const Fr pfx = fe_mul(fe_mul(fe_load(it.tot_p + i / PP_B), fe_load(kk + blockIdx.y)), fe_load(it.loc_p + i));
-    const Fr sfx = fe_mul(fe_load(it.tot_r + (i + 1) / PP_B), fe_load(it.loc_r + i + 1));
-    fe_store(it.z + i + 1, fe_mul(pfx, sfx));
+    Fr29 z = mul29(to29_x32(fe_load(it.tot_p + i / PP_B)), to29(fe_load(kk + blockIdx.y)));
+    z = mul29(z, to29_x32(fe_load(it.loc_p + i)));
+    z = mul29(z, to29_x32(fe_load(it.tot_r + (i + 1) / PP_B)));
+    z = mul29(z, to29_x32(fe_load(it.loc_r + i + 1)));
+    fe_store(it.z + i + 1, canon_lt2p(z));
 }
 
 uint32_t gp_blocks(uint32_t n) { return (n + PP_B - 1) / PP_B; }
@@ -749,7 +774,7 @@
 uint32_t kate_division_scratch(uint32_t n) { return kd_scratch_elems(n); }
 
 __global__ __launch_bounds__(KD_BLK) void kd_scan_kernel(KdPtrs a, KdStep pw, KdTop tw, uint32_t n, Fr* __restrict__ scratch) {
-    __shared__ Fr sh[KD_BLK];
+    __shared__ uint32_t sh[KD_BLK * 9];
     const uint32_t KD_L = kd_len(n);
     const uint32_t m = (n + KD_L - 1) / KD_L, nblk = (m + KD_BLK - 1) / KD_BLK;
     Fr* suf = scratch + (size_t)blockIdx.y * kd_scratch_elems(n) + m;
@@ -760,45 +785,48 @@
         const bool top = blockIdx.x > nblk;
         const uint32_t e0 = top ? (blockIdx.x - nblk - 1) * KD_BLK + threadIdx.x : threadIdx.x;
         if (top && e0 >= nblk) return;
-        Fr acc = Fr::one();
+        Fr29 acc = const_pow2_29<256, FrParams>();
         if (top) {
             for (uint32_t e = e0, j = 0; e; e >>= 1, j++)
-                if (e & 1) acc = fe_mul(acc, tw.top[blockIdx.y][j]);
-            fe_store(tpow + e0, acc);
+                if (e & 1) acc = mul29(acc, to29(tw.top[blockIdx.y][j]));
+            fe_store(tpow + e0, canon_lt2p(acc));
         } else {
             for (uint32_t e = e0, j = 0; e; e >>= 1, j++)
-                if (e & 1) acc = fe_mul(acc, pw.step[blockIdx.y][j]);
-            fe_store(zpow + e0, acc);
+                if (e & 1) acc = mul29(acc, to29(pw.step[blockIdx.y][j]));
+            fe_store(zpow + e0, canon_lt2p(acc));
         }
         return;
     }
     const uint32_t t = blockIdx.x * KD_BLK + threadIdx.x;
-    Fr v = Fr::zero();
+    Fr29 v = zero29<FrParams>();
     {
         const uint32_t base = t * KD_L;
         if (base < n) {
             const Fr* __restrict__ p = a.p[blockIdx.y];
-            const Fr z = a.z[blockIdx.y];
+            const Fr29 z = to29(a.z[blockIdx.y]);
             const uint32_t top = min(n, base + KD_L);
-            for (uint32_t i = top; i-- > base;) v = fe_add(fe_mul(v, z), fe_load(p + i));
-        }
-    }
-    sh[threadIdx.x] = v;
+            v = to29(fe_load(p + top - 1));
+            for (uint32_t i = top - 1; i-- > base;) v = add29(mul29(v, z), to29(fe_load(p + i)));
+        }
+    }
+    v = norm29(v);
+    lds29_store<KD_BLK>(sh, threadIdx.x, v);
     __syncthreads();
 #pragma unroll 1
     for (uint32_t j = 0, d = 1; d < KD_BLK; d <<= 1, j++) {
-        Fr o = Fr::zero();
+        Fr29 o;
         const bool has = threadIdx.x + d < KD_BLK;
-        if (has) o = sh[threadIdx.x + d];
+        if (has) o = lds29_load<KD_BLK, FrParams>(sh, threadIdx.x + d);
         __syncthreads();
         if (has) {
-            v = fe_add(v, fe_mul(o, pw.step[blockIdx.y][j]));
-            sh[threadIdx.x] = v;
-        }
-        __syncthreads();
-    }
-    if (t < m) fe_store(suf + t, v);
-    if (threadIdx.x == 0) fe_store(agg + blockIdx.x, v);
+            v = norm29(add29(v, mul29(o, to29(pw.step[blockIdx.y][j]))));
+            lds29_store<KD_BLK>(sh, threadIdx.x, v);
+        }
+        __syncthreads();
+    }
+    const Fr r = reduce_canonical(v);
+    if (t < m) fe_store(suf + t, r);
+    if (threadIdx.x == 0) fe_store(agg + blockIdx.x, r);
 }
 
 __global__ __launch_bounds__(KD_BLK) void kd_apply_kernel(KdPtrs a, uint32_t n, Fr* __restrict__ scratch) {
@@ -811,7 +839,7 @@
     const Fr* zpow = tpow + nblk;
     const uint32_t blk = blockIdx.x;
     Fr g = Fr::zero();
-    for (uint32_t b = blk + 1 + threadIdx.x; b < nblk; b += KD_BLK) g = fe_add(g, fe_mul(fe_load(agg + b), fe_load(tpow + (b - blk - 1))));
+    for (uint32_t b = blk + 1 + threadIdx.x; b < nblk; b += KD_BLK) g = fe_add(g, mul_mem(fe_load(agg + b), fe_load(tpow + (b - blk - 1))));
     sh[threadIdx.x] = g;
     __syncthreads();
     for (uint32_t d = KD_BLK / 2; d; d >>= 1) {
@@ -824,15 +852,16 @@
     if (base >= n) return;
     const Fr* __restrict__ p = a.p[blockIdx.y];
     Fr* __restrict__ q = a.q[blockIdx.y];
-    const Fr z = a.z[blockIdx.y];
+    const Fr29 z = to29(a.z[blockIdx.y]);
     const uint32_t top = min(n, base + KD_L);
     const uint32_t last = min(m, (blk + 1) * KD_BLK) - 1;
     Fr run = (t < last) ? fe_load(suf + t + 1) : Fr::zero();
-    run = fe_add(run, fe_mul(fe_load(zpow + (last - t)), G));
+    run = fe_add(run, mul_mem(fe_load(zpow + (last - t)), G));
     for (uint32_t i = top; i-- > base;) {
         const Fr pi = fe_load(p + i);
         fe_store(q + i, run);
-        run = fe_add(fe_mul(run, z), pi);
+        if (i == base) break;
+        run = fe_add(canon_lt2p(mul29(to29(run), z)), pi);
     }
 }
 
@@ -847,19 +876,20 @@
     memset(&pt, 0, sizeof(pt));
     memset(&stp, 0, sizeof(stp));
     memset(&tp, 0, sizeof(tp));
+    const Fr k32 = fr_from_u64(32);
     for (uint32_t b = 0; b < count; b++) {
         pt.p[b] = p[b];
         pt.q[b] = q[b];
-        pt.z[b] = z[b];
+        pt.z[b] = fe_mul(z[b], k32);
         Fr Z = z[b];
         for (uint32_t i = 1; i < KD_L; i <<= 1) Z = fe_sqr(Z);
         Fr cur = Z;
         for (int j = 0; j < 8; j++) {
-            stp.step[b][j] = cur;
+            stp.step[b][j] = fe_mul(cur, k32);
             cur = fe_sqr(cur);
         }
         for (int j = 0; j < 10; j++) {
-            tp.top[b][j] = cur;
+            tp.top[b][j] = fe_mul(cur, k32);
             cur = fe_sqr(cur);
         }
     }
diff --git a/webauthn-halo2_amd/engine.py b/webauthn-halo2_amd/engine.py
--- a/webauthn-halo2_amd/engine.py
+++ b/webauthn-halo2_amd/engine.py
@@ -9,6 +9,7 @@
 ZK_BASIS_MONOMIAL = 0
 ZK_BASIS_LAGRANGE = 1
 ZK_T_MSM, ZK_T_NTT, ZK_T_QUOTIENT, ZK_T_EVAL, ZK_T_MSM_ACCUM, ZK_T_MSM_COLUMNS, ZK_T_MSM_TAIL_MAIN, ZK_T_MSM_TAIL = 0, 1, 2, 3, 4, 5, 6, 7
+ZK_T_MSM_T1_PARTS, ZK_T_MSM_T1_BUCKET = 8, 9
 
 
 ZK_TRANSCRIPT_BLAKE2B, ZK_TRANSCRIPT_EVM = 0, 1
```

New measurement: 103.3 (median of 5 runs). No clear change (+0.4%).
